# RinceWND/extPOM

Hardware: AMD Instinct MI355X
Metric: 3D cell-updates/sec on internal mode (one internal step = the 3-D baroclinic step and its isplit 2-D external substeps; whole-step wall time) (higher is better)
Workload: dtype f64

## Files before the change

### extpom_amd/csrc/k_adv.hip

```cpp
#include "pomgpu_internal.hpp"

#define dt_(i, j) F2(dt, i, j)
#define dx_(i, j) F2(dx, i, j)
#define dy_(i, j) F2(dy, i, j)
#define h_(i, j) F2(h, i, j)
#define u_(i, j, k) F3(u, i, j, k)
#define v_(i, j, k) F3(v, i, j, k)
#define ub_(i, j, k) F3(ub, i, j, k)
#define vb_(i, j, k) F3(vb, i, j, k)
#define w_(i, j, k) F3(w, i, j, k)
#define aam_(i, j, k) F3(aam, i, j, k)

#define MARCH3(call)                                                                  \
  const int g_ = (int)(blockIdx.x * blockDim.x + threadIdx.x);    \
  const int L_ = g_ >> 6, xcd_ = L_ & 7, m_ = L_ >> 3;                                \
  const int bpl_ = P.g_bpl, nbx_ = P.g_nbx;                                           \
  const int p_ = m_ % bpl_, t_ = m_ / bpl_;                                           \
  const int k = t_ % P.kb + 1;                                                        \
  const int band_ = (t_ / P.kb) * 8 + xcd_;                                           \
  const int i = (p_ % nbx_) * 64 + (g_ & 63) + 1;                                     \
  const int j = band_ * P.g_rb + (p_ / nbx_) * 4 + (int)threadIdx.y + 1;              \
  if (i > P.iml || j > P.jml) return;                                                 \
  call;
__device__ __forceinline__ void c_advct_a(const KP &P, const int i, const int j, const int k);
// ... 322 lines not shown
  }
  if (k >= 2 && k <= P.kbm1 && i >= 2 && i <= P.imm1 && j >= 2 && j <= P.jmm1) {
    const double fu = G3(ff, i, j, k - 1);
    double r = 0.;
    if (!(fc < value_min || fu < value_min)) {
      const double m = G3(zw, i, j, k);
      const double wdz = fabs(m);
      const double w2dt = P.dti2 * m * m / (F1(dzz, k - 1) * dt_(i, j));
      const double mol = (fu - fc) / (fc + fu + epsilon);
      r = (wdz - w2dt) * mol * P.sw;
      if (fabs(wdz) < fabs(w2dt)) r = 0.;
    }
    G3(zw, i, j, k) = r;
  }
}
__device__ __forceinline__ void c_copy3(const KP &P, const int i, const int j, const int k, double *dst, const double *src);
__global__ void k_copy3(KP P, double *dst, const double *src) {
  MARCH3(c_copy3(P, i, j, k, dst, src))
}
__device__ __forceinline__ void c_copy3(const KP &P, const int i, const int j, const int k, double *dst, const double *src) {
  G3(dst, i, j, k) = G3(src, i, j, k);
}
__device__ __forceinline__ void c_aam_copy(const KP &P, const int i, const int j, const int k, double *dst, const double *src) {
  if (k <= P.kbm1) G3(dst, i, j, k) = G3(src, i, j, k);
}
__global__ void k_aam_copy(KP P, double *dst, const double *src) {
  MARCH3(c_aam_copy(P, i, j, k, dst, src))
}
__device__ __forceinline__ double advt2_xdiff(const KP &P, const double *fb, const double *fc, int i, int j, int k) {
  const double am = 0.5 * (aam_(i, j, k) + aam_(i - 1, j, k));
  return -am * (h_(i, j) + h_(i - 1, j)) * P.tprni *
         ((G3(fb, i, j, k) - G3(fc, i, j, k)) - (G3(fb, i - 1, j, k) - G3(fc, i - 1, j, k))) * F2(dum, i, j) *
         (dy_(i, j) + dy_(i - 1, j)) * 0.5 / (dx_(i, j) + dx_(i - 1, j));
}
__device__ __forceinline__ double advt2_ydiff(const KP &P, const double *fb, const double *fc, int i, int j, int k) {
  const double am = 0.5 * (aam_(i, j, k) + aam_(i, j - 1, k));
  return -am * (h_(i, j) + h_(i, j - 1)) * P.tprni *
         ((G3(fb, i, j, k) - G3(fc, i, j, k)) - (G3(fb, i, j - 1, k) - G3(fc, i, j - 1, k))) * F2(dvm, i, j) *
         (dx_(i, j) + dx_(i, j - 1)) * 0.5 / (dy_(i, j) + dy_(i, j - 1));
}
__device__ __forceinline__ void c_advt2_diff(const KP &P, const int i, const int j, const int k, const double *fb, const double *fc, double *ff);
__global__ void k_advt2_diff(KP P, const double *fb, const double *fc, double *ff) {
  MARCH3(c_advt2_diff(P, i, j, k, fb, fc, ff))
}
__device__ __forceinline__ void c_advt2_diff(const KP &P, const int i, const int j, const int k, const double *fb, const double *fc, double *ff) {
  if (k > P.kbm1 || i < 2 || i > P.imm1 || j < 2 || j > P.jmm1) return;
  G3(ff, i, j, k) = G3(ff, i, j, k) -
                    P.dti2 * (advt2_xdiff(P, fb, fc, i + 1, j, k) - advt2_xdiff(P, fb, fc, i, j, k) +
                              advt2_ydiff(P, fb, fc, i, j + 1, k) - advt2_ydiff(P, fb, fc, i, j, k)) /
                        ((h_(i, j) + F2(etf, i, j)) * F2(art, i, j));
}

__device__ __forceinline__ double dens_point(const KP &P, double si, double ti, int i, int j, int k);
template <int TAU> __device__ __forceinline__ void c_ts_update(const KP &P, const int i, const int j, const int k, double fold, double fnew, int rt, int store_rst, double tau_b, double tau_f, const unsigned long long *rtf);
template <int TAU> __global__ void k_ts_update(KP P, double fold, double fnew, int rt, int store_rst, double tau_b, double tau_f, const unsigned long long *rtf) {
  MARCH3(c_ts_update<TAU>(P, i, j, k, fold, fnew, rt, store_rst, tau_b, tau_f, rtf))
}
__global__ void k_ts_update_same(KP P, double fold, double fnew, int rt, int store_rst, const unsigned long long *rtf) {
  MARCH3(c_ts_update<2>(P, i, j, k, fold, fnew, rt, store_rst, 0., 0., rtf))
}
template <int TAU> __device__ __forceinline__ void c_ts_update(const KP &P, const int i, const int j, const int k, double fold, double fnew, int rt, int store_rst, double tau_b, double tau_f, const unsigned long long *rtf) {
  const bool act = (i <= P.im && j <= P.jm), lev = (k <= P.kbm1);
  const pomgpu_ct m = F2(fsm, i, j);
  pomgpu_ct uf = F3(uf, i, j, k), vf = F3(vf, i, j, k);
  if (lev && act) {
    uf = uf * m;
    vf = vf * m;
  }
  pomgpu_ct tb = F3(tb, i, j, k), sb = F3(sb, i, j, k);
  bool rtc = rt != 0;
  if (rtc && rtf && lev) rtc = ((rtf[RT_WORD(P, i, j, k)] >> RT_BIT(i)) & 1ull) != 0;
  if (rtc) {
    const pomgpu_ct tc = F3(tclim, i, j, k), sc = F3(sclim, i, j, k);
    tb = (tb - tc) + tc;
    sb = (sb - sc) + sc;
  }
  const pomgpu_ct t0 = F3(t, i, j, k), s0 = F3(s, i, j, k);
  pomgpu_ct tbn = t0 + CT(.5) * CT(P.smoth) * (uf + tb - CT(2.) * t0);
  pomgpu_ct sbn = s0 + CT(.5) * CT(P.smoth) * (vf + sb - CT(2.) * s0);
  pomgpu_ct tn = uf, sn = vf;
  if (lev) {
    if (act) {
      const pomgpu_ct tr = CT(fold) * CT(F3(trstrb, i, j, k)) + CT(fnew) * CT(F3(trstrf, i, j, k));
      const pomgpu_ct sr = CT(fold) * CT(F3(srstrb, i, j, k)) + CT(fnew) * CT(F3(srstrf, i, j, k));
      pomgpu_ct ta;
      if (TAU == 1) ta = CT(fold) * CT(tau_b) + CT(fnew) * CT(tau_f);
      else if (TAU == 2) { const pomgpu_ct x = CT(F3(taurstrf, i, j, k)); ta = CT(fold) * x + CT(fnew) * x; }
      else ta = CT(fold) * CT(F3(taurstrb, i, j, k)) + CT(fnew) * CT(F3(taurstrf, i, j, k));
      if (store_rst) {
        F3(trstr, i, j, k) = tr;
        F3(srstr, i, j, k) = sr;
        F3(taurstr, i, j, k) = ta;
      }
      const pomgpu_ct c = CT(2.) * CT(P.dti) / CT(86400.);
      tn = tn + c * ta * (tr - tn);
      tbn = tbn + c * ta * (tr - tbn);
      sn = sn + c * ta * (sr - sn);
      sbn = sbn + c * ta * (sr - sbn);
    }
    tn = tn * m; tbn = tbn * m; sn = sn * m; sbn = sbn * m;
  }
  F3(t, i, j, k) = tn;
  F3(tb, i, j, k) = tbn;
  F3(s, i, j, k) = sn;
  F3(sb, i, j, k) = sbn;
  if (lev && act) F3(rho, i, j, k) = dens_point(P, sn, tn, i, j, k);
}
template <int NF> struct TrUpds { TrUpd u[NF]; };
template <int NF> __device__ __forceinline__ void c_tr_update(const KP &P, const int i, const int j, const int k, const TrUpds<NF> &A, int rt) {
  const bool msk = (i <= P.im && j <= P.jm && k <= P.kbm1);
  const double m = F2(fsm, i, j);
#pragma unroll
  for (int f = 0; f < NF; f++) {
    const TrUpd &u = A.u[f];
    double ff = G3(u.ff, i, j, k);
    if (msk) ff = ff * m;
    double fb = G3(u.fb, i, j, k);
    if (rt) {
      const double fc = G3(u.fc, i, j, k);
      fb = (fb - fc) + fc;
    }
    const double f0 = G3(u.f, i, j, k);
    G3(u.fb, i, j, k) = f0 + .5 * P.smoth * (ff + fb - 2. * f0);
    G3(u.f, i, j, k) = ff;
  }
}
template <int NF> __global__ void k_tr_update(KP P, TrUpds<NF> A, int rt) {
  MARCH3(c_tr_update<NF>(P, i, j, k, A, rt))
}
__device__ __forceinline__ void c_tr_source(const KP &P, const int i, const int j, const int k, double *ff, const double *fb, const double *fc, const double *q, double lam) {
  if (k > P.kbm1 || i > P.im || j > P.jm) return;
  double x = G3(fb, i, j, k);
  if (fc) { const double y = G3(fc, i, j, k); x = (x - y) + y; }
  const double a = lam * x;
  const double b = (q ? (double)G3(q, i, j, k) : 0.) - a;
  const double d = P.dti2 * b;
  G3(ff, i, j, k) = (double)G3(ff, i, j, k) + d;
}
__global__ void k_tr_source(KP P, double *ff, const double *fb, const double *fc, const double *q, double lam) {
  MARCH3(c_tr_source(P, i, j, k, ff, fb, fc, q, lam))
}
__device__ __forceinline__ void c_mask_ts(const KP &P, const int i, const int j, const int k);
__global__ void k_mask_ts(KP P) {
  MARCH3(c_mask_ts(P, i, j, k))
}
__device__ __forceinline__ void c_mask_ts(const KP &P, const int i, const int j, const int k) {
  if (k > P.kbm1 || i > P.im || j > P.jm) return;
  const double m = F2(fsm, i, j);
  F3(uf, i, j, k) = F3(uf, i, j, k) * m;
  F3(vf, i, j, k) = F3(vf, i, j, k) * m;
}
__device__ __forceinline__ void c_mask_uv(const KP &P, const int i, const int j, const int k);
__global__ void k_mask_uv(KP P) {
  MARCH3(c_mask_uv(P, i, j, k))
}
__device__ __forceinline__ void c_mask_uv(const KP &P, const int i, const int j, const int k) {
  if (k > P.kbm1 || i > P.im || j > P.jm) return;
  F3(uf, i, j, k) = F3(uf, i, j, k) * F2(dum, i, j);
  F3(vf, i, j, k) = F3(vf, i, j, k) * F2(dvm, i, j);
// ... 325 lines not shown
}
#undef LD2
#undef A3


void launch_advct_a(pomgpu_ctx *c) { LAUNCH(c, k_advct_a, gridm(c->P), blk2(), c->P); }
void launch_advct_b(pomgpu_ctx *c) { LAUNCH(c, k_advct_b, gridm(c->P), blk2(), c->P); }
void launch_advct_c(pomgpu_ctx *c) { LAUNCH(c, k_advct_c, gridm(c->P), blk2(), c->P); }
void launch_aam(pomgpu_ctx *c) {
  const KP &P = c->P;
#ifdef POMGPU_STORE_F32
  const bool pair_ok = false;
#else
  const bool pair_ok = true;
#endif
  if (pair_ok && P.iml % 2 == 0 && !SW(c, NO_PAIR)) {
    const long nbands = (P.jml + P.g_rb - 1) / P.g_rb, rounds = (nbands + 7) / 8;
    const long bpl = (long)((P.iml / 2 + 61) / 62) * (P.g_rb / 4);
    const long nch = (P.kbm1 + AAM_KCH - 1) / AAM_KCH;
    LAUNCHN(c, "k_aam_pair", k_aam_pair, dim3((unsigned)(8 * rounds * nch * bpl), 1, 1), blk2(), c->P);
  } else {
    LAUNCH(c, k_aam, gridm(c->P), blk2(), c->P);
  }
}
void launch_roundtrip(pomgpu_ctx *c, double *a, const double *b, int fix_kb) { LAUNCH(c, k_roundtrip, gridm(c->P), blk2(), c->P, a, b, fix_kb); }
void launch_roundtrip_level(pomgpu_ctx *c, double *a, const double *b, int k) { LAUNCH(c, k_roundtrip_level, grid2(c->P), blk2(), c->P, a, b, k); }
void launch_advq_flux(pomgpu_ctx *c, const double *q, const double *qb, double *xf, double *yf) {
  LAUNCH(c, k_advq_flux, gridm(c->P), blk2(), c->P, q, qb, xf, yf);
}
void launch_advq_step(pomgpu_ctx *c, const double *q, const double *qb, double *qf, const double *xf, const double *yf, int zero_else) {
  LAUNCH(c, k_advq_step, gridm(c->P), blk2(), c->P, q, qb, qf, xf, yf, zero_else);
}
void launch_q_filter(pomgpu_ctx *c, int mask) { LAUNCH(c, k_q_filter, gridm(c->P), blk2(), c->P, mask); }
void launch_q_filter_rim(pomgpu_ctx *c) {
  const KP &P = c->P;
  const int len = P.im > P.jm ? P.im : P.jm;
  LAUNCH(c, k_q_filter_rim, dim3((len + 63) / 64, 8, P.kb), dim3(64, 1, 1), c->P);
}
void launch_mask_q(pomgpu_ctx *c) { LAUNCH(c, k_mask_q, gridm(c->P), blk2(), c->P); }
void launch_advt1(pomgpu_ctx *c, double *fb, double *f, const double *fclim, double *ff) {
  LAUNCH(c, k_advt1, gridm(c->P), blk2(), c->P, (const double *)fb, (const double *)f, fclim, ff);
  LAUNCH(c, k_copy_kb, grid2(c->P), blk2(), c->P, f, (double *)NULL);
}
void launch_copy_kb(pomgpu_ctx *c, double *f, double *g) { LAUNCH(c, k_copy_kb, grid2(c->P), blk2(), c->P, f, g); }
void launch_advt2_mass(pomgpu_ctx *c) { LAUNCH(c, k_advt2_mass, gridm(c->P), blk2(), c->P); }
void launch_advt2_step(pomgpu_ctx *c, const double *fbmem, const double *f, const double *eta, double *ff, int itera) {
  LAUNCH(c, k_advt2_step, gridm(c->P), blk2(), c->P, fbmem, f, eta, ff, itera);
}
void launch_mask3(pomgpu_ctx *c, double *a, const double *m2) { LAUNCH(c, k_mask3, gridm(c->P), blk2(), c->P, a, m2); }
void launch_smol(pomgpu_ctx *c, const double *ff) { LAUNCH(c, k_smol, gridm(c->P), blk2(), c->P, ff); }
void launch_copy3(pomgpu_ctx *c, double *dst, const double *src) { LAUNCH(c, k_copy3, gridm(c->P), blk2(), c->P, dst, src); }
void launch_aam_copy(pomgpu_ctx *c, double *dst, const double *src) { LAUNCH(c, k_aam_copy, gridm(c->P), blk2(), c->P, dst, src); }
void launch_advt2_diff(pomgpu_ctx *c, const double *fb, const double *fc, double *ff) { LAUNCH(c, k_advt2_diff, gridm(c->P), blk2(), c->P, fb, fc, ff); }
void launch_ts_update(pomgpu_ctx *c, double fold, double fnew, int rt, int store_rst, int rt_flags) {
  const unsigned long long *rtf = (rt && rt_flags) ? c->rt_words : NULL;
  if (rtf && c->prof_on) {
    const int s = pomgpu_prof_slot(c, "ts_rt_flags");
    if (s >= 0) (c->parent ? c->parent : c)->prof[s].launches++;
  }
  if (c->tau_known[0] && c->tau_known[1] && !c->tau_handed && !SW(c, TAU_ARRAYS))
    LAUNCHN(c, "k_ts_update", (k_ts_update<1>), gridm(c->P), blk2(), c->P, fold, fnew, rt, store_rst, c->tau_val[0], c->tau_val[1], rtf);
  else if (c->tau_same && !c->tau_handed && !SW(c, TAU_ARRAYS))
    LAUNCH(c, k_ts_update_same, gridm(c->P), blk2(), c->P, fold, fnew, rt, store_rst, rtf);
  else
    LAUNCHN(c, "k_ts_update", (k_ts_update<0>), gridm(c->P), blk2(), c->P, fold, fnew, rt, store_rst, 0., 0., rtf);
}
void launch_restore_fields(pomgpu_ctx *c, double fold, double fnew) { LAUNCH(c, k_restore_fields, gridm(c->P), blk2(), c->P, fold, fnew); }
void launch_mask_ts(pomgpu_ctx *c) { LAUNCH(c, k_mask_ts, gridm(c->P), blk2(), c->P); }
void launch_tr_update(pomgpu_ctx *c, const TrUpd *u, int nf, int rt) {
  if (nf == 2) {
    TrUpds<2> A; A.u[0] = u[0]; A.u[1] = u[1];
    LAUNCHN(c, "k_tr_update2", (k_tr_update<2>), gridm(c->P), blk2(), c->P, A, rt);
  } else {
    TrUpds<1> A; A.u[0] = u[0];
    LAUNCHN(c, "k_tr_update", (k_tr_update<1>), gridm(c->P), blk2(), c->P, A, rt);
  }
}
void launch_tr_source(pomgpu_ctx *c, double *ff, const double *fb, const double *fc, const double *q, double lam) {
  LAUNCH(c, k_tr_source, gridm(c->P), blk2(), c->P, ff, fb, fc, q, lam);
}
void launch_mask_uv(pomgpu_ctx *c) { LAUNCH(c, k_mask_uv, gridm(c->P), blk2(), c->P); }
void launch_mask_w(pomgpu_ctx *c) { LAUNCH(c, k_mask_w, gridm(c->P), blk2(), c->P); }
void launch_restore(pomgpu_ctx *c, double fold, double fnew) { LAUNCH(c, k_restore, gridm(c->P), blk2(), c->P, fold, fnew); }
void launch_restore_shift(pomgpu_ctx *c) { LAUNCH(c, k_restore_shift, gridm(c->P), blk2(), c->P); }
void launch_restore_load(pomgpu_ctx *c, const double *tr, const double *sr, double tau, const double *taur, int fill_tau) { LAUNCH(c, k_restore_load, gridm(c->P), blk2(), c->P, tr, sr, tau, taur, fill_tau); }
void launch_probe_gpow15(pomgpu_ctx *c, long n, const double *x, double *out) { LAUNCH(c, k_probe_gpow15, dim3((unsigned)((n + 255) / 256), 1, 1), dim3(256, 1, 1), n, x, out); }
void launch_dens(pomgpu_ctx *c, const double *si, const double *ti, double *rhoo) { LAUNCH(c, k_dens, gridm(c->P), blk2(), c->P, si, ti, rhoo); }
void launch_realvertvl(pomgpu_ctx *c, int etf_is_et) {
  if (SW(c, REALVERTVL_CELLS)) LAUNCH(c, k_realvertvl, gridm(c->P), blk2(), c->P, etf_is_et);
  else LAUNCHN(c, "k_realvertvl_col", k_realvertvl_col, grid2(c->P), blk2(), c->P, etf_is_et);
}
```

### extpom_amd/csrc/k_tile.hip

```cpp
#include "pomgpu_internal.hpp"


__global__ void k_coef_static(KP P) {
  const int i = TID_I, j = TID_J;
  if (i > P.iml || j > P.jml) return;
  const int iw = i > 1 ? i - 1 : 1, js = j > 1 ? j - 1 : 1;
  P.m8[IX2(i, j)] = (unsigned char)((F2(fsm, i, j) != 0. ? 1 : 0) | (F2(dum, i, j) != 0. ? 2 : 0) | (F2(dvm, i, j) != 0. ? 4 : 0));
  K2(HSX, i, j) = F2(h, i, j) + F2(h, iw, j);
  K2(HSY, i, j) = F2(h, i, j) + F2(h, i, js);
  K2(DYSX, i, j) = F2(dy, i, j) + F2(dy, iw, j);
  K2(DXSX, i, j) = F2(dx, i, j) + F2(dx, iw, j);
  K2(DXSY, i, j) = F2(dx, i, j) + F2(dx, i, js);
  K2(DYSY, i, j) = F2(dy, i, j) + F2(dy, i, js);
  K2(DX4, i, j) = F2(dx, i, j) + F2(dx, iw, j) + F2(dx, i, js) + F2(dx, iw, js);
  K2(DY4, i, j) = F2(dy, i, j) + F2(dy, iw, j) + F2(dy, i, js) + F2(dy, iw, js);
  const int ie = i < P.iml ? i + 1 : P.iml, jn = j < P.jml ? j + 1 : P.jml;
  K2(CVA, i, j) = F2(dy, ie, j) - F2(dy, iw, j);
  K2(CVB, i, j) = F2(dx, i, jn) - F2(dx, i, js);
  K2(R2DXSX, i, j) = 2.0 / (F2(dx, i, j) + F2(dx, iw, j));
  K2(R2DYSY, i, j) = 2.0 / (F2(dy, i, j) + F2(dy, i, js));
  K2(RDX, i, j) = 1.0 / F2(dx, i, j);
  K2(RDY, i, j) = 1.0 / F2(dy, i, j);
  if (j == 1)
    for (int n = i - 1; n < POM_NBLK1D * P.kb; n += P.iml) P.r1[n] = 1.0 / P.b1[n];
}
__global__ void k_coef_dt(KP P) {
  const int i = TID_I, j = TID_J;
  if (i > P.iml || j > P.jml) return;
  const int iw = i > 1 ? i - 1 : 1, js = j > 1 ? j - 1 : 1;
  K2(CMX, i, j) = 0.25 * (F2(dy, iw, j) + F2(dy, i, j)) * (F2(dt, iw, j) + F2(dt, i, j));
  K2(CMY, i, j) = 0.25 * (F2(dx, i, js) + F2(dx, i, j)) * (F2(dt, i, js) + F2(dt, i, j));
  K2(DTSX, i, j) = F2(dt, i, j) + F2(dt, iw, j);
  K2(DTSY, i, j) = F2(dt, i, j) + F2(dt, i, js);
  K2(DT4, i, j) = F2(dt, i, j) + F2(dt, iw, j) + F2(dt, i, js) + F2(dt, iw, js);
}
__global__ void k_coef_eta(KP P, int uvm) {
  const int i = TID_I, j = TID_J;
  if (i > P.iml || j > P.jml) return;
  K2(HEA, i, j) = (F2(h, i, j) + F2(etb, i, j)) * F2(art, i, j);
  K2(HFA, i, j) = (F2(h, i, j) + F2(etf, i, j)) * F2(art, i, j);
  if (uvm) {
    const unsigned long long mb = UVM_MARK;
    double mark;
    __builtin_memcpy(&mark, &mb, sizeof mark);
    const int iw = i > 1 ? i - 1 : 1, js = j > 1 ? j - 1 : 1;
    const double cu = (F2(utb, i, j) + F2(utf, i, j)) / (F2(dt, i, j) + F2(dt, iw, j));
    const double cv = (F2(vtb, i, j) + F2(vtf, i, j)) / (F2(dt, i, j) + F2(dt, i, js));
    K2(UCOR, i, j) = (i >= 2 && i <= P.im && j <= P.jm) ? cu : mark;
    K2(VCOR, i, j) = (j >= 2 && j <= P.jm && i <= P.im) ? cv : mark;
  }
}

__device__ __forceinline__ pomgpu_ct upw_(pomgpu_ct m, pomgpu_ct lo, pomgpu_ct hi) {
  return CT(0.5) * ((m + fabs(m)) * lo + (m - fabs(m)) * hi);
}
struct FaceT { pomgpu_ct adv, dif; };
struct TFields { const double *fb[2], *f[2], *fcl[2]; double *ff[2]; unsigned long long *rtf; };
template <int NF> struct LevT { pomgpu_ct c[2 * NF + 2], o[2], h[ROWSHARE_SLOTS(2 * NF + 2)]; };
template <int NS> struct NbrT { pomgpu_ct s[NS], n[NS]; };
struct CoefT { pomgpu_ct cm, hs, msk, ds_num; InvDc den; };
__device__ __forceinline__ CoefT coef_x(const KP &P, int i, int j) {
  CoefT c; c.cm = K2(CMX, i, j); c.hs = K2(HSX, i, j); c.msk = F2(dum, i, j); c.ds_num = K2(DYSX, i, j); c.den = inv_of(CT(K2(DXSX, i, j))); return c;
}
__device__ __forceinline__ CoefT coef_y(const KP &P, int i, int j) {
  CoefT c; c.cm = K2(CMY, i, j); c.hs = K2(HSY, i, j); c.msk = F2(dvm, i, j); c.ds_num = K2(DXSY, i, j); c.den = inv_of(CT(K2(DYSY, i, j))); return c;
}
__device__ __forceinline__ FaceT advt2_face(const pomgpu_ct tprni, const CoefT &c, pomgpu_ct vel, pomgpu_ct fb_hi, pomgpu_ct fb_lo, pomgpu_ct fc_hi,
                                            pomgpu_ct fc_lo, pomgpu_ct am_hi, pomgpu_ct am_lo) {
  FaceT f;
  f.adv = upw_(c.cm * vel, fb_lo, fb_hi);
  const pomgpu_ct am = CT(0.5) * (am_hi + am_lo);
  f.dif = divi(-am * c.hs * tprni * ((fb_hi - fc_hi) - (fb_lo - fc_lo)) * c.msk * c.ds_num * CT(0.5), c.den);
  return f;
}
#if COL_WX != 1
#error "the row-sharing column kernels keep one wavefront per workgroup row (COL_WX == 1)"
#endif
// ... 104 lines not shown
        auto east = [&] {
          return advt2_face(tprni, coef_x(P, ie, jc), uvm_ld<0>(P, ie, jc, L), G3(A.fb[f], ie, jc, L), fb_c, G3(A.fcl[f], ie, jc, L), fc_c,
                            G3(P.aamc, ie, jc, L), am_c);
        };
        FaceT xe;
        xe.adv = halo_e(xw.adv, [&] { return east().adv; });
        xe.dif = halo_e(xw.dif, [&] { return east().dif; });
        const FaceT ys = advt2_face(tprni, cs, v_c, fb_c, nb.s[f], fc_c, nb.s[NF + f], am_c, nb.s[AM]);
        const FaceT yn = advt2_face(tprni, cn, nb.n[VV], nb.n[f], fb_c, nb.n[NF + f], fc_c, nb.n[AM], am_c);
        s_adv = xe.adv - xw.adv + yn.adv - ys.adv;
        s_dif = xe.dif - xw.dif + yn.dif - ys.dif;
        zu = (L == 1) ? w_c * f1[f] * art : upw_(w_c, fb_c, p_fb[f]) * art;
      }
      {
        pomgpu_ct rr = p_adv[f] + divi(p_zu[f] - zu, dzk);
        rr = divi(p_fb[f] * hea - dti2 * rr, hfa);
        rr = rr * fsm;
        rr = rr - divi(dti2 * p_dif[f], hfa);
        bstc(bff[f], (L >= 2 && L <= kbm1 + 1) ? ost : BOFF_NONE, (unsigned)(L >= 2 ? L - 2 : 0) * lvb, rr);
      }
      p_adv[f] = s_adv; p_dif[f] = s_dif; p_fb[f] = fb_c; p_zu[f] = zu;
    }
  };
  LevT<NF> ra, rb;
  load(ra, 0u);
  rb = ra;
  for (int L = 1; L <= kbm1 + 1; L += 2) {
    step(L, 1, ra, rb);
    step(L + 1, 0, rb, ra);
  }
  if (icol) {
    for (int k = in ? P.kb : 1; k <= P.kb; k++) {
#pragma unroll
      for (int f = 0; f < NF; f++) G3(A.ff[f], i, jc, k) = CT(G3(A.ff[f], i, jc, k)) * fsm;
    }
  }
}

struct QFields { const double *q[2], *qb[2]; double *qf[2]; };
template <int NF, int NO = 2> struct LevQa { pomgpu_ct c[2 * NF + 2], o[NO], h[ROWSHARE_SLOTS(2 * NF + 2)]; };
struct CoefQ { pomgpu_ct dts, hs, msk, ds_num; InvDc den; };
__device__ __forceinline__ CoefQ coefq_x(const KP &P, int i, int j) {
  CoefQ c; c.dts = K2(DTSX, i, j); c.hs = K2(HSX, i, j); c.msk = F2(dum, i, j); c.den = inv_of(CT(K2(DXSX, i, j))); c.ds_num = K2(DYSX, i, j); return c;
}
__device__ __forceinline__ CoefQ coefq_y(const KP &P, int i, int j) {
  CoefQ c; c.dts = K2(DTSY, i, j); c.hs = K2(HSY, i, j); c.msk = F2(dvm, i, j); c.den = inv_of(CT(K2(DYSY, i, j))); c.ds_num = K2(DXSY, i, j); return c;
}
__device__ __forceinline__ pomgpu_ct advq_face(const CoefQ &c, pomgpu_ct q_hi, pomgpu_ct q_lo, pomgpu_ct vel_k, pomgpu_ct vel_km1, pomgpu_ct am_hi_k,
                                               pomgpu_ct am_lo_k, pomgpu_ct am_hi_m, pomgpu_ct am_lo_m, pomgpu_ct qb_hi, pomgpu_ct qb_lo) {
  pomgpu_ct x = CT(.125) * (q_hi + q_lo) * c.dts * (vel_k + vel_km1);
  x = x - divi(CT(.25) * (am_hi_k + am_lo_k + am_hi_m + am_lo_m) * c.hs * (qb_hi - qb_lo) * c.msk, c.den);
  return CT(.5) * c.ds_num * x;
}
template <int NF, bool WF = false, bool UM = false>
__global__ void __launch_bounds__(64 * LDS_ROWS) k_advq_col(KP P, QFields A, int zero_else) {
  constexpr int NS = 2 * NF + 2, NH = ROWSHARE_SLOTS(NS), AM = 2 * NF, VV = 2 * NF + 1;
  typedef LevQa<NF, WF ? 1 : 2> Lev;
  HALO_XCD_DECODE_R(LDS_ROWS)
  const int r = WAVE_UNIFORM((int)threadIdx.y), j0w = j - r;
  const bool jrow = j <= P.jml;
  const int jc = jrow ? j : P.jml;
  const bool icol = jrow && (lane >= 1 && lane <= 62 && i0 <= P.iml);
#ifdef POMGPU_EMU
  if (!icol) return;
#endif
  const int i = i0 < 1 ? 1 : (i0 > P.iml ? P.iml : i0);
  const int iw = i > 1 ? i - 1 : 1, ie = i < P.iml ? i + 1 : P.iml;
  const int js = jc > 1 ? jc - 1 : 1, jn = jc < P.jml ? jc + 1 : P.jml;
  const bool in = icol && (i >= 2 && i <= P.imm1 && jc >= 2 && jc <= P.jmm1);
  const CoefQ cw = coefq_x(P, i, jc), cs = coefq_y(P, i, jc), cn = coefq_y(P, i, jn);
  const pomgpu_ct art = F2(art, i, jc), hea = K2(HEA, i, jc);
  const InvDc hfa = inv_of(CT(K2(HFA, i, jc)));
  const int kb = P.kb, kbm1 = P.kbm1;
  BufA bs[NS], bo[2], bqf[NF], bh[NH];
  const double *ps[NS];
#pragma unroll
  for (int f = 0; f < NF; f++) { ps[f] = A.q[f]; ps[NF + f] = A.qb[f]; bqf[f] = BUF3(A.qf[f]); }
  ps[AM] = P.aamc; ps[VV] = A3(v); bo[0] = BUF3(A3(u)); bo[1] = BUF3(A3(w));
#pragma unroll
  for (int x = 0; x < NS; x++) bs[x] = BUF3(ps[x]);
  const RowShare<NS> S = rowshare_setup<NS>(P, r, j, j0w, i);
#pragma unroll
  for (int q = 0; q < NH; q++) bh[q] = BUF3(rowshare_pick<NS>(ps, S.hop[q]));
  const UvmC mu = UM ? uvm_of<0>(P, i, jc) : uvm_none(), mv = UM ? uvm_of<1>(P, i, jc) : uvm_none();
  UvmC mh[NH];
#pragma unroll
  for (int q = 0; q < NH; q++) mh[q] = UM ? rowshare_uvm<1, NS, LDS_ROWS>(P, S, q, VV, j0w, i) : uvm_none();
  const unsigned oc = BOFF2(i, jc), lvb = LVB;
  const unsigned ost = in ? oc : ((zero_else && icol) ? oc : BOFF_NONE);
  const unsigned ostw = in ? oc : BOFF_NONE;
#ifndef POMGPU_EMU
  __shared__ pomgpu_ct slab[2][NS][ROWSHARE_ROWS][64];
#else
  const unsigned os = BOFF2(i, js), on = BOFF2(i, jn);
#endif
  double vv_cw = 0., vv_ce = 0., vv_cs = 0., vv_cn = 0., vv_det = 0., vv_m = 0., wk = 0.;
  InvD vv_area; vv_area.b = vv_area.y = 0.;
  if constexpr (WF) {
    vv_m = F2(fsm, i, jc);
    const double dyc = F2(dy, i, jc), dtc = F2(dt, i, jc), dxc = F2(dx, i, jc);
    const double dyw = halo_w(dyc, [&] { return F2(dy, iw, jc); }), dtw = halo_w(dtc, [&] { return F2(dt, iw, jc); });
    const double dye = halo_e(dyc, [&] { return F2(dy, ie, jc); }), dte = halo_e(dtc, [&] { return F2(dt, ie, jc); });
    vv_cw = .25 * (dyc + dyw) * (dtc + dtw);
    vv_ce = .25 * (dye + dyc) * (dte + dtc);
    vv_cs = .25 * (dxc + F2(dx, i, js)) * (dtc + F2(dt, i, js));
    vv_cn = .25 * (F2(dx, i, jn) + dxc) * (F2(dt, i, jn) + dtc);
    vv_area = inv_of(dxc * dyc);
    vv_det = (F2(etf, i, jc) - F2(etb, i, jc)) / P.dti2;
    wk = 0.5 * (F2(vfluxb, i, jc) + F2(vfluxf, i, jc));
  }
  auto load = [&](Lev &L, int k) {
    const unsigned lv = (unsigned)WAVE_UNIFORM(k - 1) * lvb;
#pragma unroll
    for (int x = 0; x < NS; x++) L.c[x] = bldc(bs[x], oc, lv);
    L.o[0] = bldc(bo[0], oc, lv);
    if constexpr (!WF) L.o[1] = bldc(bo[1], oc, lv);
#pragma unroll
    for (int q = 0; q < NH; q++) L.h[q] = bldc(bh[q], S.hoff[q], lv);
  };
  pomgpu_ct u_m = 0., v_m = 0., vn_m = 0., am_m = 0., ams_m = 0., amn_m = 0.;
  pomgpu_ct am_w_prv = 0.;
  pomgpu_ct ue_m = 0.;
  pomgpu_ct wq_pp[NF], wq_p[NF];
  pomgpu_ct xe_p[NF], xw_p[NF], yn_p[NF], ys_p[NF], qb_p[NF];
#pragma unroll
  for (int f = 0; f < NF; f++) wq_pp[f] = wq_p[f] = xe_p[f] = xw_p[f] = yn_p[f] = ys_p[f] = qb_p[f] = 0.;
  auto step = [&](const int L, const int par, const Lev &cur, Lev &nxt) {
    load(nxt, L + 1 <= kb ? L + 1 : kb);
    NbrT<NS> nb;
    const bool lcor = L <= kbm1;
    const pomgpu_ct v_c = uvm_fix(cur.c[VV], mv, lcor), u_c = uvm_fix(cur.o[0], mu, lcor);
#ifndef POMGPU_EMU
#pragma unroll
    for (int x = 0; x < NS; x++) slab[par][x][r + 1][lane] = x == VV ? v_c : cur.c[x];
#pragma unroll
    for (int q = 0; q < NH; q++) slab[par][S.hop[q]][S.hrow[q]][lane] = uvm_fix(cur.h[q], mh[q], lcor);
    __syncthreads();
#pragma unroll
    for (int x = 0; x < NS; x++) { nb.s[x] = slab[par][x][S.ss][lane]; nb.n[x] = slab[par][x][S.sn][lane]; }
#else
    const unsigned lvc = (unsigned)((L <= kb ? L : kb) - 1) * lvb;
#pragma unroll
    for (int x = 0; x < NS; x++) { nb.s[x] = bldc(bs[x], os, lvc); nb.n[x] = bldc(bs[x], on, lvc); }
    nb.s[VV] = uvm_fix(nb.s[VV], uvm_of<1>(P, i, js), lcor); nb.n[VV] = uvm_fix(nb.n[VV], uvm_of<1>(P, i, jn), lcor);
#endif
    const pomgpu_ct am_c = cur.c[AM];
    const pomgpu_ct am_s = nb.s[AM], am_n = nb.n[AM], v_n = nb.n[VV];
    const pomgpu_ct am_w = halo_w(am_c, [&] { return G3(P.aamc, iw, jc, L); });
    pomgpu_ct w_c, ue_c = 0.;
    if constexpr (WF) {
      ue_c = halo_e(u_c, [&] { return uvm_ld<0>(P, ie, jc, L); });
      const double wn = wk + F1(dz, L >= 2 ? L - 1 : 1) *
                             (divi(vv_ce * (double)ue_m - vv_cw * (double)u_m + vv_cn * (double)vn_m - vv_cs * (double)v_m, vv_area) + vv_det);
      wk = L >= 2 ? wn : wk;
      const double wst = L <= kbm1 ? wk * vv_m : wk;
      bst(bo[1], ostw, (unsigned)WAVE_UNIFORM(L - 1) * lvb, wst);
      w_c = CT((pomgpu_st)wst);
    } else {
      w_c = cur.o[1];
    }
    const int k = L - 1;
    InvDc dz2; dz2.b = dz2.y = 0.;
    if (k >= 2 && k <= kbm1) { dz2.b = CT(F1(dz, k)) + CT(F1(dz, k - 1)); dz2.y = CT(1.0) / dz2.b; }
#pragma unroll
    for (int f = 0; f < NF; f++) {
      const pomgpu_ct q_c = cur.c[f], qb_c = cur.c[NF + f];
      pomgpu_ct xe_c = 0., xw_c = 0., yn_c = 0., ys_c = 0.;
      if (L >= 2 && L <= kbm1) {
        const pomgpu_ct q_w = halo_w(q_c, [&] { return G3(A.q[f], iw, jc, L); });
        const pomgpu_ct qb_w = halo_w(qb_c, [&] { return G3(A.qb[f], iw, jc, L); });
        const pomgpu_ct xw = advq_face(cw, q_c, q_w, u_c, u_m, am_c, am_w, am_m, am_w_prv, qb_c, qb_w);
        xw_c = xw;
        xe_c = halo_e(xw, [&] {
          return advq_face(coefq_x(P, ie, jc), G3(A.q[f], ie, jc, L), q_c, uvm_ld<0>(P, ie, jc, L), uvm_ld<0>(P, ie, jc, L - 1), G3(P.aamc, ie, jc, L), am_c,
                           G3(P.aamc, ie, jc, L - 1), am_m, G3(A.qb[f], ie, jc, L), qb_c);
        });
        ys_c = advq_face(cs, q_c, nb.s[f], v_c, v_m, am_c, am_s, am_m, ams_m, qb_c, nb.s[NF + f]);
        yn_c = advq_face(cn, nb.n[f], q_c, v_n, vn_m, am_n, am_c, amn_m, am_m, nb.n[NF + f], qb_c);
      }
      const pomgpu_ct wq_c = w_c * q_c;
      {
        pomgpu_ct rr = 0.;
        if (in && k >= 2 && k <= kbm1) {
          rr = divi((wq_pp[f] - wq_c) * art, dz2) + xe_p[f] - xw_p[f] + yn_p[f] - ys_p[f];
          rr = divi(hea * qb_p[f] - CT(P.dti2) * rr, hfa);
        }
        const bool lev_in = (k >= 2 && k <= kbm1);
        const unsigned o = (k >= 1) ? (lev_in ? ost : ((zero_else && icol) ? oc : BOFF_NONE)) : BOFF_NONE;
        bstc(bqf[f], o, (unsigned)WAVE_UNIFORM(k >= 1 ? k - 1 : 0) * lvb, rr);
      }
      wq_pp[f] = wq_p[f]; wq_p[f] = wq_c; qb_p[f] = qb_c;
      xe_p[f] = xe_c; xw_p[f] = xw_c; yn_p[f] = yn_c; ys_p[f] = ys_c;
    }
    am_w_prv = am_w;
    if constexpr (WF) ue_m = ue_c;
    u_m = u_c; v_m = v_c; vn_m = v_n; am_m = am_c; ams_m = am_s; amn_m = am_n;
  };
  Lev ra, rb;
  load(ra, 1);
  rb = ra;
  for (int L = 1; L <= kb; L += 2) {
    step(L, 1, ra, rb);
    if (L + 1 <= kb) step(L + 1, 0, rb, ra);
  }
  if (icol && zero_else) {
#pragma unroll
    for (int f = 0; f < NF; f++) G3(A.qf[f], i, jc, kb) = 0.;
  }
  if constexpr (WF) {
    if (icol && !in && i0 <= P.im && jc <= P.jm)
      for (int k = 1; k <= kbm1; k++) F3(w, i, jc, k) = F3(w, i, jc, k) * vv_m;
  }
// ... 370 lines not shown
                    v_n = uvm_fix(bldc(bs[V], on, (unsigned)(k - 1) * lvb), uvm_of<1>(P, i, jn));
#endif
    const pomgpu_ct w_c = c.c[W];
    const pomgpu_ct w_w = halo_w(w_c, [&] { return F3(w, iw, jc, k + 1); });
    const pomgpu_ct tc = cd_c * (v_n + v_k);
    const pomgpu_ct tw = halo_w(tc, [&] { return F2(cor, iw, jc) * F2(dt, iw, jc) * (uvm_ld<1>(P, iw, jn, k) + uvm_ld<1>(P, iw, jc, k)); });
    const pomgpu_ct u_e = halo_e(u_k, [&] { return uvm_ld<0>(P, ie, jc, k); });
    const pomgpu_ct u_se = halo_e(u_s, [&] { return uvm_ld<0>(P, ie, js, k); });
    pomgpu_ct fu_n = 0., fv_n = 0.;
    if (k + 1 <= kbm1) {
      if (i >= 2) fu_n = CT(.25) * (w_c + w_w) * (u_c + u_k);
      if (jc >= 2) fv_n = CT(.25) * (w_c + w_s) * (v_c + v_k);
    }
    pomgpu_ct ru = fu_k, rv = fv_k;
    if (in) {
      InvDc dzk; dzk.b = F1(dz, k); dzk.y = R1(dz, k);
      ru = divi(sau * c.ub - CT(2.) * dti2 * (c.advx + divi((fu_k - fu_n) * aru, dzk) - aru * CT(.25) * (tc + tw) + hcu + c.drhox), sdu);
      rv = divi(sav * c.vb -
                    CT(2.) * dti2 * (c.advy + divi((fv_k - fv_n) * arv, dzk) + arv * CT(.25) * (cd_c * (u_e + u_k) + cd_s * (u_se + u_s)) + hcv + c.drhoy),
                sdv);
    }
    const unsigned lv = (unsigned)WAVE_UNIFORM(k - 1) * lvb;
    bstc(buf, ost, lv, ru);
    bstc(bvf, ost, lv, rv);
    fu_k = fu_n; fv_k = fv_n;
    u_k = u_c; v_k = v_c;
  };
  LevUV ra, rb;
  load(ra, 1);
  rb = ra;
  for (int k = 1; k <= kbm1; k += 6) {
    step(k, 1, ra, rb);
    if (k + 1 <= kbm1) step(k + 1, 2, rb, ra);
    if (k + 2 <= kbm1) step(k + 2, 0, ra, rb);
    if (k + 3 <= kbm1) step(k + 3, 1, rb, ra);
    if (k + 4 <= kbm1) step(k + 4, 2, ra, rb);
    if (k + 5 <= kbm1) step(k + 5, 0, rb, ra);
  }
  if (out) { F3(uf, i, jc, kb) = 0.; F3(vf, i, jc, kb) = 0.; }
}

void launch_coef_static(pomgpu_ctx *c) { LAUNCH(c, k_coef_static, grid2(c->P), blk2(), c->P); }
void launch_coef_dt(pomgpu_ctx *c) { LAUNCH(c, k_coef_dt, grid2(c->P), blk2(), c->P); }
void launch_coef_eta(pomgpu_ctx *c, int uvm) { LAUNCH(c, k_coef_eta, grid2(c->P), blk2(), c->P, uvm); }
void launch_advq_col(pomgpu_ctx *c, const double *q, const double *qb, double *qf, int zero_else) {
  QFields A; A.q[0] = A.q[1] = q; A.qb[0] = A.qb[1] = qb; A.qf[0] = A.qf[1] = qf;
  LAUNCHN(c, "k_advq_col", (k_advq_col<1>), grid1_halo_r(c->P, LDS_ROWS), blk_col_r(LDS_ROWS), c->P, A, zero_else);
}
void launch_advq2_col(pomgpu_ctx *c, const double *q, const double *qb, double *qf, const double *ql, const double *qlb, double *qlf, int zero_else) {
  QFields A; A.q[0] = q; A.qb[0] = qb; A.qf[0] = qf; A.q[1] = ql; A.qb[1] = qlb; A.qf[1] = qlf;
  LAUNCHN(c, "k_advq2_col", (k_advq_col<2>), grid1_halo_r(c->P, LDS_ROWS), blk_col_r(LDS_ROWS), c->P, A, zero_else);
}
#if POMGPU_W_FUSE
void launch_advq2w_col(pomgpu_ctx *c, const double *q, const double *qb, double *qf, const double *ql, const double *qlb, double *qlf, int zero_else) {
  QFields A; A.q[0] = q; A.qb[0] = qb; A.qf[0] = qf; A.q[1] = ql; A.qb[1] = qlb; A.qf[1] = qlf;
#if POMGPU_UVM_ONLOAD
  if (c->P.uvm) { LAUNCHN(c, "k_advq2_col", (k_advq_col<2, true, true>), grid1_halo_r(c->P, LDS_ROWS), blk_col_r(LDS_ROWS), c->P, A, zero_else); return; }
#endif
  LAUNCHN(c, "k_advq2_col", (k_advq_col<2, true>), grid1_halo_r(c->P, LDS_ROWS), blk_col_r(LDS_ROWS), c->P, A, zero_else);
}
#endif
void launch_advct_col(pomgpu_ctx *c, int sum2d, double *aam_w) {
  const bool rows4 = SW(c, ADVCT_ROWS4) || (!SW(c, ADVCT_ROWS8) && c->P.jml <= 400 && c->exch);
  sum2d = (sum2d ? 1 : 0) | (POMGPU_UVM_ONLOAD && !c->exch && !c->tp.on && !c->wide.on && !(c->flags & POMGPU_CTX_2D) ? 2 : 0);
#if POMGPU_AAM_FUSE
  if (aam_w) {
    if (c->prof_on) {
      const int s = pomgpu_prof_slot(c, "advct_aam_fused");
      if (s >= 0) (c->parent ? c->parent : c)->prof[s].launches++;
    }
    LAUNCHN(c, "k_advct_col", (k_advct_col<LDS_ROWS, true>), grid1_halo_r(c->P, LDS_ROWS), blk_col_r(LDS_ROWS), c->P, sum2d, aam_w);
    return;
  }
#endif
  if (rows4) LAUNCHN(c, "k_advct_col", (k_advct_col<4>), grid1_halo_r(c->P, 4), blk_col_r(4), c->P, sum2d, (double *)NULL);
  else LAUNCHN(c, "k_advct_col", (k_advct_col<LDS_ROWS>), grid1_halo_r(c->P, LDS_ROWS), blk_col_r(LDS_ROWS), c->P, sum2d, (double *)NULL);
}
__global__ void k_advct_fix2d(KP P, int west, int south) {
  const int t = TID_I;
  if (west && t >= 2 && t <= P.jmm1) {
    double a = 0.;
#pragma unroll 8
    for (int k = 1; k <= P.kbm1; k++) a = a + F3(advx, 2, t, k) * F1(dz, k);
    F2(adx2d, 2, t) = a;
  }
  if (south && t >= 2 && t <= P.imm1) {
    double a = 0.;
#pragma unroll 8
    for (int k = 1; k <= P.kbm1; k++) a = a + F3(advy, t, 2, k) * F1(dz, k);
    F2(ady2d, t, 2) = a;
  }
}
void launch_advct_fix2d(pomgpu_ctx *c, int west, int south) {
  const KP &P = c->P;
  const int len = P.im > P.jm ? P.im : P.jm;
  LAUNCH(c, k_advct_fix2d, dim3((len + 63) / 64, 1, 1), dim3(64, 1, 1), c->P, west, south);
}
void launch_advct_edge(pomgpu_ctx *c, double *to_e, double *to_n) {
  const KP &P = c->P;
  const int len = P.im > P.jm ? P.im : P.jm;
  LAUNCH(c, k_advct_edge, dim3((len + 63) / 64, P.kbm1, 1), dim3(64, 1, 1), c->P, to_e, to_n);
}
void launch_advct_fix(pomgpu_ctx *c, const double *from_w, const double *from_s) {
  const KP &P = c->P;
  const int len = P.im > P.jm ? P.im : P.jm;
  LAUNCH(c, k_advct_fix, dim3((len + 63) / 64, P.kbm1, 1), dim3(64, 1, 1), c->P, from_w, from_s);
}
void launch_advuv_col(pomgpu_ctx *c) {
#if POMGPU_UVM_ONLOAD
// ... 29 lines not shown
```

### extpom_amd/csrc/k_vert.hip

```cpp
#include <type_traits>
#include "pomgpu_internal.hpp"
#include "dd_exp.h"

#define dt_(i, j) F2(dt, i, j)
#define dx_(i, j) F2(dx, i, j)
#define dy_(i, j) F2(dy, i, j)
#define h_(i, j) F2(h, i, j)
#define u_(i, j, k) F3(u, i, j, k)
#define v_(i, j, k) F3(v, i, j, k)
#define w_(i, j, k) F3(w, i, j, k)

#define ROWS_PROFUV 1
#define ROWS_PROFT 1
#ifndef ROWS_UVF
#define ROWS_UVF 8
#endif
#ifndef ROWS_UVM
#define ROWS_UVM 4
#endif
#define COL2                               \
  const int i = TID_I, j = TID_J;          \
  if (i > P.iml || j > P.jml) return;

__global__ void k_baropg(KP P, int sum2d) {
// ... 310 lines not shown
    const unsigned lv = (unsigned)WAVE_UNIFORM(k - 1) * lvb;
    L.u = bld(bu, oc, lv); L.v = bld(bv, oc, lv); L.vh = bld(bv, onh, lv);
  };
  double wk = 0.5 * (F2(vfluxb, i, jc) + F2(vfluxf, i, jc));
  bst(bw, ost, 0u, mask ? wk * m : wk);
  auto step = [&](const int k, const Lev &cur, Lev &nxt) {
    const int par = k & 1;
    load(nxt, k + 2 <= kbm1 ? k + 2 : kbm1);
#ifndef POMGPU_EMU
    slab[par][r][lane] = cur.v;
    if (r == VVL_ROWS - 1) slab[par][VVL_ROWS][lane] = cur.vh;
    __syncthreads();
    const double v_n = slab[par][r + 1][lane];
#else
    (void)par;
    const double v_n = F3(v, i, jn, k);
#endif
    const double u_e = halo_e(cur.u, [&] { return F3(u, ie, jc, k); });
    wk = wk + F1(dz, k) * (divi(ce * u_e - cw * cur.u + cn * v_n - cs * cur.v, area) + det);
    bst(bw, ost, (unsigned)WAVE_UNIFORM(k) * lvb, (mask && k + 1 <= kbm1) ? wk * m : wk);
  };
  Lev ra, rb, rc;
  load(ra, 1);
  load(rb, 2 <= kbm1 ? 2 : kbm1);
  rc = ra;
  for (int k = 1; k <= kbm1; k += 3) {
    step(k, ra, rc);
    if (k + 1 <= kbm1) step(k + 1, rb, ra);
    if (k + 2 <= kbm1) step(k + 2, rc, rb);
  }
  if (own && !in && mask)
    for (int k = 1; k <= kbm1; k++) F3(w, i, jc, k) = w_(i, jc, k) * m;
}

__global__ void k_profq_bc(KP P) {
  COL2
  if (i > P.im || j > P.jm) return;
  double ut = 0.;
  if (i <= P.imm1 && j <= P.jmm1) {
    ut = sqrt(sq(.5 * (F2(wusurf, i, j) + F2(wusurf, i + 1, j))) + sq(.5 * (F2(wvsurf, i, j) + F2(wvsurf, i, j + 1))));
    F3(uf, i, j, P.kb) =
        sqrt(sq(.5 * (F2(wubot, i, j) + F2(wubot, i + 1, j))) + sq(.5 * (F2(wvbot, i, j) + F2(wvbot, i, j + 1)))) * P.const1_profq;
  }
  G2(P.s2[4], i, j) = ut;
}
__device__ __forceinline__ double profq_cc(const KP &P, int i, int j, int k) {
  const double tp = F3(t, i, j, k) + P.tbias;
  const double sp = F3(s, i, j, k) + P.sbias;
  const double p = P.grav * P.rhoref * (-F1(zz, k) * h_(i, j)) * 1.e-4;
  double cc = 1449.1 + .00821 * p + 4.55 * tp - .045 * sq(tp) + 1.34 * (sp - 35.0);
  cc = cc / sqrt((1. - .01642 * p / cc) * (1. - 0.40 * p / sq(cc)));
  return cc;
}
__device__ __forceinline__ double profq_cc_v(const KP &P, double t, double s_, double hij, int k) {
  const double tp = t + P.tbias;
  const double sp = s_ + P.sbias;
  const double p = P.grav * P.rhoref * (-F1(zz, k) * hij) * 1.e-4;
  double cc = 1449.1 + .00821 * p + 4.55 * tp - .045 * sq(tp) + 1.34 * (sp - 35.0);
  cc = cc / sqrt((1. - .01642 * p / cc) * (1. - 0.40 * p / sq(cc)));
  return cc;
}
__device__ __forceinline__ double profq_rho(const KP &P, int i, int j, int k, int rho_rt) {
  const double r = F3(rho, i, j, k);
  if (!rho_rt) return r;
  const double m = F3(rmean, i, j, k);
  return (r - m) + m;
}
__device__ __forceinline__ double profq_boygr(const KP &P, int i, int j, int k, double ccm, double cck, int rho_rt = 0) {
  return P.grav * (profq_rho(P, i, j, k - 1, rho_rt) - profq_rho(P, i, j, k, rho_rt)) / (F1(dzz, k - 1) * h_(i, j)) +
         sq(P.grav) * 2. / (sq(ccm) + sq(cck));
}
__global__ void k_profq_prod(KP P, int rho_rt) {
  COL2
  if (i > P.im || j > P.jm) return;
  double *prod = P.s3[0];
  G3(prod, i, j, 1) = 0.;
  G3(prod, i, j, P.kb) = 0.;
  const bool in = (i >= 2 && i <= P.imm1 && j >= 2 && j <= P.jmm1);
  if (!in) {
    for (int k = 2; k <= P.kbm1; k++) G3(prod, i, j, k) = 0.;
    return;
  }
  const double dh = h_(i, j) + F2(etf, i, j);
  const double sef = 1., shiw = 0.;
  double ccm = profq_cc(P, i, j, 1);
  for (int k = 2; k <= P.kbm1; k++) {
    const double cck = profq_cc(P, i, j, k);
    const double bg = profq_boygr(P, i, j, k, ccm, cck, rho_rt);
    const double km = F3(km, i, j, k);
    double p = km * .25 * sef *
                   (sq(u_(i, j, k) - u_(i, j, k - 1) + u_(i + 1, j, k) - u_(i + 1, j, k - 1)) +
                    sq(v_(i, j, k) - v_(i, j, k - 1) + v_(i, j + 1, k) - v_(i, j + 1, k - 1))) /
                   sq(F1(dzz, k - 1) * dh) -
               shiw * km * bg;
    p = p + F3(kh, i, j, k) * bg;
    G3(prod, i, j, k) = p;
    ccm = cck;
  }
}
__global__ void k_profq_prod_lines(KP P, int rho_rt) {
  const int t = TID_I, line = (int)blockIdx.y, k = (int)blockIdx.z + 1;
  int i, j;
  if (line < 4) { if (t > P.jm) return; j = t; i = line == 0 ? 1 : (line == 1 ? 2 : (line == 2 ? P.imm1 : P.im)); }
  else { if (t > P.im) return; i = t; j = line == 4 ? 1 : (line == 5 ? 2 : (line == 6 ? P.jmm1 : P.jm)); }
  double *prod = P.s3[0];
  double p = 0.;
  const bool wanted = line == 1 ? !P.W : (line == 2 ? !P.E : (line == 5 ? !P.S : (line == 6 ? !P.N : true)));
  if (!wanted) return;
  if (k >= 2 && k <= P.kbm1 && i >= 2 && i <= P.imm1 && j >= 2 && j <= P.jmm1) {
    const double dh = h_(i, j) + F2(etf, i, j);
    const double sef = 1., shiw = 0.;
    const double ccm = profq_cc(P, i, j, k - 1), cck = profq_cc(P, i, j, k);
    const double bg = profq_boygr(P, i, j, k, ccm, cck, rho_rt);
    const double km = F3(km, i, j, k);
    p = km * .25 * sef *
            (sq(u_(i, j, k) - u_(i, j, k - 1) + u_(i + 1, j, k) - u_(i + 1, j, k - 1)) +
             sq(v_(i, j, k) - v_(i, j, k - 1) + v_(i, j + 1, k) - v_(i, j + 1, k - 1))) /
            sq(F1(dzz, k - 1) * dh) -
        shiw * km * bg;
    p = p + F3(kh, i, j, k) * bg;
  }
  G3(prod, i, j, k) = p;
}
struct LevQ { double t, s, rho, rm, q2b, q2lb, q2, km, kh, uf, vf, uc, ue, vc, vn, kq1, prod; };
struct LevB { double e1, g1, e2, g2, qb, qlb, q, ql; };
#ifndef PROFQ_KL
#define PROFQ_KL 19
#endif
#ifndef PROFQ_BIG
#define PROFQ_BIG 8
#endif
template <int FP, int FF, int ROWS, int LD = 1>
__global__ void __launch_bounds__(64 * ROWS) k_profq(KP P, int rho_rt_pace, int jfirst, int jlast, const unsigned *rtcol) {
#ifndef POMGPU_EMU
  constexpr int KL = ROWS >= 8 ? PROFQ_KL : (PROFQ_KL < 9 ? PROFQ_KL : 9);
  __shared__ double evec[2 * KL][ROWS][64];
#endif
  const int i = TID_I, j = TID_J + jfirst - 1;
  if (i > P.iml || j > P.jml || j > jlast) return;
  const int rho_rt = rho_rt_pace & 1, pace = rho_rt_pace & 2;
  const int ty = (int)threadIdx.y, tx = (int)threadIdx.x;
  if (i > P.im || j > P.jm) return;
  const double a1 = 0.92, b1 = 16.6, a2 = 0.74, b2 = 10.1, c1 = 0.08, e1 = 1.8, e2 = 1.33, surfl = 2.e5;
  const int kb = P.kb, kbm1 = P.kbm1;
  const double dh = h_(i, j) + F2(etf, i, j);
  const double utau2 = G2(P.s2[4], i, j);
  const double l0 = surfl * utau2 / P.grav;
  const double umol2 = 2. * P.umol;
  const double z1 = F1(z, 1), zkb = F1(z, kb);
  const double coef4 = 18. * a1 * a1 + 9. * a1 * a2, coef5 = 9. * a1 * a2;
  const double coef1 = a2 * (1. - 6. * a1 / b1 * 1.), coef2 = 3. * a2 * b2 / 1. + 18. * a1 * a2,
               coef3 = a1 * (1. - 3. * c1 - 6. * a1 / b1 * 1.);
  const bool repl = (P.W && i == 1) || (P.E && i == P.im) || (P.S && j == 1) || (P.N && j == P.jm);
  const int ti = (P.W && i == 2) ? 1 : ((P.E && i == P.imm1) ? P.im : 0);
  const int tj = (P.S && j == 2) ? 1 : ((P.N && j == P.jmm1) ? P.jm : 0);
  const double fsm_c = F2(fsm, i, j);
  const double m_ti = F2(fsm, ti ? ti : i, j), m_tj = F2(fsm, i, tj ? tj : j), m_tij = F2(fsm, ti ? ti : i, tj ? tj : j);
  const bool pin = FP && (i >= 2 && i <= P.imm1 && j >= 2 && j <= P.jmm1);
  const bool ffil = FF && (i >= 3 && i <= P.imm1 - 1 && j >= 3 && j <= P.jmm1 - 1);
  const int ie = i < P.iml ? i + 1 : i, jn = j < P.jml ? j + 1 : j;
  const double hij = h_(i, j);
  const InvD dhk = inv_of(dh * P.kappa);
  UvmC m_uc = uvm_none(), m_ue = uvm_none(), m_vc = uvm_none(), m_vn = uvm_none();
#if POMGPU_UVM_ONLOAD
  if (FP == 1 && P.uvm) {
    m_uc.s = K2(USUM, i, j); m_uc.c = K2(UCOR, i, j); m_ue.s = K2(USUM, ie, j); m_ue.c = K2(UCOR, ie, j);
    m_vc.s = K2(VSUM, i, j); m_vc.c = K2(VCOR, i, j); m_vn.s = K2(VSUM, i, jn); m_vn.c = K2(VCOR, i, jn);
    m_uc.on = m_ue.on = m_vc.on = m_vn.on = true;
  }
#endif
#define bt BUF3(A3(t))
#define bs_ BUF3(A3(s))
#define brho BUF3(A3(rho))
#define bq2b BUF3(A3(q2b))
#define bq2lb BUF3(A3(q2lb))
#define bq2 BUF3(A3(q2))
#define bq2l BUF3(A3(q2l))
#define bkm BUF3(A3(km))
#define bkh BUF3(A3(kh))
#define bkq BUF3(A3(kq))
#define buf BUF3(A3(uf))
#define bvf BUF3(A3(vf))
#define bu BUF3(A3(u))
#define bv BUF3(A3(v))
#define bl BUF3(A3(l))
#define bdt BUF3(A3(dtef))
#define bpr BUF3(P.s3[0])
#define be1 BUF3(P.s3[4])
#define be2 BUF3(P.s3[5])
  const unsigned oc = BOFF2(i, j), oe = BOFF2(ie, j), on = BOFF2(i, jn), lvb = LVB;
  const unsigned o_k = repl ? BOFF_NONE : oc;
  const unsigned o_abs = ffil ? BOFF_NONE : oc;
  const unsigned o_fil = ffil ? oc : BOFF_NONE, o_uv = ffil ? BOFF_NONE : oc;
  const unsigned o_pr = (FP == 0 || (FP == 2 && !pin)) ? oc : BOFF_NONE;
  unsigned o_rm = rho_rt ? oc : BOFF_NONE;
  if (rho_rt_pace & 4) o_rm = (rho_rt && rtcol[(size_t)(j - 1) * P.iml + (i - 1)]) ? oc : BOFF_NONE;
#ifdef PROFQ_OLDWALK
  const double vbot = P.kappa * (1 + F1(z, kbm1)) * dh * F3(q2, i, j, kbm1);
  const double ufbot = F3(uf, i, j, kb);
#else
  double ufbot;
#endif
  double e1p = 0., g1p = P.cb_profq * utau2;
  double e2p = 0., g2p = 0.;
  double ccm = 0., rhom = 0.;
  double kqm = 0., kqc = F3(kq, i, j, 1);
  double ucm = 0., uem = 0., vcm = 0., vnm = 0.;
#ifdef PROFQ_OLDWALK
  auto lev = [&](LevQ &L, int k) {
    const unsigned lv = (unsigned)WAVE_UNIFORM(k - 1) * lvb;
    L.t = bld(bt, oc, lv); L.s = bld(bs_, oc, lv); L.rho = bld(brho, oc, lv); L.rm = bld(BUF3(A3(rmean)), o_rm, lv);
    L.q2b = bld(bq2b, oc, lv); L.q2lb = bld(bq2lb, oc, lv); L.q2 = bld(bq2, oc, lv);
    L.km = bld(bkm, oc, lv); L.kh = bld(bkh, oc, lv);
    L.uf = bld(buf, oc, lv); L.vf = bld(bvf, oc, lv);
    if (FP) { L.uc = bld(bu, oc, lv); L.ue = bld(bu, oe, lv); L.vc = bld(bv, oc, lv); L.vn = bld(bv, on, lv); }
    else L.uc = L.ue = L.vc = L.vn = 0.;
    L.kq1 = bld(bkq, oc, (unsigned)WAVE_UNIFORM(k < kb ? k : kb - 1) * lvb);
    L.prod = (FP != 1) ? bld(bpr, o_pr, lv) : 0.;
  };
  auto step = [&](const int k, const LevQ &cur, LevQ &nxt) {
    lev(nxt, k + 1 <= kb ? k + 1 : kb);
    const bool mid = (k >= 2 && k <= kbm1);
    const unsigned lv = (unsigned)WAVE_UNIFORM(k - 1) * lvb;
    const double kqp = cur.kq1;
    double cck = 0., rhok = 0.;
    if (k <= kbm1) { cck = profq_cc_v(P, cur.t, cur.s, hij, k); rhok = (o_rm != BOFF_NONE) ? (cur.rho - cur.rm) + cur.rm : cur.rho; }
    double q2b = cur.q2b;
    double l, gh = 0.;
    double uck = 0., uek = 0., vck = 0., vnk = 0., bg = 0.;
    if (pin && k <= kbm1) { uck = uvm_fix(cur.uc, m_uc); uek = uvm_fix(cur.ue, m_ue); vck = uvm_fix(cur.vc, m_vc); vnk = uvm_fix(cur.vn, m_vn); }
    double q2lb = 0.;
    if (mid) {
      q2b = fabs(q2b);
      q2lb = fabs(cur.q2lb);
      bg = P.grav * (rhom - rhok) / (F1(dzz, k - 1) * hij) + sq(P.grav) * 2. / (sq(ccm) + sq(cck));
      l = fabs(q2lb / q2b);
      if (F1(z, k) > -0.5) l = fmax(l, P.kappa * l0);
      gh = fmin(sq(l) * bg / q2b, .028);
    } else {
      l = (k == 1) ? P.kappa * l0 : 0.;
    }
    bst(bq2b, mid ? o_abs : BOFF_NONE, lv, q2b);
    bst(bq2lb, mid ? o_abs : BOFF_NONE, lv, q2lb);
    if (LD) bst(bl, oc, lv, l);
    const double dtef1 = sqrt(fabs(q2b)) * 1. / (b1 * l + P.small_);
    double dtef2 = dtef1;
    if (mid) dtef2 = dtef1 * (1. + e2 * sq(divi((1. / fabs(F1(z, k) - z1) + 1. / fabs(F1(z, k) - zkb)) * l, dhk)));
    if (LD) bst(bdt, oc, lv, dtef2);
    if (mid) {
      const double a = -P.dti2 * (kqp + kqc + umol2) * .5 / (F1(dzz, k - 1) * F1(dz, k) * dh * dh);
      const double c = -P.dti2 * (kqm + kqc + umol2) * .5 / (F1(dzz, k - 1) * F1(dz, k - 1) * dh * dh);
      double pr;
      if (FP == 0 || (FP == 2 && !pin)) {
        pr = cur.prod;
      } else if (pin) {
        const double sef = 1., shiw = 0.;
        const double km = cur.km;
        pr = km * .25 * sef * (sq(uck - ucm + uek - uem) + sq(vck - vcm + vnk - vnm)) / sq(F1(dzz, k - 1) * dh) - shiw * km * bg;
        pr = pr + cur.kh * bg;
      } else {
        pr = 0.;
      }
      const double g = 1. / (a + c * (1. - e1p) - (2. * P.dti2 * dtef1 + 1.));
      e1p = a * g;
      g1p = (-2. * P.dti2 * pr + c * g1p - cur.uf) * g;
      if (k == 2) {
        e2p = 0.;
        g2p = -P.kappa * F1(z, 2) * dh * cur.q2;
      } else {
        const double rhs = (k == kbm1) ? vbot : cur.vf;
        const double g2 = 1. / (a + c * (1. - e2p) - (P.dti2 * dtef2 + 1.));
        e2p = a * g2;
        g2p = (P.dti2 * (-pr * l * e1) + c * g2p - rhs) * g2;
      }
    }
    {
      const unsigned ov = (k <= kbm1) ? oc : BOFF_NONE;
#ifndef POMGPU_EMU
      const bool inl = k <= KL;
      if (inl) { evec[k - 1][ty][tx] = e1p; evec[KL + k - 1][ty][tx] = e2p; }
      const unsigned oe_ = inl ? BOFF_NONE : ov;
#else
      const unsigned oe_ = ov;
#endif
      bst(be1, oe_, lv, e1p); bst(buf, ov, lv, g1p); bst(be2, oe_, lv, e2p); bst(bvf, ov, lv, g2p);
    }
    double kq_n = 0., km_n = 0., kh_n = 0.;
    {
      const double sh = coef1 / (1. - coef2 * gh);
      double sm = coef3 + sh * coef4 * gh;
      sm = sm / (1. - coef5 * gh);
      const double pl = l * sqrt(fabs(cur.q2));
      kq_n = (pl * .41 * sh + kqc) * .5;
      km_n = (pl * sm + cur.km) * .5;
      kh_n = (pl * sh + cur.kh) * .5;
      bst(bkq, o_k, lv, kq_n * fsm_c);
      bst(bkm, o_k, lv, km_n * fsm_c);
      bst(bkh, o_k, lv, kh_n * fsm_c);
    }
    if ((ti | tj) && !repl) {
#define PUT(ii, jj, m)                               \
  {                                                  \
    G3(P.s3[1], ii, jj, k) = km_n * m;               \
    G3(P.s3[2], ii, jj, k) = kh_n * m;               \
    G3(P.s3[3], ii, jj, k) = kq_n * m;               \
  }
      if (ti) PUT(ti, j, m_ti)
      if (tj) PUT(i, tj, m_tj)
      if (ti && tj) PUT(ti, tj, m_tij)
#undef PUT
    }
    ccm = cck; rhom = rhok;
    ucm = uck; uem = uek; vcm = vck; vnm = vnk;
    kqm = kqc; kqc = kqp;
  };
  {
    LevQ ra, rb;
    lev(ra, 1);
    rb = ra;
    for (int k = 1; k <= kb; k += 2) {
      if (pace) PACE_BARRIER();
      step(k, ra, rb);
      if (k + 1 <= kb) step(k + 1, rb, ra);
    }
  }
#else
  enum { PH_1, PH_2, PH_LDS, PH_MEM, PH_KBM1, PH_KB };
  auto lev = [&](LevQ &L, int k) {
    const unsigned lv = (unsigned)WAVE_UNIFORM(k - 1) * lvb;
    L.t = bld(bt, oc, lv); L.s = bld(bs_, oc, lv); L.rho = bld(brho, oc, lv); L.rm = bld(BUF3(A3(rmean)), o_rm, lv);
    L.q2b = bld(bq2b, oc, lv); L.q2lb = bld(bq2lb, oc, lv); L.q2 = bld(bq2, oc, lv);
    L.km = bld(bkm, oc, lv); L.kh = bld(bkh, oc, lv);
    L.uf = bld(buf, oc, lv); L.vf = bld(bvf, oc, lv);
    if (FP) { L.uc = bld(bu, oc, lv); L.ue = bld(bu, oe, lv); L.vc = bld(bv, oc, lv); L.vn = bld(bv, on, lv); }
    else L.uc = L.ue = L.vc = L.vn = 0.;
    L.kq1 = bld(bkq, oc, (unsigned)WAVE_UNIFORM(k < kb ? k : kb - 1) * lvb);
    L.prod = (FP != 1) ? bld(bpr, o_pr, lv) : 0.;
  };
  auto step = [&](auto ph, const int k, const LevQ &cur, LevQ &nxt) {
    constexpr int PH = decltype(ph)::value;
    constexpr bool mid = (PH != PH_1 && PH != PH_KB);
    if (PH != PH_KB) lev(nxt, k + 1);
    const unsigned lv = (unsigned)WAVE_UNIFORM(k - 1) * lvb;
    const double kqp = cur.kq1;
    double cck = 0., rhok = 0.;
    if (PH != PH_KB) { cck = profq_cc_v(P, cur.t, cur.s, hij, k); rhok = (o_rm != BOFF_NONE) ? (cur.rho - cur.rm) + cur.rm : cur.rho; }
    double q2b = cur.q2b;
    double l, gh = 0.;
    double uck = 0., uek = 0., vck = 0., vnk = 0., bg = 0.;
    if (PH != PH_KB) {
      uck = pin ? uvm_fix(cur.uc, m_uc) : 0.; uek = pin ? uvm_fix(cur.ue, m_ue) : 0.;
      vck = pin ? uvm_fix(cur.vc, m_vc) : 0.; vnk = pin ? uvm_fix(cur.vn, m_vn) : 0.;
    }
    double q2lb = 0.;
    if (mid) {
      q2b = fabs(q2b);
      q2lb = fabs(cur.q2lb);
      bg = P.grav * (rhom - rhok) / (F1(dzz, k - 1) * hij) + sq(P.grav) * 2. / (sq(ccm) + sq(cck));
      l = fabs(q2lb / q2b);
      const double lmx = fmax(l, P.kappa * l0);
      l = (F1(z, k) > -0.5) ? lmx : l;
      gh = fmin(sq(l) * bg / q2b, .028);
      bst(bq2b, o_abs, lv, q2b);
      bst(bq2lb, o_abs, lv, q2lb);
    } else {
      l = (PH == PH_1) ? P.kappa * l0 : 0.;
    }
    if (LD) bst(bl, oc, lv, l);
    const double dtef1 = sqrt(fabs(q2b)) * 1. / (b1 * l + P.small_);
    double dtef2 = dtef1;
    if (mid) dtef2 = dtef1 * (1. + e2 * sq(divi((1. / fabs(F1(z, k) - z1) + 1. / fabs(F1(z, k) - zkb)) * l, dhk)));
    if (LD) bst(bdt, oc, lv, dtef2);
    if (mid) {
      const double a = -P.dti2 * (kqp + kqc + umol2) * .5 / (F1(dzz, k - 1) * F1(dz, k) * dh * dh);
      const double c = -P.dti2 * (kqm + kqc + umol2) * .5 / (F1(dzz, k - 1) * F1(dz, k - 1) * dh * dh);
      double pr;
      if (FP == 0) {
        pr = cur.prod;
      } else {
        const double sef = 1., shiw = 0.;
        const double km = cur.km;
        pr = km * .25 * sef * (sq(uck - ucm + uek - uem) + sq(vck - vcm + vnk - vnm)) / sq(F1(dzz, k - 1) * dh) - shiw * km * bg;
        pr = pr + cur.kh * bg;
        pr = pin ? pr : (FP == 2 ? cur.prod : 0.);
      }
      const double g = 1. / (a + c * (1. - e1p) - (2. * P.dti2 * dtef1 + 1.));
      e1p = a * g;
      g1p = (-2. * P.dti2 * pr + c * g1p - cur.uf) * g;
      if (PH == PH_2) {
        e2p = 0.;
        g2p = -P.kappa * F1(z, 2) * dh * cur.q2;
      } else {
        const double rhs = (PH == PH_KBM1) ? P.kappa * (1 + F1(z, kbm1)) * dh * cur.q2 : cur.vf;
        const double g2 = 1. / (a + c * (1. - e2p) - (P.dti2 * dtef2 + 1.));
        e2p = a * g2;
        g2p = (P.dti2 * (-pr * l * e1) + c * g2p - rhs) * g2;
      }
    }
    if (PH != PH_KB) {
#ifndef POMGPU_EMU
      if (PH == PH_1 || PH == PH_2 || PH == PH_LDS) {
        evec[k - 1][ty][tx] = e1p; evec[KL + k - 1][ty][tx] = e2p;
      } else if (PH == PH_MEM) {
        bst(be1, oc, lv, e1p); bst(be2, oc, lv, e2p);
      } else {
        const bool inl = k <= KL;
        if (inl) { evec[k - 1][ty][tx] = e1p; evec[KL + k - 1][ty][tx] = e2p; }
        const unsigned oe_ = inl ? BOFF_NONE : oc;
        bst(be1, oe_, lv, e1p); bst(be2, oe_, lv, e2p);
      }
#else
      bst(be1, oc, lv, e1p); bst(be2, oc, lv, e2p);
#endif
      bst(buf, oc, lv, g1p); bst(bvf, oc, lv, g2p);
    }
    double kq_n = 0., km_n = 0., kh_n = 0.;
    {
      const double sh = coef1 / (1. - coef2 * gh);
      double sm = coef3 + sh * coef4 * gh;
      sm = sm / (1. - coef5 * gh);
      const double pl = l * sqrt(fabs(cur.q2));
      kq_n = (pl * .41 * sh + kqc) * .5;
      km_n = (pl * sm + cur.km) * .5;
      kh_n = (pl * sh + cur.kh) * .5;
      bst(bkq, o_k, lv, kq_n * fsm_c);
      bst(bkm, o_k, lv, km_n * fsm_c);
      bst(bkh, o_k, lv, kh_n * fsm_c);
    }
    if ((ti | tj) && !repl) {
#define PUT(ii, jj, m)                               \
  {                                                  \
    G3(P.s3[1], ii, jj, k) = km_n * m;               \
    G3(P.s3[2], ii, jj, k) = kh_n * m;               \
    G3(P.s3[3], ii, jj, k) = kq_n * m;               \
  }
// ... 865 lines not shown
  G3(b, i, j, kb) = c_kb;
  G3(c, i, j, kb) = f_kb;
  if (V) F2(tps, i, j) = su;
#undef KC
}
__global__ void k_uv_filter_rim(KP P) {
  if (blockIdx.z == 0) d_uv_filter_rim<0>(P);
  else d_uv_filter_rim<1>(P);
}

static inline dim3 colblk() { return dim3(64, 2, 1); }
static inline dim3 rowblk(int rows) { return dim3(64, rows, 1); }
static inline dim3 rowgrid(const KP &P, int rows) { return dim3((P.iml + 63) / 64, (P.jml + rows - 1) / rows, 1); }
static inline dim3 colgrid(const KP &P) { return dim3((P.iml + 63) / 64, (P.jml + 1) / 2, 1); }
#define COLV_G(P) dim3(((P).iml + 63) / 64, ((P).jml + 3) / 4, 1)
#define COLV_B dim3(64, 4, 1)
int launch_baropg(pomgpu_ctx *c, int sum2d, unsigned *rtcol) {
  if (SW(c, BAROPG_CELLS)) { LAUNCH(c, k_baropg, COLV_G(c->P), COLV_B, c->P, sum2d); return 0; }
  LAUNCHN(c, "k_baropg", k_baropg_rs, grid1_halo_r(c->P, BPG_ROWS), blk_col_r(BPG_ROWS), c->P, sum2d, rtcol);
  return rtcol != NULL;
}
void launch_baropg_mcc(pomgpu_ctx *c, int sum2d) { LAUNCH(c, k_baropg_mcc, colgrid(c->P), colblk(), c->P, sum2d); }
void launch_order_pack(pomgpu_ctx *c, double *send_e, double *send_n) {
  const KP &P = c->P;
  const int len = P.iml > P.jml ? P.iml : P.jml;
  LAUNCH(c, k_order_pack, dim3((len + 63) / 64, P.kb + 1, 1), dim3(64, 1, 1), c->P, send_e, send_n);
}
static inline dim3 twin(dim3 g) { g.z = 2; return g; }
template <class F> static void with_kbt(int kb, F f) {
  if (kb <= 24) f(std::integral_constant<int, 24>{});
  else if (kb <= 32) f(std::integral_constant<int, 32>{});
  else if (kb <= 40) f(std::integral_constant<int, 40>{});
  else if (kb <= 44) f(std::integral_constant<int, 44>{});
  else if (kb <= 50) f(std::integral_constant<int, 50>{});
  else if (kb <= 56) f(std::integral_constant<int, 56>{});
  else f(std::integral_constant<int, 64>{});
}
#define KBT_OF(t) decltype(t)::value
void launch_int_uvmean(pomgpu_ctx *c) {
  if (!pomgpu_reg_kb(c)) { LAUNCH(c, k_int_uvmean, colgrid(c->P), colblk(), c->P); return; }
  with_kbt(c->P.kb, [&](auto t) { LAUNCHN(c, "k_int_uvmean_reg2", (k_int_uvmean_reg2<KBT_OF(t)>), twin(rowgrid(c->P, ROWS_UVM)), rowblk(ROWS_UVM), c->P); });
}
void launch_vertvl(pomgpu_ctx *c, int mask) {
  if (SW(c, VERTVL_CELLS)) { LAUNCH(c, k_vertvl, COLV_G(c->P), COLV_B, c->P, mask); return; }
  LAUNCHN(c, "k_vertvl", k_vertvl_rs, grid1_halo_r(c->P, VVL_ROWS), blk_col_r(VVL_ROWS), c->P, mask);
}
void launch_profq_bc(pomgpu_ctx *c) { LAUNCH(c, k_profq_bc, colgrid(c->P), colblk(), c->P); }
void launch_profq_prod(pomgpu_ctx *c, int lines_only, int rho_rt) {
  if (!lines_only) { LAUNCH(c, k_profq_prod, colgrid(c->P), colblk(), c->P, rho_rt); return; }
  const KP &P = c->P;
  const int len = P.im > P.jm ? P.im : P.jm;
  LAUNCH(c, k_profq_prod_lines, dim3((len + 63) / 64, 8, P.kb), dim3(64, 1, 1), c->P, rho_rt);
}
void launch_profq(pomgpu_ctx *c, int fuse_prod, int fuse_filter, int rho_rt, int jfirst, int jlast, int store_ld) {
  if (jlast < jfirst) { jfirst = 1; jlast = c->P.jml; }
  const int ld = store_ld || fuse_prod != 1 || !fuse_filter;
  if (ld && c->prof_on) {
    const int s = pomgpu_prof_slot(c, "profq_ld_store");
    if (s >= 0) (c->parent ? c->parent : c)->prof[s].launches++;
  }
  const int nrows = jlast - jfirst + 1;
  const int rows8 = !SW(c, PROFQ_ROWS2) && (SW(c, PROFQ_ROWS8) || (long)((c->P.iml + 63) / 64) * ((c->P.jml + 7) / 8) >= 3 * 256);
  const int cols = rho_rt && c->rho_rt_cols && !SW(c, RT_LOAD);
  if (cols && c->prof_on) {
    const int s = pomgpu_prof_slot(c, "profq_rm_flags");
    if (s >= 0) (c->parent ? c->parent : c)->prof[s].launches++;
  }
  rho_rt = (rho_rt ? 1 : 0) | (SW(c, PROFQ_NOPACE) ? 0 : 2) | (cols ? 4 : 0);
#define PQ(FP, FF, LD)                                                                                                                   \
  do {                                                                                                                                   \
    if (rows8) LAUNCHN(c, "k_profq", (k_profq<FP, FF, PROFQ_BIG, LD>), dim3((c->P.iml + 63) / 64, (nrows + PROFQ_BIG - 1) / PROFQ_BIG, 1), dim3(64, PROFQ_BIG, 1), c->P, rho_rt, jfirst, jlast, c->rt_cols); \
    else LAUNCHN(c, "k_profq", (k_profq<FP, FF, 2, LD>), dim3((c->P.iml + 63) / 64, (nrows + 1) / 2, 1), dim3(64, 2, 1), c->P, rho_rt, jfirst, jlast, c->rt_cols); \
  } while (0)
  if (fuse_filter) { if (fuse_prod == 0) PQ(0, 1, 1); else if (fuse_prod == 1) { if (ld) PQ(1, 1, 1); else PQ(1, 1, 0); } else PQ(2, 1, 1); }
  else { if (fuse_prod == 0) PQ(0, 0, 1); else if (fuse_prod == 1) PQ(1, 0, 1); else PQ(2, 0, 1); }
#undef PQ
  const KP &P = c->P;
  if (P.W || P.E || P.S || P.N) {
    const int len = P.im > P.jm ? P.im : P.jm;
    LAUNCH(c, k_profq_rim, dim3((len + 63) / 64, 4, P.kb), dim3(64, 1, 1), c->P);
  }
}
template <int KBT>
static void launch_proft_reg(pomgpu_ctx *c, double *f, const double *wfsurf, const double *fsurf, int nbc) {
  if (nbc == 2 || nbc == 4) LAUNCHN(c, "k_proft_reg", (k_proft_reg<KBT, 1>), rowgrid(c->P, ROWS_PROFT), rowblk(ROWS_PROFT), c->P, f, wfsurf, fsurf, nbc);
  else LAUNCHN(c, "k_proft_reg", (k_proft_reg<KBT, 0>), rowgrid(c->P, ROWS_PROFT), rowblk(ROWS_PROFT), c->P, f, wfsurf, fsurf, nbc);
}
void launch_proft(pomgpu_ctx *c, double *f, const double *wfsurf, const double *fsurf, int nbc) {
  if (!pomgpu_reg_kb(c)) { LAUNCH(c, k_proft, colgrid(c->P), colblk(), c->P, f, wfsurf, fsurf, nbc); return; }
  with_kbt(c->P.kb, [&](auto t) { launch_proft_reg<KBT_OF(t)>(c, f, wfsurf, fsurf, nbc); });
}
#define PROFT_TS_KBMAX 56
template <int KBT>
static void launch_proft2_reg(pomgpu_ctx *c, const ProftArgs &a0, const ProftArgs &a1, int sw, int lane) {
  if constexpr (KBT <= PROFT_TS_KBMAX) {
    if (lane) {
      if (c->prof_on) {
        const int s = pomgpu_prof_slot(c, "proft_ts_lane");
        if (s >= 0) (c->parent ? c->parent : c)->prof[s].launches++;
      }
      LAUNCHN(c, "k_proft_reg2", (k_proft_ts_reg<KBT>), rowgrid(c->P, ROWS_PROFT), rowblk(ROWS_PROFT), c->P, a0, a1);
      return;
    }
  }
  if (sw) LAUNCHN(c, "k_proft_reg2", (k_proft_reg2<KBT, 1>), twin(rowgrid(c->P, ROWS_PROFT)), rowblk(ROWS_PROFT), c->P, a0, a1);
  else LAUNCHN(c, "k_proft_reg2", (k_proft_reg2<KBT, 0>), twin(rowgrid(c->P, ROWS_PROFT)), rowblk(ROWS_PROFT), c->P, a0, a1);
}
int launch_proft2(pomgpu_ctx *c, double *f0, const double *wfsurf0, const double *fsurf0, int nbc0, double *f1, const double *wfsurf1, const double *fsurf1, int nbc1) {
  const int sw0 = (nbc0 == 2 || nbc0 == 4), sw1 = (nbc1 == 2 || nbc1 == 4);
  if (!pomgpu_reg_kb(c) || sw0 != sw1) return 0;
  const ProftArgs a0 = {f0, wfsurf0, fsurf0, nbc0}, a1 = {f1, wfsurf1, fsurf1, nbc1};
  const int lane = !SW(c, PROFT_TWIN) && !sw0 && (nbc0 <= 2) == (nbc1 <= 2);
  with_kbt(c->P.kb, [&](auto t) { launch_proft2_reg<KBT_OF(t)>(c, a0, a1, sw0, lane); });
  return 1;
}
void launch_advu_profu(pomgpu_ctx *c, int do_adv, int do_prof) { LAUNCH(c, k_advu_profu, colgrid(c->P), colblk(), c->P, do_adv, do_prof); }
void launch_advv_profv(pomgpu_ctx *c, int do_adv, int do_prof) { LAUNCH(c, k_advv_profv, colgrid(c->P), colblk(), c->P, do_adv, do_prof); }
int launch_profuv_reg(pomgpu_ctx *c) {
  const KP &P = c->P;
  if (!pomgpu_reg_kb(c)) return 0;
  with_kbt(P.kb, [&](auto t) {
    LAUNCHN(c, "k_profuv_reg2", (k_profuv_reg2<KBT_OF(t)>), dim3((P.iml + 61) / 62, (P.jml + ROWS_PROFUV - 1) / ROWS_PROFUV, 2), rowblk(ROWS_PROFUV), c->P);
  });
  return 1;
}
void launch_profuv_filter_reg(pomgpu_ctx *c, double *ubk, double *vbk) {
  const KP &P = c->P;
  LAUNCH(c, k_uvb_bottom, grid2(P), blk2(), c->P, ubk, vbk);
  with_kbt(P.kb, [&](auto t) {
// ... 38 lines not shown
```

### extpom_amd/csrc/pomgpu_api.hip

```cpp
#include <math.h>
#include <stdarg.h>
#include <stdio.h>
#include <stdlib.h>
#include <string.h>
#include <vector>
#include "pomgpu.h"
#include "pomgpu_internal.hpp"

struct ProfPair { int slot; hipEvent_t a, b; };
struct ProfState { std::vector<ProfPair> pending; std::vector<ProfPair> free_; char filter[64]; };
static ProfState *PS(pomgpu_ctx *c) { return (ProfState *)c->prof_state; }

#define SLOT2(c, n) ((c)->P.b2 + (size_t)(n) * (c)->P.n2)
#define SLOT3(c, n) ((c)->P.b3 + (size_t)(n) * (c)->P.a3)
#define D2(c, name) SLOT2(c, P2_##name)
#define D3(c, name) SLOT3(c, P3_##name)
#define LEV3(c, p, lev) ((double *)((pomgpu_st *)(p) + (size_t)(lev) * (c)->P.n2))

int pomgpu_fail(pomgpu_ctx *c, int code, const char *fmt, ...) {
  if (c && c->parent) c = c->parent;
  if (c) {
    va_list ap;
    va_start(ap, fmt);
    vsnprintf(c->err, sizeof c->err, fmt, ap);
// ... 175 lines not shown
}

static const int X2_SLOT[POMGPU_NGEN] = {P2_ua, P2_va, P2_d, P2_el, P2_elb, P2_uab, P2_vab};
static void ext_buffers(pomgpu_ctx *c) {
  KP &P = c->P;
  for (int n = 0; n < POMGPU_NGEN; n++) P.x2[n] = P.y2[n] = c->ext_parity ? c->alt2[n] : P.b2 + (size_t)X2_SLOT[n] * P.n2;
}
static void rho_materialize(pomgpu_ctx *c) {
  if (!c->rho_rt_pending || (c->flags & POMGPU_CTX_2D)) return;
  c->rho_rt_pending = c->rho_rt_cols = 0;
  launch_roundtrip(c, SLOT3(c, P3_rho), SLOT3(c, P3_rmean), 2);
}
static void side_join(pomgpu_ctx *c);
static void side_begin(pomgpu_ctx *c);
static void side_end(pomgpu_ctx *c, hipEvent_t ev);
static int rim_side(pomgpu_ctx *c);
static void early_invalidate(pomgpu_ctx *c);
void pomgpu_wr_materialize(pomgpu_ctx *c) {
  if (!c->wr_pending) return;
  c->wr_pending = 0;
  (void)hipSetDevice(c->device);
  if (!(c->flags & POMGPU_CTX_2D)) launch_realvertvl(c, 1);
}
static bool wr_on_demand(const pomgpu_ctx *c) {
  return !c->exch && !c->tp.on && !c->wide.on && !c->parent && !(c->flags & POMGPU_CTX_2D) && !c->wr_eager && !SW(c, WR_NODEFER);
}
static bool uv_fused(const pomgpu_ctx *c) {
  const KP &P = c->P;
  return !c->exch && !c->tp.on && !c->wide.on && !c->parent && !(c->flags & POMGPU_CTX_2D) && !c->wr_eager && pomgpu_reg_kb(c) &&
         P.im >= 8 && P.jm >= 8 && !SW(c, UV_NOFUSE);
}
static bool w_fused(const pomgpu_ctx *c) {
  return POMGPU_W_FUSE && !c->exch && !c->tp.on && !c->wide.on && !(c->flags & POMGPU_CTX_2D) && !SW(c, ADVQ_SINGLE) && !SW(c, ADVQ_EXCHANGE) &&
         !SW(c, VERTVL_CELLS) && !SW(c, W_NOFUSE);
}
static bool uvm_onload(const pomgpu_ctx *c) {
  const pom_blkcon &k = c->con;
  return POMGPU_UVM_ONLOAD && w_fused(c) && uv_fused(c) && c->uvm_valid && !SW(c, UVMEAN_PASS) &&
         (k.mode == 4 || (k.nadv == 2 && c->P.nitera == 1 && !SW(c, ADVT2_SINGLE))) &&
         (!c->ntr || (k.nadv == 2 && c->P.nitera == 1));
}
static bool rt_one_tile(const pomgpu_ctx *c) { return !c->exch && !c->tp.on && !c->wide.on && !c->parent && !(c->flags & POMGPU_CTX_2D) && !c->wr_eager; }
static bool ld_on_demand(const pomgpu_ctx *c) {
  return !c->exch && !c->tp.on && !c->wide.on && !c->parent && !(c->flags & POMGPU_CTX_2D) && !c->wr_eager && !SW(c, LD_EAGER);
}
static bool next_step_fetches_record(const pomgpu_ctx *c) {
  if (!c->frc_on && !c->lat_on && !c->wat_on) return false;
  const pom_blkcon &k = c->con;
  const int isrf = (int)(.125 * 86400. / k.dti), ibc = (int)((double)(1.f / 24.f) * 86400. / k.dti), iwater = (int)(86400. / k.dti);
  const int next = k.iint + 1 + k.cont_bry;
  return (c->frc_on && (isrf < 1 || next % isrf == 0)) || (c->lat_on && (ibc < 1 || next % ibc == 0)) ||
         (c->wat_on && (iwater < 1 || (k.iint + 1) % iwater == 0));
}
static void aam_buffers(pomgpu_ctx *c) {
  KP &P = c->P;
  P.aamc = (c->aam_parity && c->aam_spare) ? c->aam_spare : (P.b3 ? P.b3 + (size_t)P3_aam * P.a3 : NULL);
}
static void aam_canonical(pomgpu_ctx *c) {
  if (!c->aam_parity) return;
  (void)hipSetDevice(c->device);
  launch_aam_copy(c, SLOT3(c, P3_aam), c->aam_spare);
  c->aam_parity = 0;
  aam_buffers(c);
}
static bool aam_fused(pomgpu_ctx *c) {
  if (!POMGPU_AAM_FUSE || c->exch || c->tp.on || c->wide.on || c->parent || (c->flags & POMGPU_CTX_2D) || c->wr_eager || c->P.mode == 2 ||
      SW(c, AAM_NOFUSE) || c->aam_spare_failed)
    return false;
  if (!c->aam_spare) {
    const size_t bytes = c->P.n3 * sizeof(pomgpu_st);
    if (hipMalloc((void **)&c->aam_spare, bytes) != hipSuccess) { (void)hipGetLastError(); c->aam_spare = NULL; c->aam_spare_failed = 1; return false; }
    (void)hipMemsetAsync(c->aam_spare, 0, bytes, c->stream);
  }
  return true;
}
static void uvf_materialize(pomgpu_ctx *c) {
  if (!c->uvf_pending) return;
  c->uvf_pending = 0;
  launch_uvf_copy(c);
}
static void restore_materialize(pomgpu_ctx *c) {
  c->uvm_valid = 0;
  side_join(c);
  rho_materialize(c);
  pomgpu_wr_materialize(c);
  uvf_materialize(c);
  aam_canonical(c);
  if (!c->rst_pending) return;
  c->rst_pending = 0;
  launch_restore_fields(c, c->rst_fold, c->rst_fnew);
}
static void ext_flush_deferred(pomgpu_ctx *c);
static void ext_canonical(pomgpu_ctx *c) {
  ext_flush_deferred(c);
  if (!c->ext_parity) return;
  KP &P = c->P;
  for (int n = 0; n < POMGPU_NGEN; n++) launch_copy2(c, P.b2 + (size_t)X2_SLOT[n] * P.n2, c->alt2[n]);
  c->ext_parity = 0;
  ext_buffers(c);
}
static int ctx_create(pomgpu_ctx **out, const pomgpu_dims *d, int device, void *stream, int flags);
extern "C" int pomgpu_create(pomgpu_ctx **out, const pomgpu_dims *d, int device, void *stream) {
  return ctx_create(out, d, device, stream, 0);
}
static int ctx_create(pomgpu_ctx **out, const pomgpu_dims *d, int device, void *stream, int flags) {
  if (!out || !d) return POMGPU_EINVAL;
  *out = NULL;
  if (d->kb < 4 || d->kb > POMGPU_KBMAX || d->im < 5 || d->jm < 5 || d->im > d->im_local || d->jm > d->jm_local) {
    fprintf(stderr, "pomgpu_create: unsupported extents im=%d jm=%d kb=%d (need im,jm>=5, 4<=kb<=%d)\n", d->im, d->jm,
            d->kb, POMGPU_KBMAX);
    return POMGPU_EINVAL;
  }
  if ((size_t)d->im_local * d->jm_local * d->kb * sizeof(double) >= ((size_t)1 << 32)) {
    fprintf(stderr, "pomgpu_create: a 3-D array of this tile has %zu bytes; the column kernels address a level with 32-bit offsets "
                    "(< 4 GiB per array): split the domain into more tiles\n", (size_t)d->im_local * d->jm_local * d->kb * sizeof(double));
    return POMGPU_EINVAL;
  }
  int ndev = 0;
  if (hipGetDeviceCount(&ndev) != hipSuccess || ndev <= 0 || device < 0 || device >= ndev) {
    fprintf(stderr, "pomgpu_create: no usable HIP device (count=%d, asked %d); the hot path has no CPU fallback\n", ndev,
            device);
    return POMGPU_ENODEV;
  }
  pomgpu_ctx *c = (pomgpu_ctx *)calloc(1, sizeof(pomgpu_ctx));
  if (!c) return POMGPU_ENOMEM;
  c->device = device;
  c->flags = flags;
  c->lbry_sides = POMGPU_SIDE_EAST | POMGPU_SIDE_SOUTH;
  if (hipSetDevice(device) != hipSuccess) { free(c); return POMGPU_EHIP; }
  KP &P = c->P;
  P.im = d->im; P.jm = d->jm; P.kb = d->kb; P.imm1 = d->im - 1; P.jmm1 = d->jm - 1; P.kbm1 = d->kb - 1; P.kbm2 = d->kb - 2;
  P.iml = d->im_local; P.jml = d->jm_local;
  P.W = d->n_west == -1; P.E = d->n_east == -1; P.S = d->n_south == -1; P.N = d->n_north == -1;
  P.n2 = (size_t)P.iml * P.jml; P.n3 = P.n2 * P.kb;
  pomgpu_switches_read(c->sw);
  {
    const long pages = SW(c, PAD3) ? SWV(c, PAD3) : 0;
    P.a3 = P.n3 + (pages > 0 ? (size_t)pages * 512 : 0);
  }
  set_band_geometry(P, c->sw);
  size_t off = 0; int s = 0;
#define BD_(name, shape) P.bdoff[s++] = off; off += BDN_##shape;
#define BDN_J ((size_t)P.jml)
#define BDN_I ((size_t)P.iml)
#define BDN_JK ((size_t)P.jml * P.kb)
#define BDN_IK ((size_t)P.iml * P.kb)
  POM_BDRY(BD_)
#undef BD_
  const size_t nbd = off;
  c->con.error_status = 0;
  if (stream) { c->stream = (hipStream_t)stream; c->own_stream = false; }
  else {
    if (hipStreamCreateWithFlags(&c->stream, hipStreamNonBlocking) != hipSuccess) { free(c); return POMGPU_EHIP; }
    c->own_stream = true;
  }
  c->cur = c->stream;
  c->prof_state = new ProfState();
  PS(c)->filter[0] = 0;
  bool ok = true;
  auto alloc = [&](double **p, size_t n) {
    if (!ok) return;
    if (hipMalloc((void **)p, n * sizeof(double)) != hipSuccess) { ok = false; *p = NULL; return; }
    if (hipMemsetAsync(*p, 0, n * sizeof(double), c->stream) != hipSuccess) ok = false;
  };
  alloc(&P.b1, (size_t)POM_NBLK1D * P.kb);
  alloc(&P.r1, (size_t)POM_NBLK1D * P.kb);
  alloc(&P.b2, (size_t)POM_NBLK2D * P.n2);
  const bool only2d = (flags & POMGPU_CTX_2D) != 0;
  if (!only2d) alloc(&P.b3, (size_t)POM_NBLK3D * P.a3);
  alloc(&P.bd, nbd);
  for (int n = 0; n < POMGPU_NSCR3 && !only2d; n++) alloc(&P.s3[n], P.n3);
  for (int n = 0; n < POMGPU_NSCR2; n++) alloc(&P.s2[n], P.n2);
  for (int n = 0; n < 2 && !only2d; n++) alloc(&c->uvb_bot[n], P.n2);
  if (!only2d) {
    double *m = NULL; alloc(&m, (size_t)(P.kb > 1 ? P.kb - 1 : 1) * P.jml * RT_NBX(P)); c->rt_words = (unsigned long long *)m;
    m = NULL; alloc(&m, (P.n2 + 1) / 2); c->rt_cols = (unsigned *)m;
  }
  for (int n = 0; n < POMGPU_NCOEF2; n++) alloc(&P.c2[n], P.n2);
  alloc(&c->alt2[0], (size_t)POMGPU_NGEN * P.n2);
  for (int n = 1; n < POMGPU_NGEN && ok; n++) c->alt2[n] = c->alt2[0] + (size_t)n * P.n2;
  { double *m = NULL; alloc(&m, (P.n2 + 7) / 8 + 1); P.m8 = (unsigned char *)m; }
  for (int n = 0; n < 2; n++) {
    const size_t len = (size_t)(P.kb + 1) * (n == 0 ? P.jml : P.iml);
    alloc(&c->ord_send[n], len);
    alloc(&c->ord_recv[n], len);
  }
  if (ok) { P.g4[2] = c->ord_recv[0]; P.g4[0] = c->ord_recv[0] + P.jml; P.g4[3] = c->ord_recv[1]; P.g4[1] = c->ord_recv[1] + P.iml; }
  alloc(&c->d_vel, 4);
  alloc(&c->d_stats, 8);
  if (ok && hipMalloc((void **)&c->d_err, sizeof(int)) != hipSuccess) ok = false;
  if (ok && hipMalloc((void **)&c->d_areas, sizeof(int)) != hipSuccess) ok = false;
  if (ok && hipMemsetAsync(c->d_areas, 0, sizeof(int), c->stream) != hipSuccess) ok = false;
  if (ok && hipMemsetAsync(c->d_err, 0, sizeof(int), c->stream) != hipSuccess) ok = false;
  if (SW(c, DEBUG_ALLOC))
    fprintf(stderr, "pomgpu_create: b1 %p r1 %p b2 %p b3 %p bd %p s3[0] %p s3[4] %p s2[0] %p c2[0] %p\n", (void *)P.b1, (void *)P.r1, (void *)P.b2,
            (void *)P.b3, (void *)P.bd, (void *)P.s3[0], (void *)P.s3[4], (void *)P.s2[0], (void *)P.c2[0]);
  if (!ok) {
    fprintf(stderr, "pomgpu_create: device allocation failed (%zu MB per 3-D array)\n", P.n3 * 8 >> 20);
    pomgpu_destroy(c);
    return POMGPU_ENOMEM;
  }
  c->ext_parity = 0;
  c->rst_pending = 0;
  ext_buffers(c);
  aam_buffers(c);
  (void)hipStreamSynchronize(c->stream);
  *out = c;
  return POMGPU_OK;
}

static void wide_free(pomgpu_ctx *c);
extern "C" void pomgpu_destroy(pomgpu_ctx *c) {
  if (!c) return;
  (void)hipSetDevice(c->device);
  if (c->stream) (void)hipStreamSynchronize(c->stream);
  if (c->side) (void)hipStreamSynchronize(c->side);
  if (pomgpu_io_wait(c) != POMGPU_OK)
    fprintf(stderr, "pomgpu_destroy: the output / restart file still being written could not be completed -- call pomgpu_io_wait (or pomgpu_sync) "
                    "before pomgpu_destroy to get its status\n");
  wide_free(c);
  pomgpu_tp_free(c);
  pomgpu_ff_free(c);
  KP &P = c->P;
  (void)hipFree(P.r1);
  if (c->tune_block) {
    (void)hipFree(c->tune_block);
    c->tune_block = NULL; P.b3 = NULL;
    for (int n = 0; n < POMGPU_NSCR3; n++) P.s3[n] = NULL;
  }
  (void)hipFree(P.b1); (void)hipFree(P.b2); (void)hipFree(P.b3); (void)hipFree(P.bd);
  for (int n = 0; n < POMGPU_NSCR3; n++) (void)hipFree(P.s3[n]);
  for (int n = 0; n < POMGPU_NSCR2; n++) (void)hipFree(P.s2[n]);
  (void)hipFree(c->uvb_bot[0]); (void)hipFree(c->uvb_bot[1]);
  (void)hipFree(c->rt_words); (void)hipFree(c->rt_cols);
  (void)hipFree(c->aam_spare);
  for (int n = 0; n < POMGPU_NCOEF2; n++) (void)hipFree(P.c2[n]);
  (void)hipFree(c->alt2[0]); (void)hipFree(c->alt3[0]);
  (void)hipFree(P.m8);
  for (int n = 0; n < 2; n++) { (void)hipFree(c->ord_send[n]); (void)hipFree(c->ord_recv[n]); }
  for (int n = 0; n <= POMGPU_MAXREC; n++) { (void)hipFree(c->rec_t[n]); (void)hipFree(c->rec_s[n]); (void)hipFree(c->rec_tau[n]); }
  (void)hipFree(c->d_vel); (void)hipFree(c->d_err); (void)hipFree(c->d_areas); (void)hipFree(c->d_stats); (void)hipFree(c->ext_bar);
  for (int k = 0; k < 3; k++) for (int sl = 0; sl < 4; sl++) { (void)hipFree(c->frc_dev[k][sl][0]); (void)hipFree(c->frc_dev[k][sl][1]); }
  for (int sl = 0; sl < 4; sl++) { (void)hipFree(c->lat_dev[sl]); (void)hipFree(c->wat_dev[sl]); }
  (void)hipFree(c->mean_acc);
  tracers_free(c);
  ProfState *ps = PS(c);
  if (ps) {
    for (auto &p : ps->pending) { (void)hipEventDestroy(p.a); (void)hipEventDestroy(p.b); }
    for (auto &p : ps->free_) { (void)hipEventDestroy(p.a); (void)hipEventDestroy(p.b); }
    delete ps;
  }
  if (c->side) {
    (void)hipEventDestroy(c->ev_fork); (void)hipEventDestroy(c->ev_early);
    for (auto &e : c->side_ev) (void)hipEventDestroy(e.ev);
    (void)hipStreamDestroy(c->side);
  }
  if (c->own_stream && c->stream) (void)hipStreamDestroy(c->stream);
  free(c);
}

extern "C" int pomgpu_debug_switch(pomgpu_ctx *c, const char *name, const char *value) {
  if (!c || !name) return POMGPU_EINVAL;
  if (strncmp(name, "POMGPU_", 7) == 0) name += 7;
  for (int n = 0; n < SW__count; n++)
    if (strcmp(POMGPU_SW_NAMES[n], name) == 0) {
      pomgpu_ctx *two[2] = {c, c->wide.x};
      for (pomgpu_ctx *t : two)
        if (t) { t->sw.on[n] = value ? 1 : 0; t->sw.val[n] = value ? atol(value) : 0; }
      if (n == SW_AAM_NOFUSE) aam_canonical(c);
      return POMGPU_OK;
    }
  return fail(c, POMGPU_EINVAL, "debug_switch: no switch named %s", name);
}
extern "C" const char *pomgpu_last_error(const pomgpu_ctx *c) { return c ? c->err : "null context"; }
extern "C" void *pomgpu_stream(pomgpu_ctx *c) { return c ? (void *)c->stream : NULL; }
extern "C" void *pomgpu_current_stream(pomgpu_ctx *c) { return c ? (void *)c->cur : NULL; }

static int pull_err(pomgpu_ctx *c) {
  if (c->launch_err) return POMGPU_EHIP;
  int e = 0;
  HIPCHK(c, hipMemcpyAsync(&e, c->d_err, sizeof(int), hipMemcpyDeviceToHost, c->stream));
  HIPCHK(c, hipStreamSynchronize(c->stream));
  if (e) c->con.error_status = 1;
  if (e & POMGPU_DERR_BARRIER) {
    pomgpu_ctx *two[2] = {c, c->wide.x};
    for (pomgpu_ctx *t : two)
      if (t && t->ext_bar) {
        (void)hipMemsetAsync(t->ext_bar, 0, 2 * sizeof(unsigned), c->stream);
        t->ext_bar_base = 0;
        t->ext_loop_off = 1;
      }
  }
  return POMGPU_OK;
}
extern "C" int pomgpu_sync(pomgpu_ctx *c) {
  if (!c) return POMGPU_EINVAL;
  side_join(c);
  HIPCHK(c, hipStreamSynchronize(c->stream));
  { const int rio = pomgpu_io_wait(c); if (rio) return rio; }
  return c->launch_err ? POMGPU_EHIP : POMGPU_OK;
}

extern "C" int pomgpu_set_con(pomgpu_ctx *c, const pom_blkcon *con, int lramp) {
  if (!c || !con) return POMGPU_EINVAL;
  if (c->wr_pending && con->dti2 != c->P.dti2) pomgpu_wr_materialize(c);
  c->con = *con;
  c->lramp = lramp;
  sync_scalars(c);
  return POMGPU_OK;
}
extern "C" int pomgpu_get_con(pomgpu_ctx *c, pom_blkcon *con) {
  if (!c || !con) return POMGPU_EINVAL;
  int rc = pull_err(c);
  if (rc) return rc;
  *con = c->con;
  return POMGPU_OK;
}
static int check_masks(pomgpu_ctx *c, const double *blk2d) {
  const int slots[3] = {P2_fsm, P2_dum, P2_dvm};
  for (int s = 0; s < 3; s++) {
    const double *m = blk2d + (size_t)slots[s] * c->P.n2;
    for (size_t n = 0; n < c->P.n2; n++)
      if (m[n] != 0. && m[n] != 1.) return fail(c, POMGPU_EINVAL, "mask array (blk2d slot %d) holds a value other than 0/1", slots[s]);
  }
  return POMGPU_OK;
}
static void refresh_coefs(pomgpu_ctx *c);
extern "C" int pomgpu_upload(pomgpu_ctx *c, const double *b1, const double *b2, const double *b3, const double *bd,
                             const pom_blkcon *con, int lramp) {
  if (!c) return POMGPU_EINVAL;
  KP &P = c->P;
  HIPCHK(c, hipSetDevice(c->device));
  ext_canonical(c);
  restore_materialize(c);
  c->wide.static_done = 0;
  early_invalidate(c);
  if (b2) { int rc = check_masks(c, b2); if (rc) return rc; }
  if (b1) HIPCHK(c, hipMemcpyAsync(P.b1, b1, sizeof(double) * POM_NBLK1D * P.kb, hipMemcpyHostToDevice, c->stream));
  if (b2) HIPCHK(c, hipMemcpyAsync(P.b2, b2, sizeof(double) * POM_NBLK2D * P.n2, hipMemcpyHostToDevice, c->stream));
  if (b3) {
    pomgpu_tau_touched(c, 0); pomgpu_tau_touched(c, 1);
#ifndef POMGPU_STORE_F32
    if (P.a3 == P.n3) HIPCHK(c, hipMemcpyAsync(P.b3, b3, sizeof(double) * POM_NBLK3D * P.n3, hipMemcpyHostToDevice, c->stream));
    else
#endif
    for (int n = 0; n < POM_NBLK3D; n++) {
      const int rc3 = copy3_h2d(c, SLOT3(c, n), b3 + (size_t)n * P.n3);
      if (rc3) return rc3;
#ifdef POMGPU_STORE_F32
      HIPCHK(c, hipStreamSynchronize(c->stream));
#endif
    }
  }
  if (bd) {
    const size_t nbd = P.bdoff[PB__count - 1] + (size_t)P.iml * P.kb;
    HIPCHK(c, hipMemcpyAsync(P.bd, bd, sizeof(double) * nbd, hipMemcpyHostToDevice, c->stream));
  }
  HIPCHK(c, hipStreamSynchronize(c->stream));
// ... 205 lines not shown
    const size_t sc[8] = {0, T.nbr[1] >= 0 ? ne : 0, 0, T.nbr[3] >= 0 ? nn : 0, 0, 0, 0, 0};
    const size_t rc[8] = {T.nbr[0] >= 0 ? ne : 0, 0, T.nbr[2] >= 0 ? nn : 0, 0, 0, 0, 0, 0};
    const bool side = rim_side(c);
    double *const *snd = side ? T.send2 : T.send, *const *rcv = side ? T.recv2 : T.recv;
    if (side) side_begin(c);
    launch_advct_edge(c, T.nbr[1] >= 0 ? snd[1] : NULL, T.nbr[3] >= 0 ? snd[3] : NULL);
    const int rcm = side ? pomgpu_tp_move_side(c, sc, rc) : pomgpu_tp_move(c, sc, rc);
    if (side) side_end(c, c->side_ev[SIDE_R1].ev);
    if (rcm) return;
    launch_advct_col(c, sum2d);
    if (side) (void)hipStreamWaitEvent(c->stream, c->side_ev[SIDE_R1].ev, 0);
    launch_advct_fix(c, T.nbr[0] >= 0 ? rcv[0] : NULL, T.nbr[2] >= 0 ? rcv[2] : NULL);
    if (sum2d) launch_advct_fix2d(c, T.nbr[0] >= 0, T.nbr[2] >= 0);
    if (!defer_xch) xch(c, 2, D3(c, advx), P.kb, D3(c, advy), P.kb);
    return;
  }
  launch_advct_a(c);
  xch(c, 2, P.s3[0], P.kbm1, P.s3[1], P.kbm1);
  launch_advct_b(c);
  xch(c, 2, D3(c, advx), P.kb, P.s3[4], P.kbm1);
  launch_advct_c(c);
  xch(c, 1, D3(c, advy), P.kb);
}
static void seq_rho_roundtrip(pomgpu_ctx *c, int defer_rt, int cols = 0) {
  if (defer_rt) {
    launch_roundtrip_level(c, D3(c, rho), D3(c, rmean), c->P.kb);
    c->rho_rt_pending = 1;
    c->rho_rt_cols = cols;
  } else {
    launch_roundtrip(c, D3(c, rho), D3(c, rmean), 0);
  }
}
static void seq_baropg(pomgpu_ctx *c, int sum2d = 0, int defer_rt = 0) {
  const int cols = launch_baropg(c, sum2d, (defer_rt && rt_one_tile(c)) ? c->rt_cols : NULL);
  seq_rho_roundtrip(c, defer_rt, cols);
}
static void seq_baropg_mcc(pomgpu_ctx *c, int sum2d = 0, int defer_rt = 0) {
  KP &P = c->P;
  if (c->order) {
    launch_order_pack(c, c->ord_send[0], c->ord_send[1]);
    c->order(c->order_user, c->ord_send[0], (P.kb + 1) * P.jml, c->ord_send[1], (P.kb + 1) * P.iml, c->ord_recv[0], c->ord_recv[1]);
  }
  launch_baropg_mcc(c, sum2d);
  seq_rho_roundtrip(c, defer_rt);
}
static void seq_advq(pomgpu_ctx *c, double *qb, double *q, double *qf, int pair, int zero_else) {
  KP &P = c->P;
  if (!c->exch) { launch_coef_eta(c); launch_advq_col(c, q, qb, qf, zero_else); return; }
  double *xf = P.s3[pair ? 2 : 0], *yf = P.s3[pair ? 3 : 1];
  launch_advq_flux(c, q, qb, xf, yf);
  xch(c, 2, xf, P.kbm1, yf, P.kbm1);
  launch_advq_step(c, q, qb, qf, xf, yf, zero_else);
}
static void seq_profq(pomgpu_ctx *c, int fuse_filter = 0, int with_w = 0, int store_ld = 1) {
  KP &P = c->P;
  launch_profq_bc(c);
  double *ufkb = LEV3(c, D3(c, uf), P.kb - 1);
  const int lines = c->exch && c->tp.on && !SW(c, PROD_FULL);
  if (lines) {
    launch_profq_prod(c, 1, c->rho_rt_pending);
    if (with_w) xch(c, 4, P.s2[4], 1, ufkb, 1, LEV3(c, P.s3[0], 1), P.kbm2, D3(c, w), P.kb);
    else xch(c, 3, P.s2[4], 1, ufkb, 1, LEV3(c, P.s3[0], 1), P.kbm2);
    launch_profq(c, 2, fuse_filter, c->rho_rt_pending);
    return;
  }
  if (with_w) xch(c, 3, P.s2[4], 1, ufkb, 1, D3(c, w), P.kb);
  else xch(c, 2, P.s2[4], 1, ufkb, 1);
  if (!c->exch) { launch_profq(c, 1, fuse_filter, c->rho_rt_pending, 0, -1, store_ld); return; }
  launch_profq_prod(c, 0, c->rho_rt_pending);
  xch(c, 1, LEV3(c, P.s3[0], 1), P.kbm2);
  launch_profq(c, 0, fuse_filter, c->rho_rt_pending);
}
static void seq_fb_fix(pomgpu_ctx *c, double *fb, const double *fclim) {
  launch_copy_kb(c, fb);
  launch_roundtrip(c, fb, fclim, 0);
}
static void seq_advt1(pomgpu_ctx *c, double *fb, double *f, const double *fclim, double *ff) {
  launch_advt1(c, fb, f, fclim, ff);
  seq_fb_fix(c, fb, fclim);
}
static void seq_advt2(pomgpu_ctx *c, double *fb, double *f, const double *fclim, double *ff, bool defer_roundtrip = false) {
  KP &P = c->P;
  if (P.nitera == 1) {
    launch_coef_eta(c);
    launch_advt2_rows(c, fb, f, fclim, ff);
  } else {
    launch_advt2_mass(c);
    const double *fbmem = fb, *eta = D2(c, etb);
    for (int itera = 1; itera <= P.nitera; itera++) {
      launch_advt2_step(c, fbmem, f, eta, ff, itera);
      xch(c, 1, ff, P.kbm1);
      launch_mask3(c, ff, D2(c, fsm));
      launch_smol(c, ff);
      eta = D2(c, etf);
      launch_copy3(c, P.s3[3], ff);
      fbmem = P.s3[3];
    }
    launch_advt2_diff(c, fb, fclim, ff);
  }
  xch(c, 1, ff, P.kbm1);
  if (defer_roundtrip) launch_copy_kb(c, fb);
  else seq_fb_fix(c, fb, fclim);
}
static int restore_prepare(pomgpu_ctx *c, double *fold_out, double *fnew_out) {
  const pom_blkcon &k = c->con;
  const double trst = 30.;
  const int irst = (int)(trst * 86400. / k.dti);
  const int ntime = (int)(k.time / trst);
  auto load = [&](int n) -> int {
    const int rfile = pomgpu_ff_has(c, 3), steady = rfile && pomgpu_ff_rate_steady(c);
    if (rfile) { const int rc = pomgpu_ff_rate_have(c, n); if (rc) return rc; }
    const double *tr, *sr;
    if (pomgpu_ff_has(c, 2)) {
      const int rc = pomgpu_ff_fetch_restore(c, n);
      if (rc) return rc;
      tr = c->rec_t[0]; sr = c->rec_s[0];
    } else {
      if (n < 1 || n > POMGPU_MAXREC || !c->rec_t[n])
        return fail(c, POMGPU_EINVAL, "restore_interior: record %d was not supplied (pomgpu_set_restore_record)", n);
      tr = c->rec_t[n]; sr = c->rec_s[n];
    }
// ... 70 lines not shown
  const char *what = side ? "exchange (side stream)" : "exchange";
  double *const *snd = side ? T.send2 : T.send, *const *rcv = side ? T.recv2 : T.recv;
  const size_t *cap = side ? T.cap2 : T.cap;
  size_t total = 0;
  for (int a = 0; a < count; a++) total += (size_t)nz[a];
  const size_t len[8] = {(size_t)P.jm, (size_t)P.jm, (size_t)P.im, (size_t)P.im, 1, 1, 1, 1};
  size_t cnt[8];
  for (int d = 0; d < 8; d++) {
    cnt[d] = T.nbr[d] >= 0 ? total * len[d] : 0;
    if (cnt[d] > cap[d]) return fail(c, POMGPU_EINVAL, "%s: %zu doubles exceed the staging buffer", what, cnt[d]);
  }
  if (launch_halo_pack8(c, dev, nz, count, snd)) return fail(c, POMGPU_EINVAL, "%s: bad array list", what);
  const int rc = side ? pomgpu_tp_move_side(c, cnt, cnt) : pomgpu_tp_move(c, cnt, cnt);
  if (rc) return rc;
  (void)launch_halo_unpack8(c, dev, nz, count, rcv);
  if (dev2) (void)launch_halo_unpack8(c, dev2, nz, count, rcv);
  return POMGPU_OK;
}
static int rim_round(pomgpu_ctx *c, side_round r, double *const *dev, const int *nz, int count, double *const *dev2 = NULL) {
  side_begin(c);
  const int rc = round8(c, 1, dev, nz, count, dev2);
  side_post(c, r);
  return rc;
}
static void early_invalidate(pomgpu_ctx *c) {
  if (c->early_started) { (void)hipStreamWaitEvent(c->stream, c->ev_early, 0); c->early_started = 0; }
}
int pomgpu_side_stream(pomgpu_ctx *c) {
  if (c->side) return 1;
  if (hipStreamCreateWithFlags(&c->side, hipStreamNonBlocking) != hipSuccess) { c->side = NULL; return 0; }
  bool ok = hipEventCreateWithFlags(&c->ev_fork, hipEventDisableTiming) == hipSuccess && hipEventCreateWithFlags(&c->ev_early, hipEventDisableTiming) == hipSuccess;
  for (auto &e : c->side_ev) ok = ok && hipEventCreateWithFlags(&e.ev, hipEventDisableTiming) == hipSuccess;
  if (!ok) {
    (void)hipStreamDestroy(c->side);
    c->side = NULL;
    return 0;
  }
#ifdef POMGPU_EMU
  emu_stream_defer(c->side);
#endif
  return 1;
}
#define NEED_RAW(c) if (!(c)) return POMGPU_EINVAL; if ((c)->broken) return POMGPU_EHIP; (void)hipSetDevice((c)->device)
static void wide_flush(pomgpu_ctx *c);
#define NEED_HOT(c) NEED_RAW(c); ext_canonical(c); wide_flush(c)
#define NEED(c) NEED_HOT(c); side_join(c); restore_materialize(c)

int pomgpu_materialize(pomgpu_ctx *c) {
  NEED(c);
  return POMGPU_OK;
}
void pomgpu_mirrors_written(pomgpu_ctx *c) {
  c->uvm_valid = 0;
  c->rho_rt_cols = 0;
  c->wide.static_done = 0;
  early_invalidate(c);
  refresh_coefs(c);
}
void pomgpu_cold_tail(pomgpu_ctx *c, void (*update_initial)(pomgpu_ctx *), void (*sums)(pomgpu_ctx *)) {
  launch_dens(c, D3(c, sclim), D3(c, tclim), D3(c, rmean));
  launch_dens(c, D3(c, sb), D3(c, tb), D3(c, rho));
  update_initial(c);
  if (c->con.npg == 2) seq_baropg_mcc(c); else seq_baropg(c);
  sums(c);
  pomgpu_tau_touched(c, 0); pomgpu_tau_touched(c, 1);
  pomgpu_mirrors_written(c);
}
extern "C" int pomgpu_get_time(pomgpu_ctx *c) {
  NEED_HOT(c);
  pom_blkcon &k = c->con;
  k.time = k.dti * (double)(float)k.iint / 86400. + k.time0;
  if (k.iint >= k.iswtch) k.iprint = (int)lround(k.prtd2 * 24. * 3600. / k.dti);
  if (c->lramp) { k.ramp = k.time / k.period; if (k.ramp > 1.) k.ramp = 1.; }
  else k.ramp = 1.;
  sync_scalars(c);
  return POMGPU_OK;
}
static int lateral_viscosity(pomgpu_ctx *c, int sum2d, int defer_rt = 0) {
  NEED_HOT(c);
  side_wait(c, SIDE_RTS);
  rho_materialize(c);
  KP &P = c->P;
  c->aam2d_done = 0;
  if (P.mode != 2) {
    const bool lib_x = c->tp.on && c->exch && !SW(c, ADVCT_SPLIT);
    auto pressure_gradient = [&]() {
      if (P.npg == 1) seq_baropg(c, sum2d, defer_rt);
      else if (P.npg == 2) seq_baropg_mcc(c, sum2d, defer_rt);
      else {
        fprintf(stderr, "\nError: invalid value for npg\n");
        c->con.error_status = 1;
      }
    };
    const bool pg_first = c->side_ev[SIDE_R8].pending != 0;
    if (pg_first) pressure_gradient();
    side_wait(c, SIDE_R8);
    const bool fuse = sum2d && aam_fused(c);
    if (!fuse) aam_canonical(c);
    seq_advct(c, sum2d, lib_x, fuse ? (c->aam_parity ? SLOT3(c, P3_aam) : c->aam_spare) : NULL);
    if (!pg_first) pressure_gradient();
    if (fuse) { c->aam_parity ^= 1; aam_buffers(c); c->aam2d_done = 1; }
    else launch_aam(c);
    if (lib_x && sum2d && rim_side(c)) {
      double *arr[3] = {D3(c, advx), D3(c, advy), D3(c, aam)};
      const int nz[3] = {P.kb, P.kb, P.kbm1};
      side_begin(c);
// ... 504 lines not shown
    n += 1;
  }
  for (int n = 0; n < ntr; n++) {
    const pomgpu_ctx::pomgpu_tracer &a = c->trc[n];
    if (a.q || a.lam != 0.) launch_tr_source(c, a.trf, a.trb, rt ? a.clim : NULL, a.q, a.lam);
  }
  {
    double *ptr[POMGPU_TRMAX];
    int nz[POMGPU_TRMAX];
    for (int n = 0; n < ntr; n++) { ptr[n] = c->trc[n].trf; nz[n] = P.kbm1; }
    xchv(c, ptr, nz, ntr);
  }
  side_wait(c, SIDE_RQ);
  for (int n = 0; n < ntr;) {
    const pomgpu_ctx::pomgpu_tracer &a = c->trc[n];
    const int nf = (pairs && n + 1 < ntr) ? 2 : 1;
    const pomgpu_ctx::pomgpu_tracer &b = c->trc[n + nf - 1];
    if (nf == 1 || !launch_proft2(c, a.trf, a.wsurf, a.surf, a.nbc, b.trf, b.wsurf, b.surf, b.nbc)) {
      launch_proft(c, a.trf, a.wsurf, a.surf, a.nbc);
      if (nf == 2) launch_proft(c, b.trf, b.wsurf, b.surf, b.nbc);
    }
    const TrEdge e[2] = {{a.trf, a.tr, a.bd[0], a.bd[1], a.bd[2], a.bd[3]}, {b.trf, b.tr, b.bd[0], b.bd[1], b.bd[2], b.bd[3]}};
    launch_tr_edges(c, e, nf);
    const TrUpd u[2] = {{a.trf, a.clim, a.tr, a.trb}, {b.trf, b.clim, b.tr, b.trb}};
    launch_tr_update(c, u, nf, rt);
    n += nf;
  }
  return POMGPU_OK;
}
static int wr_on_side(pomgpu_ctx *c, int with_kernel) {
  const KP &P = c->P;
  side_wait(c, SIDE_WR);
  side_begin(c);
  if (with_kernel) launch_realvertvl(c);
  double *arr[1] = {D3(c, wr)};
  const int nz[1] = {P.kbm1};
  const int rcw = round8(c, 1, arr, nz, 1);
  side_post(c, SIDE_WR);
  return rcw;
}
static int mode_internal(pomgpu_ctx *c, int defer_wr) {
  NEED_HOT(c);
  KP &P = c->P;
  const pom_blkcon &k = c->con;
  side_wait(c, SIDE_R2);
  side_wait(c, SIDE_R8);
  if ((k.iint != 1 || k.time0 != 0.) && k.mode != 2) {
    c->uvf_pending = 0;
    if (!(k.nadv == 2 && P.nitera == 1) || (c->exch && SW(c, ADVQ_EXCHANGE))) aam_canonical(c);
    struct UvmScope { pomgpu_ctx *c; ~UvmScope() { c->P.uvm = 0; c->uvm_valid = 0; } } uvm_scope{c};
    P.uvm = uvm_onload(c) ? 1 : 0;
    if (!P.uvm) launch_int_uvmean(c);
    const bool wf = w_fused(c);
    if (!wf) launch_vertvl(c, 1);
    const bool lib_x = c->tp.on && c->exch;
    const bool rimr = lib_x && rim_side(c) && !SW(c, RIM_RESULTS_MAIN) && !SW(c, ADVQ_EXCHANGE) && !SW(c, PROD_FULL);
    if (rimr) {
      double *aw[1] = {D3(c, w)};
      const int nw[1] = {P.kb};
      const int rcw = rim_round(c, SIDE_RW, aw, nw, 1);
      if (rcw) return rcw;
    }
    else if (!lib_x) xch(c, 1, D3(c, w), P.kb);
    launch_coef_eta(c, P.uvm);
    if (!c->exch || !SW(c, ADVQ_EXCHANGE)) {
      if (SW(c, ADVQ_SINGLE)) {
        launch_advq_col(c, D3(c, q2), D3(c, q2b), D3(c, uf), 1);
        launch_advq_col(c, D3(c, q2l), D3(c, q2lb), D3(c, vf), 1);
#if POMGPU_W_FUSE
      } else if (wf) {
        launch_advq2w_col(c, D3(c, q2), D3(c, q2b), D3(c, uf), D3(c, q2l), D3(c, q2lb), D3(c, vf), 1);
#endif
      } else {
        launch_advq2_col(c, D3(c, q2), D3(c, q2b), D3(c, uf), D3(c, q2l), D3(c, q2lb), D3(c, vf), 1);
      }
    } else {
      double *x0 = P.s3[0], *y0 = P.s3[1], *x1 = P.s3[2], *y1 = P.s3[3];
      launch_advq_flux(c, D3(c, q2), D3(c, q2b), x0, y0);
      launch_advq_flux(c, D3(c, q2l), D3(c, q2lb), x1, y1);
      xch(c, 4, x0, P.kbm1, y0, P.kbm1, x1, P.kbm1, y1, P.kbm1);
      launch_advq_step(c, D3(c, q2), D3(c, q2b), D3(c, uf), x0, y0, 1);
      launch_advq_step(c, D3(c, q2l), D3(c, q2lb), D3(c, vf), x1, y1, 1);
    }
    const int qfuse = !SW(c, QFILTER_SPLIT);
    if (rimr) {
      launch_profq_bc(c);
      launch_profq(c, 1, qfuse, c->rho_rt_pending, P.S ? 1 : 2, P.N ? P.jm : P.jmm1);
    } else {
      seq_profq(c, qfuse, lib_x, !(defer_wr && ld_on_demand(c) && !next_step_fetches_record(c)));
      xch(c, 2, LEV3(c, D3(c, uf), 1), P.kbm2, LEV3(c, D3(c, vf), 1), P.kbm2);
    }
    launch_bcond6_edges(c);
    if (qfuse) launch_q_filter_rim(c);
    else launch_q_filter(c, 1);
    if (rimr) {
      double *aq[9] = {D3(c, q2), D3(c, q2b), D3(c, q2l), D3(c, q2lb), D3(c, km), D3(c, kh), D3(c, kq), D3(c, l), D3(c, dtef)};
      const int nq[9] = {P.kb, P.kb, P.kb, P.kb, P.kb, P.kb, P.kb, P.kb, P.kb};
      const int rcq = rim_round(c, SIDE_RQ, aq, nq, 9);
      if (rcq) return rcq;
    }
    side_wait(c, SIDE_RW);
    if (k.mode != 4) {
      bool ts_flags = false;
      if (k.nadv == 1) {
        seq_advt1(c, D3(c, tb), D3(c, t), D3(c, tclim), D3(c, uf));
        seq_advt1(c, D3(c, sb), D3(c, s), D3(c, sclim), D3(c, vf));
      } else if (k.nadv == 2) {
        if (P.nitera == 1 && !SW(c, ADVT2_SINGLE)) {
          ts_flags = rt_one_tile(c);
          launch_advt2x2_col(c, D3(c, tb), D3(c, t), D3(c, tclim), D3(c, uf), D3(c, sb), D3(c, s), D3(c, sclim), D3(c, vf), ts_flags ? c->rt_words : NULL);
          if (!lib_x) xch(c, 1, D3(c, uf), P.kbm1);
          if (!lib_x) xch(c, 1, D3(c, vf), P.kbm1);
          launch_copy_kb(c, D3(c, tb), D3(c, sb));
        } else {
          seq_advt2(c, D3(c, tb), D3(c, t), D3(c, tclim), D3(c, uf), true);
          seq_advt2(c, D3(c, sb), D3(c, s), D3(c, sclim), D3(c, vf), true);
        }
      } else {
        return fail(c, POMGPU_EINVAL, "Error: invalid value for nadv");
      }
      const bool rts = rimr && k.nadv == 2 && P.nitera == 1 && !SW(c, ADVT2_SINGLE);
      if (!rts) xch(c, 2, D3(c, uf), rimr ? P.kb : P.kbm1, D3(c, vf), P.kbm1);
      if (!rts) side_wait(c, SIDE_RQ);
      if (!launch_proft2(c, D3(c, uf), D2(c, wtsurf), D2(c, tsurf), k.nbct, D3(c, vf), D2(c, wssurf), D2(c, ssurf), k.nbcs)) {
        launch_proft(c, D3(c, uf), D2(c, wtsurf), D2(c, tsurf), k.nbct);
        launch_proft(c, D3(c, vf), D2(c, wssurf), D2(c, ssurf), k.nbcs);
      }
      launch_bcond4_edges(c);
      double fold, fnew;
      int rc = restore_prepare(c, &fold, &fnew);
      if (rc) return rc;
      launch_ts_update(c, fold, fnew, k.nadv == 2, 0, ts_flags && !SW(c, RT_LOAD));
      c->rho_rt_pending = c->rho_rt_cols = 0;
      c->rst_pending = 1; c->rst_fold = fold; c->rst_fnew = fnew;
      if (rts) {
        double *at[5] = {D3(c, t), D3(c, tb), D3(c, s), D3(c, sb), D3(c, rho)};
        const int nt[5] = {P.kb, P.kb, P.kb, P.kb, P.kb};
        const int rct = rim_round(c, SIDE_RTS, at, nt, 5);
        if (rct) return rct;
      }
    }
    if (c->ntr) {
      const int rct = tracer_stage(c, lib_x);
      if (rct) return rct;
    }
    side_wait(c, SIDE_RQ);
    const bool fuse = uv_fused(c);
    if (pomgpu_reg_kb(c)) {
      launch_advuv_col(c);
      if (fuse) launch_profuv_filter_reg(c, c->uvb_bot[0], c->uvb_bot[1]);
      else launch_profuv_reg(c);
    } else {
      launch_advu_profu(c, 1, 1);
      launch_advv_profv(c, 1, 1);
    }
    if (!lib_x) xch(c, 2, D2(c, wubot), 1, D2(c, wvbot), 1);
    launch_bcondorl3(c);
    const bool rim78 = lib_x && rim_side(c);
    if (rim78) {
      const int top = P.kb - 1;
      double *a7[4] = {D2(c, wubot), D2(c, wvbot), D3(c, uf), D3(c, vf)}, *b7[4] = {D2(c, wubot), D2(c, wvbot), D3(c, u), D3(c, v)};
      const int n7[4] = {1, 1, P.kbm1, P.kbm1};
      side_begin(c);
      const int rc7 = round8(c, 1, a7, n7, 4, b7);
      side_end(c, c->side_ev[SIDE_R8].ev);
      launch_uv_filter(c, 1);
      double *a8[6] = {D3(c, ub), D3(c, vb), LEV3(c, D3(c, u), top), LEV3(c, D3(c, uf), top), LEV3(c, D3(c, v), top), LEV3(c, D3(c, vf), top)};
      const int n8[6] = {P.kb, P.kb, 1, 1, 1, 1};
      if (rc7) { side_begin(c); side_post(c, SIDE_R8); return rc7; }
      const int rc8 = rim_round(c, SIDE_R8, a8, n8, 6);
      if (rc8) return rc8;
    } else {
      if (lib_x) xch(c, 4, D2(c, wubot), 1, D2(c, wvbot), 1, D3(c, uf), P.kbm1, D3(c, vf), P.kbm1);
      else xch(c, 2, D3(c, uf), P.kbm1, D3(c, vf), P.kbm1);
      if (fuse) { launch_uv_filter_rim(c); c->uvf_pending = 1; }
      else launch_uv_filter(c);
      if (lib_x) {
        const int top = P.kb - 1;
        xch(c, 6, D3(c, ub), P.kb, D3(c, vb), P.kb, LEV3(c, D3(c, u), top), 1, LEV3(c, D3(c, uf), top), 1, LEV3(c, D3(c, v), top), 1, LEV3(c, D3(c, vf), top), 1);
      } else {
        xch(c, 6, D3(c, ub), P.kb, D3(c, u), P.kb, D3(c, uf), P.kb, D3(c, vb), P.kb, D3(c, v), P.kb, D3(c, vf), P.kb);
      }
    }
  }
  launch_int_tail(c);
// ... 479 lines not shown
  const int ph_ext = prof_phase_open(c);
  if (!ext_loop_all(c))
  for (int iext = 1; iext <= c->con.isplit; iext++) {
    if (ext_pair(c, iext)) { iext++; continue; }
    c->con.iext = iext;
    if ((rc = mode_external(c, 0))) return rc;
  }
  prof_phase_close(c, ph_ext, "phase_external");
  c->con.iext = c->con.isplit + 1;
  if ((rc = mode_internal(c, more_steps_follow))) return rc;
  if (c->mean_acc && (rc = mean_accumulate(c))) return rc;
  launch_check_velocity(c);
  prof_phase_close(c, ph_step, "phase_step");
  return POMGPU_OK;
}
extern "C" int pomgpu_run(pomgpu_ctx *c, int nsteps) {
  NEED_HOT(c);
  c->wr_deferred = 0;
  for (int n = 0; n < nsteps; n++) {
    c->con.iint += 1;
    int rc = advance(c, n + 1 < nsteps);
    if (rc) return rc;
  }
  return POMGPU_OK;
}

static int piece_move(pomgpu_ctx *c, double *dst, const double *src, size_t n) {
  if (dst == src || !n) return POMGPU_OK;
  const size_t shift = dst > src ? (size_t)(dst - src) : (size_t)(src - dst), chunk = shift < n ? shift : n;
  const size_t nch = (n + chunk - 1) / chunk;
  for (size_t q = 0; q < nch; q++) {
    const size_t m = dst > src ? nch - 1 - q : q;
    const size_t o = m * chunk, len = (o + chunk <= n ? chunk : n - o);
    HIPCHK(c, hipMemcpyAsync(dst + o, src + o, len * sizeof(double), hipMemcpyDeviceToDevice, c->stream));
  }
  return POMGPU_OK;
}
struct TuneLay { size_t f, a; };
static double *tune_piece(const pomgpu_ctx *c, const TuneLay &L, int i) {
  return c->tune_block + L.f + (i < POM_NBLK3D ? (size_t)i * L.a : (size_t)POM_NBLK3D * L.a + (size_t)(i - POM_NBLK3D) * c->P.n3);
}
static int tune_relayout(pomgpu_ctx *c, TuneLay to) {
  const int np = POM_NBLK3D + POMGPU_NSCR3;
  auto one_way = [&](const TuneLay &from, const TuneLay &dst_) -> int {
    const bool up = dst_.f >= from.f && dst_.a >= from.a;
    for (int q = 0; q < np; q++) {
      const int i = up ? np - 1 - q : q;
      const int rc = piece_move(c, tune_piece(c, dst_, i), tune_piece(c, from, i), c->P.n3);
      if (rc) return rc;
    }
    return POMGPU_OK;
  };
  aam_canonical(c);
  const TuneLay cur = {c->tune_front, c->P.a3};
  int rc = POMGPU_OK;
  if ((to.f >= cur.f && to.a >= cur.a) || (to.f <= cur.f && to.a <= cur.a)) rc = one_way(cur, to);
  else {
    const TuneLay mid = {to.f > cur.f ? to.f : cur.f, to.a > cur.a ? to.a : cur.a};
    rc = one_way(cur, mid);
    if (!rc) rc = one_way(mid, to);
  }
  if (rc) return rc;
  KP &P = c->P;
  c->tune_front = to.f;
  P.a3 = to.a;
  P.b3 = c->tune_block + to.f;
  for (int n = 0; n < POMGPU_NSCR3; n++) P.s3[n] = P.b3 + (size_t)POM_NBLK3D * P.a3 + (size_t)n * P.n3;
  aam_buffers(c);
  return POMGPU_OK;
}
extern "C" int pomgpu_tune_placement(pomgpu_ctx *c, int steps, int max_try, double *ms_out, long *front_mib_out, long *pad_mib_out, int *ntried, int *kept) {
  NEED(c);
  if (ntried) *ntried = 0;
  if (kept) *kept = 0;
  if (c->mean_acc)
    return fail(c, POMGPU_EINVAL, "tune_placement: the time-mean output is on and the trial steps would count -- tune first, switch the mean on afterwards");
  if (c->ntr)
    return fail(c, POMGPU_EINVAL, "tune_placement: passive tracers are registered and the trial steps would move them -- tune first, register tracers afterwards");
#ifdef POMGPU_EMU
  (void)steps; (void)max_try; (void)ms_out; (void)front_mib_out; (void)pad_mib_out;
  return POMGPU_OK;
#else
  KP &P = c->P;
  if ((c->flags & POMGPU_CTX_2D) || !P.b3 || steps < 1 || max_try < 1) return fail(c, POMGPU_EINVAL, "tune_placement: a context with 3-D arrays, steps >= 1, max_try >= 1");
  if (c->dev3_handed)
    return fail(c, POMGPU_EINVAL, "tune_placement: pomgpu_device_3d has handed out addresses of the 3-D arrays, which this call would leave dangling -- tune first, take addresses afterwards");
  if (P.n3 * sizeof(double) < ((size_t)64 << 20) && !SW(c, TUNE_FORCE)) return POMGPU_OK;
  const size_t unit = 2 * P.n3;
  size_t pad1 = P.n3 * sizeof(double) >= ((size_t)512 << 20) ? ((size_t)256 << 20) / sizeof(double) : (P.n3 / 4 + 8191) / 8192 * 8192;
  HIPCHK(c, hipStreamSynchronize(c->stream));
  if (c->side) HIPCHK(c, hipStreamSynchronize(c->side));
  if (!c->tune_block) {
    size_t fre = 0, tot = 0;
    HIPCHK(c, hipMemGetInfo(&fre, &tot));
    const size_t a0 = P.a3;
    size_t amax = a0 + pad1;
    auto need = [&](int kmax, size_t am) { return ((size_t)kmax * unit + (size_t)POM_NBLK3D * am + (size_t)POMGPU_NSCR3 * P.n3) * sizeof(double) + ((size_t)2 << 30); };
    int kmax = max_try > 12 ? 30 : 10;
    while (kmax > 0 && need(kmax, amax) > fre) kmax--;
    if (kmax < 1) { amax = a0; kmax = 10; while (kmax > 0 && need(kmax, amax) > fre) kmax--; }
    if (kmax < 1) return POMGPU_OK;
    double *blk = NULL;
    if (hipMalloc((void **)&blk, need(kmax, amax) - ((size_t)2 << 30)) != hipSuccess) { (void)hipGetLastError(); return POMGPU_OK; }
    for (int n = 0; n < POM_NBLK3D; n++)
      HIPCHK(c, hipMemcpyAsync(blk + (size_t)n * a0, P.b3 + (size_t)n * a0, P.n3 * sizeof(double), hipMemcpyDeviceToDevice, c->stream));
    for (int n = 0; n < POMGPU_NSCR3; n++)
// ... 209 lines not shown
```

### extpom_amd/csrc/pomgpu_internal.hpp

```cpp
#pragma once
#include <hip/hip_runtime.h>
#include <stddef.h>
#include <stdlib.h>
#include "pom_layout.h"

#ifndef COL_ROWS
#define COL_ROWS 4
#endif
#ifndef COL_WX
#define COL_WX 1
#endif
#define POMGPU_NSCR3 8
#define POMGPU_NSCR2 8
#define POMGPU_NCOEF2 25
#define POMGPU_MAXREC 8
#define POMGPU_TRMAX 8
#define POMGPU_KBMAX 128
#define POMGPU_CTX_2D 1
#define POMGPU_DERR_VELOCITY 1
#define POMGPU_DERR_BARRIER 2
#define POMGPU_NGEN 7

struct KP {
  int im, jm, kb, imm1, jmm1, kbm1, kbm2, iml, jml;
// ... 19 lines not shown
  int uvm;
  const double *aamc;
};
enum pomgpu_x2 { X2_ua, X2_va, X2_d, X2_el, X2_elb, X2_uab, X2_vab };

#ifdef POMGPU_STORE_F32
typedef float pomgpu_st;
#else
typedef double pomgpu_st;
#endif
#define POMGPU_ST_BYTES ((unsigned)sizeof(pomgpu_st))
#if defined(POMGPU_COMPUTE_F32) && !defined(POMGPU_STORE_F32)
#error "POMGPU_COMPUTE_F32 is the fp32-arithmetic variant of the fp32-storage build: it needs POMGPU_STORE_F32"
#endif
#ifdef POMGPU_COMPUTE_F32
typedef float pomgpu_ct;
#else
typedef double pomgpu_ct;
#endif
#define CT(x) ((pomgpu_ct)(x))
#ifdef POMGPU_COMPUTE_F32
#define POMGPU_W_FUSE 0
#else
#define POMGPU_W_FUSE 1
#endif
#ifdef POMGPU_COMPUTE_F32
#define POMGPU_UVM_ONLOAD 0
#else
#define POMGPU_UVM_ONLOAD 1
#endif
#ifdef POMGPU_COMPUTE_F32
#define POMGPU_AAM_FUSE 0
#else
#define POMGPU_AAM_FUSE 1
#endif
#ifdef POMGPU_STORE_F32
struct Ref3 {
  pomgpu_st *p;
  __device__ __forceinline__ operator double() const { return (double)*p; }
  __device__ __forceinline__ const Ref3 &operator=(double v) const { *p = (pomgpu_st)v; return *this; }
  __device__ __forceinline__ const Ref3 &operator=(const Ref3 &o) const { *p = *o.p; return *this; }
};
#define REF3(ptr, idx) (Ref3{(pomgpu_st *)(ptr) + (idx)})
#else
#define REF3(ptr, idx) ((ptr)[(idx)])
#endif

#define IX2(i, j) ((size_t)((j)-1) * (size_t)P.iml + (size_t)((i)-1))
#define IX3(i, j, k) ((size_t)((k)-1) * P.n2 + IX2(i, j))
#if !defined(POMGPU_EMU) && !defined(POMGPU_F1_GLOBAL)
typedef const double __attribute__((address_space(4))) *pomgpu_cptr;
#define F1(name, k) ((pomgpu_cptr)(size_t)P.b1)[(size_t)P1_##name * P.kb + ((k)-1)]
#define R1(name, k) ((pomgpu_cptr)(size_t)P.r1)[(size_t)P1_##name * P.kb + ((k)-1)]
#else
#define F1(name, k) P.b1[(size_t)P1_##name * P.kb + ((k)-1)]
#define R1(name, k) P.r1[(size_t)P1_##name * P.kb + ((k)-1)]
#endif
#define F2(name, i, j) P.b2[(size_t)P2_##name * P.n2 + IX2(i, j)]
#define F3(name, i, j, k) REF3(P.b3 + (size_t)P3_##name * P.a3, IX3(i, j, k))
#define A2(name) (P.b2 + (size_t)P2_##name * P.n2)
#define A3(name) (P.b3 + (size_t)P3_##name * P.a3)
#define G3(p, i, j, k) REF3(p, IX3(i, j, k))
#define G2(p, i, j) (p)[IX2(i, j)]

enum pom_bdry_slot_dev {
#define POMGPU_BD_(name, shape) PB_##name,
  POM_BDRY(POMGPU_BD_)
#undef POMGPU_BD_
  PB__count
};
#define BD1(name, a) P.bd[P.bdoff[PB_##name] + (size_t)((a)-1)]
#define BDJ(name, a, k) P.bd[P.bdoff[PB_##name] + (size_t)((k)-1) * P.jml + (size_t)((a)-1)]
#define BDI(name, a, k) P.bd[P.bdoff[PB_##name] + (size_t)((k)-1) * P.iml + (size_t)((a)-1)]

__device__ __forceinline__ double sq(double x) { return x * x; }

enum pomgpu_coef2 {
  C2_HSX, C2_HSY,
  C2_DYSX, C2_DXSX,
  C2_DXSY, C2_DYSY,
  C2_CMX, C2_CMY,
  C2_HEA, C2_HFA,
  C2_DTSX, C2_DTSY,
  C2_DT4,
  C2_DX4, C2_DY4,
  C2_CVA, C2_CVB,
  C2_R2DXSX, C2_R2DYSY,
  C2_RDX, C2_RDY,
  C2_USUM, C2_VSUM,
  C2_UCOR, C2_VCOR,
  C2__count
};
static_assert(C2__count <= POMGPU_NCOEF2, "raise POMGPU_NCOEF2");
#define K2(name, i, j) P.c2[C2_##name][IX2(i, j)]

#define UVM_MARK 0x7ff8c0de5eed0001ULL
struct UvmC { double s, c; bool on; };
__device__ __forceinline__ UvmC uvm_none() { UvmC m; m.s = 0.; m.c = 0.; m.on = false; return m; }
template <int V> __device__ __forceinline__ UvmC uvm_of(const KP &P, int i, int j) {
  UvmC m = uvm_none();
#if POMGPU_UVM_ONLOAD
  if (P.uvm) {
    m.s = V ? K2(VSUM, i, j) : K2(USUM, i, j);
    m.c = V ? K2(VCOR, i, j) : K2(UCOR, i, j);
    unsigned long long b;
    __builtin_memcpy(&b, &m.c, sizeof b);
    m.on = b != UVM_MARK;
  }
#endif
  return m;
}
__device__ __forceinline__ double uvm_fix(double x, const UvmC &m, bool lev = true) {
#if POMGPU_UVM_ONLOAD
  const double y = (double)(pomgpu_st)((x - m.s) + m.c);
  return (m.on && lev) ? y : x;
#else
  return x;
#endif
}
__device__ __forceinline__ float uvm_fix(float x, const UvmC &, bool = true) { return x; }
template <int V> __device__ __forceinline__ double uvm_ld(const KP &P, int i, int j, int k) {
  const double x = V ? (double)F3(v, i, j, k) : (double)F3(u, i, j, k);
  return uvm_fix(x, uvm_of<V>(P, i, j), k <= P.kbm1);
}

#ifndef POMGPU_EMU
__device__ __forceinline__ double wave_up1(double x) {
  int lo = __double2loint(x), hi = __double2hiint(x);
// ... 247 lines not shown
    const int rem__ = m__ - s__ * rpx__ * st__, w__ = s__ < nfull__ ? st__ : (wlast__ > 0 ? wlast__ : 1); \
    byl__ = rem__ / w__; bxg__ = s__ * st__ + rem__ % w__;                                \
    if (bxg__ >= nbx__ || byl__ >= rpx__) return;                                         \
  } else {                                                                                \
    byl__ = m__ / nbx__; bxg__ = m__ % nbx__;                                             \
    if (byl__ >= rpx__) return;                                                           \
  }
#define HALO_XCD_DECODE HALO_XCD_DECODE_R(COL_ROWS)
#define HALO_XCD_DECODE_R(ROWS__)                                                         \
  const int g__ = (int)(blockIdx.x * blockDim.x + threadIdx.x);                           \
  const int L__ = g__ >> 6, nwx__ = (P.iml + 61) / 62, nbx__ = (nwx__ + COL_WX - 1) / COL_WX; \
  const int nby__ = (P.jml + ROWS__ - 1) / ROWS__;                                        \
  const int rpx__ = (nby__ + 7) / 8, m__ = L__ >> 3;                                      \
  int by__, bxg__;                                                                        \
  if (P.g_lin && 10 * nby__ < 72 * rpx__) {                                               \
    const int x__ = L__ & 7, T__ = nby__ * nbx__;                                         \
    const int c0__ = (int)(((long)x__ * T__) >> 3), c1__ = (int)(((long)(x__ + 1) * T__) >> 3); \
    const int t__ = c0__ + m__;                                                           \
    if (t__ >= c1__) return;                                                              \
    const int st__ = P.g_strip > 0 ? P.g_strip : nbx__, per__ = st__ * nby__, s__ = t__ / per__; \
    const int rem__ = t__ - s__ * per__, w__ = (s__ + 1) * st__ <= nbx__ ? st__ : nbx__ - s__ * st__; \
    by__ = rem__ / w__; bxg__ = s__ * st__ + rem__ % w__;                                 \
  } else {                                                                                \
    int byl__;                                                                            \
    HALO_XCD_ORDER                                                                        \
    by__ = (L__ & 7) * rpx__ + byl__;                                                     \
    if (by__ >= nby__) return;                                                            \
  }                                                                                       \
  const int lane = g__ & 63;                                                              \
  const int i0 = (bxg__ * COL_WX + (int)threadIdx.y % COL_WX) * 62 + lane;                \
  const int j = by__ * ROWS__ + (int)threadIdx.y / COL_WX + 1;
static inline dim3 grid1_halo_r(const KP &P, int rows) {
  const int nwx = (P.iml + 61) / 62, nbx = (nwx + COL_WX - 1) / COL_WX, nby = (P.jml + rows - 1) / rows, rpx = (nby + 7) / 8;
  if (P.g_lin && 10 * nby < 72 * rpx) return dim3((unsigned)(8 * ((nby * nbx + 7) / 8)), 1, 1);
  return dim3((unsigned)(8 * rpx * nbx), 1, 1);
}
static inline dim3 grid1_halo(const KP &P) { return grid1_halo_r(P, COL_ROWS); }
static inline dim3 blk_col_r(int rows) { return dim3(64, rows * COL_WX, 1); }
static inline dim3 blk_col() { return dim3(64, COL_ROWS * COL_WX, 1); }
#define HALO_COL (int)(((blockIdx.x * blockDim.x + threadIdx.x) >> 6) * 62 + ((blockIdx.x * blockDim.x + threadIdx.x) & 63))
static inline dim3 grid2_halo(const KP &P) { return dim3((P.iml + 61) / 62, (P.jml + 3) / 4, 1); }

#define TID_I (int)(blockIdx.x * blockDim.x + threadIdx.x + 1)
#define TID_J (int)(blockIdx.y * blockDim.y + threadIdx.y + 1)
#define TID_K (int)(blockIdx.z * blockDim.z + threadIdx.z + 1)

#define POMGPU_SWITCHES(X)                                                                                                    \
  X(THOMAS_SCRATCH) X(NO_PAIR) X(EXT_SPLIT) X(ADVAVE_SEPARATE) X(EXT_RIM_KERNEL) X(EXT_LOOP) X(EXT_NOMARCH) X(EXT_MARCH)      \
  X(EXT_ROWS) X(EXT_NOPAIR) X(EXT_PAIR) X(EXT_ROWS2) X(EXT_TWO_SETS) X(EXT_AREAS_LOAD) X(BAROPG_CELLS) X(VERTVL_CELLS)        \
  X(NO_LIN) X(ADVQ_SINGLE) X(ADVT2_SINGLE) X(REALVERTVL_CELLS) X(RHO_ROUNDTRIP) X(TAU_ARRAYS) X(PROFQ_ROWS8) X(PROFQ_ROWS2)    \
  X(PROFQ_NOPACE) X(COL_STRIP) X(BAND_BYTES) X(PAD3) X(IO_SYNC) X(ADVCT_SPLIT) X(ADVQ_EXCHANGE) X(PROD_FULL) X(QFILTER_SPLIT) \
  X(NO_OVERLAP) X(NO_SIDE_COMM) X(WR_MAIN) X(WIDE_W) X(WIDE_FULL) X(DEBUG_ALLOC) X(TEST_SPLIT_FAIL_RANK)  \
  X(WR_NODEFER) X(EXT_RING_FIRST) X(TUNE_FORCE) X(RIM_MAIN) X(RIM_RESULTS_MAIN) X(SUM2D_OFF) X(ADVCT_ROWS4) X(ADVCT_ROWS8) \
  X(IO_CHUNK_KB) X(UV_NOFUSE) X(W_NOFUSE) X(UVMEAN_PASS) X(PROFT_TWIN) X(LD_EAGER) X(TR_NOPAIR) X(RT_LOAD) X(AAM_NOFUSE)
enum pomgpu_sw {
#define POMGPU_SW_(name) SW_##name,
  POMGPU_SWITCHES(POMGPU_SW_)
#undef POMGPU_SW_
  SW__count
};
struct pomgpu_switches {
  unsigned char on[SW__count];
  long val[SW__count];
};
static const char *const POMGPU_SW_NAMES[SW__count] = {
#define POMGPU_SW_(name) #name,
  POMGPU_SWITCHES(POMGPU_SW_)
#undef POMGPU_SW_
};
static inline void pomgpu_switches_read(pomgpu_switches &s) {
  for (int n = 0; n < SW__count; n++) {
    char var[64] = "POMGPU_";
    size_t k = 7;
    for (const char *q = POMGPU_SW_NAMES[n]; *q && k + 1 < sizeof var; q++) var[k++] = *q;
    var[k] = 0;
    const char *e = getenv(var);
    s.on[n] = e ? 1 : 0;
    s.val[n] = e ? atol(e) : 0;
  }
}
static inline unsigned pomgpu_switches_collective_digest(const pomgpu_switches &s) {
  static const int coll[] = {SW_ADVCT_SPLIT, SW_ADVQ_EXCHANGE, SW_PROD_FULL, SW_QFILTER_SPLIT, SW_NO_OVERLAP,
                             SW_NO_SIDE_COMM, SW_WR_MAIN, SW_WIDE_W, SW_WIDE_FULL, SW_EXT_SPLIT, SW_ADVAVE_SEPARATE, SW_WR_NODEFER, SW_RIM_MAIN, SW_ADVT2_SINGLE, SW_RIM_RESULTS_MAIN, SW_SUM2D_OFF};
  unsigned h = 2166136261u;
  for (size_t n = 0; n < sizeof coll / sizeof coll[0]; n++) {
    h = (h ^ (unsigned)(s.on[coll[n]] ? 1 + coll[n] : 0)) * 16777619u;
    h = (h ^ (unsigned)s.val[coll[n]]) * 16777619u;
  }
  return h & 0x3fffffffu;
}
#define SW(c, NAME) ((c)->sw.on[SW_##NAME] != 0)
#define SWV(c, NAME) ((c)->sw.val[SW_##NAME])
struct ProfEntry { const char *name; long launches; double ms; };
struct pomgpu_ctx;

static const int POMGPU_OPP[8] = {1, 0, 3, 2, 7, 6, 5, 4};
struct pomgpu_transport {
  int on;
  int nbr[8];
  void (*fn)(void *, const double *const *, const size_t *, double *const *, const size_t *);
  void *user;
  void *rccl;
  double *send[8], *recv[8];
  size_t cap[8];
  double *send2[8], *recv2[8];
  size_t cap2[8];
  int fn_ordered;
// ... 14 lines not shown
  size_t e_scount[8], e_rcount[8], l_scount[8], l_rcount[8];
  int split;
  int pending;
  int static_done;
};
enum side_round { SIDE_WR, SIDE_R1, SIDE_R2, SIDE_R8, SIDE_RW, SIDE_RQ, SIDE_RTS, SIDE__count };

struct pomgpu_ctx {
  KP P;
  pomgpu_switches sw;
  int device;
  hipStream_t stream;
  bool own_stream;
  hipStream_t cur, side;
  hipEvent_t ev_fork, ev_early;
  struct { hipEvent_t ev; int pending; } side_ev[SIDE__count];
  int early_started;
  double *tune_block;
  size_t tune_front;
  int tune_kmax;
  size_t tune_a0, tune_amax;
  int dev3_handed;
  int broken;
  int wr_deferred;
  pom_blkcon con;
  int lramp;
  double *rec_t[POMGPU_MAXREC + 1], *rec_s[POMGPU_MAXREC + 1];
  const double *host2, *host3;
  void (*exch)(void *, double *const *, const int *, int);
  void *exch_user;
  void (*order)(void *, const double *, int, const double *, int, double *, double *);
  void *order_user;
  double *ord_send[2], *ord_recv[2];
  double *alt2[POMGPU_NGEN];
  double *alt3[POMGPU_NGEN];
  int ext_parity;
  int ext_deferred;
  int tau_known[2];
  double tau_val[2];
  double *rec_tau[POMGPU_MAXREC + 1];
  long tau_id[2], tau_gen;
  int tau_same, rate_in_f, tau_handed;
  int rho_rt_pending;
  unsigned long long *rt_words;
  unsigned *rt_cols;
  int rho_rt_cols;
  int rst_pending;
  double rst_fold, rst_fnew;
  int wr_pending;
  int uvf_pending;
  int uvm_valid;
  double *aam_spare;
  int aam_parity, aam_spare_failed, aam2d_done;
  double *uvb_bot[2];
  int wr_eager;
  double *d_vel;
  int *d_err;
  int *d_areas;
  int areas_checked;
  double *d_stats;
  double *frc_dev[3][4][2];
  int frc_n[3][4];
  double *lat_dev[4];
  int lat_n[4];
  int frc_on, lat_on;
  double *wat_dev[4];
  int wat_n[4];
  int wat_on;
  int sss_on;
  bool prof_on;
  ProfEntry prof[96];
  int nprof;
  void *prof_state;
  pomgpu_transport tp;
  pomgpu_wide wide;
  pomgpu_ctx *parent;
  int flags;
  unsigned *ext_bar;
  unsigned ext_bar_base;
  int ext_loop_off;
  void *io_job;
  int z_init, z_clim;
  int z_lbry;
  int lbry_sides;
  void *frc_files;
  int launch_err;
  double *mean_acc;
  size_t mean_off[9];
  int mean_count;
  int ntr;
  struct pomgpu_tracer { double *trb, *tr, *trf, *clim, *q, *wsurf, *surf, *bd[4]; int nbc; double lam; } trc[POMGPU_TRMAX];
  double *tr_zero3;
  double *trmean_acc;
  size_t trmean_stride;
  int trmean_count;
  double *d_trstats;
  char err[512];
};
static inline bool pomgpu_reg_kb(const pomgpu_ctx *c) { return c->P.kb >= 6 && c->P.kb <= 64 && !SW(c, THOMAS_SCRATCH); }

int pomgpu_prof_slot(pomgpu_ctx *c, const char *name);
void pomgpu_prof_pre(pomgpu_ctx *c);
void pomgpu_prof_post(pomgpu_ctx *c, int slot);
int pomgpu_fail(pomgpu_ctx *c, int code, const char *fmt, ...);
void pomgpu_launch_check(pomgpu_ctx *c, const char *name);

// ... 12 lines not shown
    if (_s >= 0) pomgpu_prof_pre(c);                                             \
    hipLaunchKernelGGL(kern, grid, block, 0, (c)->cur, __VA_ARGS__);             \
    pomgpu_launch_check((c), name);                                              \
    if (_s >= 0) pomgpu_prof_post((c), _s);                                      \
  } while (0)

static inline dim3 blk2() { return dim3(64, 4, 1); }
static inline dim3 grid2(const KP &P) { return dim3((P.iml + 63) / 64, (P.jml + 3) / 4, 1); }
static inline dim3 grid3(const KP &P, int nz) { return dim3((P.iml + 63) / 64, (P.jml + 3) / 4, nz); }
static inline dim3 gridm(const KP &P) {
  const long nbands = (P.jml + P.g_rb - 1) / P.g_rb;
  const long rounds = (nbands + 7) / 8;
  return dim3((unsigned)(8 * rounds * P.kb * P.g_bpl), 1, 1);
}
static inline void set_band_geometry(KP &P, const pomgpu_switches &sw) {
  long budget = 3L << 20;
  const bool e = sw.on[SW_BAND_BYTES] != 0;
  if (e && sw.val[SW_BAND_BYTES] >= 1024) budget = sw.val[SW_BAND_BYTES];
  long rows = budget / ((long)P.iml * 8 * 24);
  rows = (rows / 4) * 4;
  if (rows < 4) rows = 4;
  if (rows > ((P.jml + 3) / 4) * 4) rows = ((P.jml + 3) / 4) * 4;
  P.g_rb = (int)rows;
  P.g_nbx = (P.iml + 63) / 64;
  P.g_bpl = P.g_nbx * (int)(rows / 4);
  const int nbx = ((P.iml + 61) / 62 + COL_WX - 1) / COL_WX;
  const int nstr = (nbx + 11) / 12;
  P.g_strip = nbx >= 20 ? (nbx + nstr - 1) / nstr : 0;
  if (sw.on[SW_COL_STRIP]) P.g_strip = (int)sw.val[SW_COL_STRIP];
  P.g_lin = sw.on[SW_NO_LIN] ? 0 : 1;
  if (!e) {
    long best = -1, bslots = 0;
    for (long r = 4; r <= rows; r += 4) {
      const long nb = (P.jml + r - 1) / r, slots = (nb + 7) / 8 * 8 * r;
      if (best < 0 || slots < bslots || (slots == bslots && r > best)) { best = r; bslots = slots; }
    }
    P.g_rb = (int)best;
    P.g_bpl = P.g_nbx * (int)(best / 4);
  }
}

void launch_advave_a(pomgpu_ctx *c);
void launch_advave_b(pomgpu_ctx *c);
void launch_advave_c(pomgpu_ctx *c);
void launch_advave_fused(pomgpu_ctx *c);
void launch_advct_col(pomgpu_ctx *c, int sum2d, double *aam_w = NULL);
void launch_advct_edge(pomgpu_ctx *c, double *to_e, double *to_n);
void launch_advct_fix(pomgpu_ctx *c, const double *from_w, const double *from_s);
void launch_advct_fix2d(pomgpu_ctx *c, int west, int south);
void launch_advt2x2_col(pomgpu_ctx *c, const double *tb, const double *t, const double *tc, double *tf, const double *sb, const double *s_,
                        const double *sc, double *sf, unsigned long long *rtf = NULL);
void launch_advq2_col(pomgpu_ctx *c, const double *q, const double *qb, double *qf, const double *ql, const double *qlb, double *qlf, int zero_else);
#if POMGPU_W_FUSE
void launch_advq2w_col(pomgpu_ctx *c, const double *q, const double *qb, double *qf, const double *ql, const double *qlb, double *qlf, int zero_else);
#endif
void launch_advuv_col(pomgpu_ctx *c);
int launch_profuv_reg(pomgpu_ctx *c);
void launch_profuv_filter_reg(pomgpu_ctx *c, double *ubk, double *vbk);
void launch_uv_filter_rim(pomgpu_ctx *c);
void launch_uvf_copy(pomgpu_ctx *c);
void launch_advave_m2a(pomgpu_ctx *c);
void launch_advave_m2b(pomgpu_ctx *c);
void launch_vint(pomgpu_ctx *c, int only_aam, int ghost = 0);
void launch_modeint_tail(pomgpu_ctx *c);
void launch_ext_elf(pomgpu_ctx *c);
void launch_ext_uvaf(pomgpu_ctx *c, int interior);
void launch_ext_update(pomgpu_ctx *c);
void launch_ext_step(pomgpu_ctx *c, const KP &Q, int store_f, int fuse_adv);
void launch_check_areas(pomgpu_ctx *c);
int launch_ext_loop(pomgpu_ctx *c, const KP &Q, int first, int last);
int launch_ext_pair_ok(const pomgpu_switches &sw, const KP &Q);
int launch_ext_pair(pomgpu_ctx *c, const KP &Q, double *const *T, int store_f2);
void launch_copy2(pomgpu_ctx *c, double *dst, const double *src);
void launch_lat(pomgpu_ctx *c, int phase, const double *rec, double fold, double fnew);
void launch_frc_load(pomgpu_ctx *c, const double *ra, const double *rb, double *xf, double *yf);
void launch_frc_interp(pomgpu_ctx *c, double fold, double fnew, double *x, const double *xb, const double *xf, double *y, const double *yb,
                       const double *yf);
void launch_frc_load1(pomgpu_ctx *c, const double *ra, double *xf, double *xb);
void launch_frc_interp1(pomgpu_ctx *c, double fold, double fnew, double *x, const double *xb, const double *xf);
void launch_int_tail(pomgpu_ctx *c);
void launch_bcond1(pomgpu_ctx *c);
void launch_advct_a(pomgpu_ctx *c);
void launch_advct_b(pomgpu_ctx *c);
void launch_advct_c(pomgpu_ctx *c);
void launch_aam(pomgpu_ctx *c);
void launch_roundtrip(pomgpu_ctx *c, double *a, const double *b, int fix_kb);
void launch_roundtrip_level(pomgpu_ctx *c, double *a, const double *b, int k);
void launch_advq_flux(pomgpu_ctx *c, const double *q, const double *qb, double *xf, double *yf);
void launch_advq_step(pomgpu_ctx *c, const double *q, const double *qb, double *qf, const double *xf, const double *yf, int zero_else);
void launch_q_filter(pomgpu_ctx *c, int mask);
void launch_q_filter_rim(pomgpu_ctx *c);
void launch_mask_q(pomgpu_ctx *c);
void launch_advt1(pomgpu_ctx *c, double *fb, double *f, const double *fclim, double *ff);
void launch_copy_kb(pomgpu_ctx *c, double *f, double *g = NULL);
void launch_advt2_mass(pomgpu_ctx *c);
void launch_advt2_step(pomgpu_ctx *c, const double *fbmem, const double *f, const double *eta, double *ff, int itera);
void launch_mask3(pomgpu_ctx *c, double *a, const double *m2);
void launch_smol(pomgpu_ctx *c, const double *ff);
void launch_copy3(pomgpu_ctx *c, double *dst, const double *src);
void launch_aam_copy(pomgpu_ctx *c, double *dst, const double *src);
void launch_advt2_diff(pomgpu_ctx *c, const double *fb, const double *fc, double *ff);
void launch_ts_update(pomgpu_ctx *c, double fold, double fnew, int rt, int store_rst, int rt_flags = 0);
void launch_restore_fields(pomgpu_ctx *c, double fold, double fnew);
void launch_mask_ts(pomgpu_ctx *c);
struct TrUpd { const double *ff, *fc; double *f, *fb; };
void launch_tr_update(pomgpu_ctx *c, const TrUpd *u, int nf, int rt);
void launch_mask_uv(pomgpu_ctx *c);
void launch_mask_w(pomgpu_ctx *c);
void launch_restore(pomgpu_ctx *c, double fold, double fnew);
void launch_restore_shift(pomgpu_ctx *c);
void launch_restore_load(pomgpu_ctx *c, const double *tr, const double *sr, double tau, const double *taur = NULL, int fill_tau = 1);
void launch_dens(pomgpu_ctx *c, const double *si, const double *ti, double *rhoo);
void launch_realvertvl(pomgpu_ctx *c, int etf_is_et = 0);
int launch_baropg(pomgpu_ctx *c, int sum2d, unsigned *rtcol = NULL);
void launch_baropg_mcc(pomgpu_ctx *c, int sum2d);
void launch_order_pack(pomgpu_ctx *c, double *send_e, double *send_n);
void launch_int_uvmean(pomgpu_ctx *c);
void launch_vertvl(pomgpu_ctx *c, int mask);
void launch_profq_bc(pomgpu_ctx *c);
void launch_profq_prod(pomgpu_ctx *c, int lines_only, int rho_rt = 0);
void launch_profq(pomgpu_ctx *c, int fuse_prod, int fuse_filter, int rho_rt = 0, int jfirst = 0, int jlast = -1, int store_ld = 1);
void launch_proft(pomgpu_ctx *c, double *f, const double *wfsurf, const double *fsurf, int nbc);
int launch_proft2(pomgpu_ctx *c, double *f0, const double *wfsurf0, const double *fsurf0, int nbc0, double *f1, const double *wfsurf1, const double *fsurf1, int nbc1);
void launch_advu_profu(pomgpu_ctx *c, int do_adv, int do_prof);
void launch_advv_profv(pomgpu_ctx *c, int do_adv, int do_prof);
void launch_uv_filter(pomgpu_ctx *c, int own = 0);
void launch_coef_static(pomgpu_ctx *c);
void launch_coef_dt(pomgpu_ctx *c);
void launch_coef_eta(pomgpu_ctx *c, int uvm = 0);
void launch_advt2_rows(pomgpu_ctx *c, const double *fb, const double *f, const double *fc, double *ff);
void launch_advq_col(pomgpu_ctx *c, const double *q, const double *qb, double *qf, int zero_else);
void launch_bcond4_edges(pomgpu_ctx *c);
void launch_bcond6_edges(pomgpu_ctx *c);
void launch_bcondorl3(pomgpu_ctx *c);
struct TrEdge { double *ff; const double *f, *be, *bw, *bn, *bs; };
void launch_tr_edges(pomgpu_ctx *c, const TrEdge *e, int nf);
void launch_tr_source(pomgpu_ctx *c, double *ff, const double *fb, const double *fc, const double *q, double lam);
int launch_halo_pack(pomgpu_ctx *c, double *const *dev, const int *nz, int count, int dir, double *to_lo, double *to_hi);
int launch_halo_pack8(pomgpu_ctx *c, double *const *dev, const int *nz, int count, double *const *to);
int launch_halo_unpack8(pomgpu_ctx *c, double *const *dev, const int *nz, int count, const double *const *from);
int launch_halo_unpack(pomgpu_ctx *c, double *const *dev, const int *nz, int count, int dir, const double *from_lo, const double *from_hi);
void launch_rect_jobs(pomgpu_ctx *c, const RectJob *jobs_dev, int njobs, int max_ni, int max_nj);
int pomgpu_tp_move(pomgpu_ctx *c, const size_t *scount, const size_t *rcount);
int pomgpu_tp_move_ptr(pomgpu_ctx *c, const double *const *send, const size_t *scount, double *const *recv, const size_t *rcount);
int pomgpu_tp_setup(pomgpu_ctx *c, const int *nbr8);
int pomgpu_tp_rccl(pomgpu_ctx *c, const void *id128, int rank, int nranks, const char *librccl_path);
void pomgpu_tp_free(pomgpu_ctx *c);
int pomgpu_tp_reserve(pomgpu_ctx *c, const size_t *need);
int pomgpu_tp_reserve2(pomgpu_ctx *c, const size_t *need);
void pomgpu_wr_materialize(pomgpu_ctx *c);
int pomgpu_materialize(pomgpu_ctx *c);
void pomgpu_mirrors_written(pomgpu_ctx *c);
void pomgpu_cold_tail(pomgpu_ctx *c, void (*update_initial)(pomgpu_ctx *), void (*sums)(pomgpu_ctx *));
int pomgpu_side_stream(pomgpu_ctx *c);
int pomgpu_tp_side_ok(pomgpu_ctx *c);
int pomgpu_tp_move_side(pomgpu_ctx *c, const size_t *scount, const size_t *rcount);
int pomgpu_ff_has(pomgpu_ctx *c, int src);
int pomgpu_ff_fetch_surface(pomgpu_ctx *c, int kind, int n);
int pomgpu_ff_fetch_lateral(pomgpu_ctx *c, int n);
int pomgpu_ff_fetch_restore(pomgpu_ctx *c, int n);
int pomgpu_ff_has_water(pomgpu_ctx *c);
int pomgpu_ff_fetch_water(pomgpu_ctx *c, int n);
int pomgpu_ff_rate_steady(pomgpu_ctx *c);
int pomgpu_ff_rate_have(pomgpu_ctx *c, int n);
int pomgpu_ff_fetch_rate(pomgpu_ctx *c, int n);
static inline void pomgpu_tau_touched(pomgpu_ctx *c, int which) {
  c->tau_known[which] = 0; c->tau_id[which] = 0; c->tau_same = 0;
  if (which) c->rate_in_f = 0;
}
void pomgpu_ff_free(pomgpu_ctx *c);
int launch_ztosig(pomgpu_ctx *c, double *t, const double *zs, int ks, const double *src);
void launch_ztosig_edges(pomgpu_ctx *c, double *t);
int launch_ztosig_line(pomgpu_ctx *c, int edge, const double *zs, int ks, const double *src, double *out);
void launch_mean_accum(pomgpu_ctx *c, const double *const *x);
// ... 8 lines not shown
```

Baseline: 5.033 billion.

## Hand off sound speed and shear from upstream kernels into profq

The T/S update kernel now computes the sound-speed term per cell and stores it in a new buffer. profq then reads one value instead of loading t and s and recomputing the sqrt-heavy formula. The fused advq column kernel, which already holds the corrected velocities, writes the shear-squared term into scratch, so profq (new FP==3 mode) skips its four velocity loads. The per-level z reciprocal term is precomputed into r1 at setup. This trades an extra 3-D buffer and extra stores upstream, plus validity tracking that must be invalidated on constant or layout changes, for fewer loads and less arithmetic in profq.

```diff
diff --git a/extpom_amd/csrc/k_adv.hip b/extpom_amd/csrc/k_adv.hip
--- a/extpom_amd/csrc/k_adv.hip
+++ b/extpom_amd/csrc/k_adv.hip
@@ -398,14 +398,14 @@
 }
 
 __device__ __forceinline__ double dens_point(const KP &P, double si, double ti, int i, int j, int k);
-template <int TAU> __device__ __forceinline__ void c_ts_update(const KP &P, const int i, const int j, const int k, double fold, double fnew, int rt, int store_rst, double tau_b, double tau_f, const unsigned long long *rtf);
-template <int TAU> __global__ void k_ts_update(KP P, double fold, double fnew, int rt, int store_rst, double tau_b, double tau_f, const unsigned long long *rtf) {
-  MARCH3(c_ts_update<TAU>(P, i, j, k, fold, fnew, rt, store_rst, tau_b, tau_f, rtf))
-}
-__global__ void k_ts_update_same(KP P, double fold, double fnew, int rt, int store_rst, const unsigned long long *rtf) {
-  MARCH3(c_ts_update<2>(P, i, j, k, fold, fnew, rt, store_rst, 0., 0., rtf))
-}
-template <int TAU> __device__ __forceinline__ void c_ts_update(const KP &P, const int i, const int j, const int k, double fold, double fnew, int rt, int store_rst, double tau_b, double tau_f, const unsigned long long *rtf) {
+template <int TAU> __device__ __forceinline__ void c_ts_update(const KP &P, const int i, const int j, const int k, double fold, double fnew, int rt, int store_rst, double tau_b, double tau_f, const unsigned long long *rtf, double *cc);
+template <int TAU> __global__ void k_ts_update(KP P, double fold, double fnew, int rt, int store_rst, double tau_b, double tau_f, const unsigned long long *rtf, double *cc) {
+  MARCH3(c_ts_update<TAU>(P, i, j, k, fold, fnew, rt, store_rst, tau_b, tau_f, rtf, cc))
+}
+__global__ void k_ts_update_same(KP P, double fold, double fnew, int rt, int store_rst, const unsigned long long *rtf, double *cc) {
+  MARCH3(c_ts_update<2>(P, i, j, k, fold, fnew, rt, store_rst, 0., 0., rtf, cc))
+}
+template <int TAU> __device__ __forceinline__ void c_ts_update(const KP &P, const int i, const int j, const int k, double fold, double fnew, int rt, int store_rst, double tau_b, double tau_f, const unsigned long long *rtf, double *cc) {
   const bool act = (i <= P.im && j <= P.jm), lev = (k <= P.kbm1);
   const pomgpu_ct m = F2(fsm, i, j);
   pomgpu_ct uf = F3(uf, i, j, k), vf = F3(vf, i, j, k);
@@ -451,6 +451,11 @@
   F3(s, i, j, k) = sn;
   F3(sb, i, j, k) = sbn;
   if (lev && act) F3(rho, i, j, k) = dens_point(P, sn, tn, i, j, k);
+#ifndef POMGPU_COMPUTE_F32
+  if (cc && lev && act) cc[IX3(i, j, k)] = profq_cc_v(P, (double)(pomgpu_st)tn, (double)(pomgpu_st)sn, h_(i, j), k);
+#else
+  (void)cc;
+#endif
 }
 template <int NF> struct TrUpds { TrUpd u[NF]; };
 template <int NF> __device__ __forceinline__ void c_tr_update(const KP &P, const int i, const int j, const int k, const TrUpds<NF> &A, int rt) {
@@ -882,18 +887,18 @@
 void launch_copy3(pomgpu_ctx *c, double *dst, const double *src) { LAUNCH(c, k_copy3, gridm(c->P), blk2(), c->P, dst, src); }
 void launch_aam_copy(pomgpu_ctx *c, double *dst, const double *src) { LAUNCH(c, k_aam_copy, gridm(c->P), blk2(), c->P, dst, src); }
 void launch_advt2_diff(pomgpu_ctx *c, const double *fb, const double *fc, double *ff) { LAUNCH(c, k_advt2_diff, gridm(c->P), blk2(), c->P, fb, fc, ff); }
-void launch_ts_update(pomgpu_ctx *c, double fold, double fnew, int rt, int store_rst, int rt_flags) {
+void launch_ts_update(pomgpu_ctx *c, double fold, double fnew, int rt, int store_rst, int rt_flags, double *cc) {
   const unsigned long long *rtf = (rt && rt_flags) ? c->rt_words : NULL;
   if (rtf && c->prof_on) {
     const int s = pomgpu_prof_slot(c, "ts_rt_flags");
     if (s >= 0) (c->parent ? c->parent : c)->prof[s].launches++;
   }
   if (c->tau_known[0] && c->tau_known[1] && !c->tau_handed && !SW(c, TAU_ARRAYS))
-    LAUNCHN(c, "k_ts_update", (k_ts_update<1>), gridm(c->P), blk2(), c->P, fold, fnew, rt, store_rst, c->tau_val[0], c->tau_val[1], rtf);
+    LAUNCHN(c, "k_ts_update", (k_ts_update<1>), gridm(c->P), blk2(), c->P, fold, fnew, rt, store_rst, c->tau_val[0], c->tau_val[1], rtf, cc);
   else if (c->tau_same && !c->tau_handed && !SW(c, TAU_ARRAYS))
-    LAUNCH(c, k_ts_update_same, gridm(c->P), blk2(), c->P, fold, fnew, rt, store_rst, rtf);
+    LAUNCH(c, k_ts_update_same, gridm(c->P), blk2(), c->P, fold, fnew, rt, store_rst, rtf, cc);
   else
-    LAUNCHN(c, "k_ts_update", (k_ts_update<0>), gridm(c->P), blk2(), c->P, fold, fnew, rt, store_rst, 0., 0., rtf);
+    LAUNCHN(c, "k_ts_update", (k_ts_update<0>), gridm(c->P), blk2(), c->P, fold, fnew, rt, store_rst, 0., 0., rtf, cc);
 }
 void launch_restore_fields(pomgpu_ctx *c, double fold, double fnew) { LAUNCH(c, k_restore_fields, gridm(c->P), blk2(), c->P, fold, fnew); }
 void launch_mask_ts(pomgpu_ctx *c) { LAUNCH(c, k_mask_ts, gridm(c->P), blk2(), c->P); }
diff --git a/extpom_amd/csrc/k_tile.hip b/extpom_amd/csrc/k_tile.hip
--- a/extpom_amd/csrc/k_tile.hip
+++ b/extpom_amd/csrc/k_tile.hip
@@ -23,6 +23,10 @@
   K2(RDY, i, j) = 1.0 / F2(dy, i, j);
   if (j == 1)
     for (int n = i - 1; n < POM_NBLK1D * P.kb; n += P.iml) P.r1[n] = 1.0 / P.b1[n];
+  if (j == 1)
+    for (int k = i; k <= P.kb; k += P.iml)
+      P.r1[(size_t)POM_NBLK1D * P.kb + (k - 1)] = 1. / fabs(P.b1[(size_t)P1_z * P.kb + (k - 1)] - P.b1[(size_t)P1_z * P.kb]) +
+                                                  1. / fabs(P.b1[(size_t)P1_z * P.kb + (k - 1)] - P.b1[(size_t)P1_z * P.kb + (P.kb - 1)]);
 }
 __global__ void k_coef_dt(KP P) {
   const int i = TID_I, j = TID_J;
@@ -233,8 +237,9 @@
   x = x - divi(CT(.25) * (am_hi_k + am_lo_k + am_hi_m + am_lo_m) * c.hs * (qb_hi - qb_lo) * c.msk, c.den);
   return CT(.5) * c.ds_num * x;
 }
-template <int NF, bool WF = false, bool UM = false>
+template <int NF, bool WF = false, bool UM = false, bool SH = false>
 __global__ void __launch_bounds__(64 * LDS_ROWS) k_advq_col(KP P, QFields A, int zero_else) {
+  static_assert(!SH || (WF && UM), "the shear hand-off rides on the march that holds the corrected u_e");
   constexpr int NS = 2 * NF + 2, NH = ROWSHARE_SLOTS(NS), AM = 2 * NF, VV = 2 * NF + 1;
   typedef LevQa<NF, WF ? 1 : 2> Lev;
   HALO_XCD_DECODE_R(LDS_ROWS)
@@ -270,6 +275,9 @@
   const unsigned oc = BOFF2(i, jc), lvb = LVB;
   const unsigned ost = in ? oc : ((zero_else && icol) ? oc : BOFF_NONE);
   const unsigned ostw = in ? oc : BOFF_NONE;
+  constexpr unsigned SHS = 8 / POMGPU_ST_BYTES;
+  const unsigned osh = in ? oc * SHS : BOFF_NONE;
+  const BufA bsh = buf2_of(P.s3[0], P.n3);
 #ifndef POMGPU_EMU
   __shared__ pomgpu_ct slab[2][NS][ROWSHARE_ROWS][64];
 #else
@@ -339,6 +347,10 @@
       w_c = CT((pomgpu_st)wst);
     } else {
       w_c = cur.o[1];
+    }
+    if constexpr (SH) {
+      const double shr = sq((double)u_c - (double)u_m + (double)ue_c - (double)ue_m) + sq((double)v_c - (double)v_m + (double)v_n - (double)vn_m);
+      bst2(bsh, (L >= 2 && L <= kbm1) ? osh : BOFF_NONE, (unsigned)WAVE_UNIFORM(L - 1) * lvb * SHS, shr);
     }
     const int k = L - 1;
     InvDc dz2; dz2.b = dz2.y = 0.;
@@ -815,9 +827,10 @@
   LAUNCHN(c, "k_advq2_col", (k_advq_col<2>), grid1_halo_r(c->P, LDS_ROWS), blk_col_r(LDS_ROWS), c->P, A, zero_else);
 }
 #if POMGPU_W_FUSE
-void launch_advq2w_col(pomgpu_ctx *c, const double *q, const double *qb, double *qf, const double *ql, const double *qlb, double *qlf, int zero_else) {
+void launch_advq2w_col(pomgpu_ctx *c, const double *q, const double *qb, double *qf, const double *ql, const double *qlb, double *qlf, int zero_else, int shear) {
   QFields A; A.q[0] = q; A.qb[0] = qb; A.qf[0] = qf; A.q[1] = ql; A.qb[1] = qlb; A.qf[1] = qlf;
 #if POMGPU_UVM_ONLOAD
+  if (c->P.uvm && shear) { LAUNCHN(c, "k_advq2_col", (k_advq_col<2, true, true, true>), grid1_halo_r(c->P, LDS_ROWS), blk_col_r(LDS_ROWS), c->P, A, zero_else); return; }
   if (c->P.uvm) { LAUNCHN(c, "k_advq2_col", (k_advq_col<2, true, true>), grid1_halo_r(c->P, LDS_ROWS), blk_col_r(LDS_ROWS), c->P, A, zero_else); return; }
 #endif
   LAUNCHN(c, "k_advq2_col", (k_advq_col<2, true>), grid1_halo_r(c->P, LDS_ROWS), blk_col_r(LDS_ROWS), c->P, A, zero_else);
diff --git a/extpom_amd/csrc/k_vert.hip b/extpom_amd/csrc/k_vert.hip
--- a/extpom_amd/csrc/k_vert.hip
+++ b/extpom_amd/csrc/k_vert.hip
@@ -386,14 +386,6 @@
   cc = cc / sqrt((1. - .01642 * p / cc) * (1. - 0.40 * p / sq(cc)));
   return cc;
 }
-__device__ __forceinline__ double profq_cc_v(const KP &P, double t, double s_, double hij, int k) {
-  const double tp = t + P.tbias;
-  const double sp = s_ + P.sbias;
-  const double p = P.grav * P.rhoref * (-F1(zz, k) * hij) * 1.e-4;
-  double cc = 1449.1 + .00821 * p + 4.55 * tp - .045 * sq(tp) + 1.34 * (sp - 35.0);
-  cc = cc / sqrt((1. - .01642 * p / cc) * (1. - 0.40 * p / sq(cc)));
-  return cc;
-}
 __device__ __forceinline__ double profq_rho(const KP &P, int i, int j, int k, int rho_rt) {
   const double r = F3(rho, i, j, k);
   if (!rho_rt) return r;
@@ -464,8 +456,8 @@
 #ifndef PROFQ_BIG
 #define PROFQ_BIG 8
 #endif
-template <int FP, int FF, int ROWS, int LD = 1>
-__global__ void __launch_bounds__(64 * ROWS) k_profq(KP P, int rho_rt_pace, int jfirst, int jlast, const unsigned *rtcol) {
+template <int FP, int FF, int ROWS, int LD = 1, int CC = 0>
+__global__ void __launch_bounds__(64 * ROWS) k_profq(KP P, int rho_rt_pace, int jfirst, int jlast, const unsigned *rtcol, const double *cc) {
 #ifndef POMGPU_EMU
   constexpr int KL = ROWS >= 8 ? PROFQ_KL : (PROFQ_KL < 9 ? PROFQ_KL : 9);
   __shared__ double evec[2 * KL][ROWS][64];
@@ -481,7 +473,6 @@
   const double utau2 = G2(P.s2[4], i, j);
   const double l0 = surfl * utau2 / P.grav;
   const double umol2 = 2. * P.umol;
-  const double z1 = F1(z, 1), zkb = F1(z, kb);
   const double coef4 = 18. * a1 * a1 + 9. * a1 * a2, coef5 = 9. * a1 * a2;
   const double coef1 = a2 * (1. - 6. * a1 / b1 * 1.), coef2 = 3. * a2 * b2 / 1. + 18. * a1 * a2,
                coef3 = a1 * (1. - 3. * c1 - 6. * a1 / b1 * 1.);
@@ -520,13 +511,17 @@
 #define bl BUF3(A3(l))
 #define bdt BUF3(A3(dtef))
 #define bpr BUF3(P.s3[0])
+#define bsh buf2_of(P.s3[0], P.n3)
+#define bcc buf2_of(cc, P.n3)
 #define be1 BUF3(P.s3[4])
 #define be2 BUF3(P.s3[5])
   const unsigned oc = BOFF2(i, j), oe = BOFF2(ie, j), on = BOFF2(i, jn), lvb = LVB;
+  constexpr unsigned CCS = 8 / POMGPU_ST_BYTES;
+  const unsigned occ = oc * CCS;
+  const unsigned o_pr = (FP == 3) ? (pin ? occ : BOFF_NONE) : ((FP == 0 || (FP == 2 && !pin)) ? oc : BOFF_NONE);
   const unsigned o_k = repl ? BOFF_NONE : oc;
   const unsigned o_abs = ffil ? BOFF_NONE : oc;
   const unsigned o_fil = ffil ? oc : BOFF_NONE, o_uv = ffil ? BOFF_NONE : oc;
-  const unsigned o_pr = (FP == 0 || (FP == 2 && !pin)) ? oc : BOFF_NONE;
   unsigned o_rm = rho_rt ? oc : BOFF_NONE;
   if (rho_rt_pace & 4) o_rm = (rho_rt && rtcol[(size_t)(j - 1) * P.iml + (i - 1)]) ? oc : BOFF_NONE;
 #ifdef PROFQ_OLDWALK
@@ -543,14 +538,16 @@
 #ifdef PROFQ_OLDWALK
   auto lev = [&](LevQ &L, int k) {
     const unsigned lv = (unsigned)WAVE_UNIFORM(k - 1) * lvb;
-    L.t = bld(bt, oc, lv); L.s = bld(bs_, oc, lv); L.rho = bld(brho, oc, lv); L.rm = bld(BUF3(A3(rmean)), o_rm, lv);
+    if (CC) { L.t = bld2(bcc, occ, lv * CCS); L.s = 0.; }
+    else { L.t = bld(bt, oc, lv); L.s = bld(bs_, oc, lv); }
+    L.rho = bld(brho, oc, lv); L.rm = bld(BUF3(A3(rmean)), o_rm, lv);
     L.q2b = bld(bq2b, oc, lv); L.q2lb = bld(bq2lb, oc, lv); L.q2 = bld(bq2, oc, lv);
     L.km = bld(bkm, oc, lv); L.kh = bld(bkh, oc, lv);
     L.uf = bld(buf, oc, lv); L.vf = bld(bvf, oc, lv);
-    if (FP) { L.uc = bld(bu, oc, lv); L.ue = bld(bu, oe, lv); L.vc = bld(bv, oc, lv); L.vn = bld(bv, on, lv); }
+    if (FP == 1 || FP == 2) { L.uc = bld(bu, oc, lv); L.ue = bld(bu, oe, lv); L.vc = bld(bv, oc, lv); L.vn = bld(bv, on, lv); }
     else L.uc = L.ue = L.vc = L.vn = 0.;
     L.kq1 = bld(bkq, oc, (unsigned)WAVE_UNIFORM(k < kb ? k : kb - 1) * lvb);
-    L.prod = (FP != 1) ? bld(bpr, o_pr, lv) : 0.;
+    L.prod = (FP == 3) ? bld2(bsh, o_pr, lv * CCS) : ((FP != 1) ? bld(bpr, o_pr, lv) : 0.);
   };
   auto step = [&](const int k, const LevQ &cur, LevQ &nxt) {
     lev(nxt, k + 1 <= kb ? k + 1 : kb);
@@ -558,11 +555,11 @@
     const unsigned lv = (unsigned)WAVE_UNIFORM(k - 1) * lvb;
     const double kqp = cur.kq1;
     double cck = 0., rhok = 0.;
-    if (k <= kbm1) { cck = profq_cc_v(P, cur.t, cur.s, hij, k); rhok = (o_rm != BOFF_NONE) ? (cur.rho - cur.rm) + cur.rm : cur.rho; }
+    if (k <= kbm1) { cck = CC ? cur.t : profq_cc_v(P, cur.t, cur.s, hij, k); rhok = (o_rm != BOFF_NONE) ? (cur.rho - cur.rm) + cur.rm : cur.rho; }
     double q2b = cur.q2b;
     double l, gh = 0.;
     double uck = 0., uek = 0., vck = 0., vnk = 0., bg = 0.;
-    if (pin && k <= kbm1) { uck = uvm_fix(cur.uc, m_uc); uek = uvm_fix(cur.ue, m_ue); vck = uvm_fix(cur.vc, m_vc); vnk = uvm_fix(cur.vn, m_vn); }
+    if (FP != 3 && pin && k <= kbm1) { uck = uvm_fix(cur.uc, m_uc); uek = uvm_fix(cur.ue, m_ue); vck = uvm_fix(cur.vc, m_vc); vnk = uvm_fix(cur.vn, m_vn); }
     double q2lb = 0.;
     if (mid) {
       q2b = fabs(q2b);
@@ -579,7 +576,7 @@
     if (LD) bst(bl, oc, lv, l);
     const double dtef1 = sqrt(fabs(q2b)) * 1. / (b1 * l + P.small_);
     double dtef2 = dtef1;
-    if (mid) dtef2 = dtef1 * (1. + e2 * sq(divi((1. / fabs(F1(z, k) - z1) + 1. / fabs(F1(z, k) - zkb)) * l, dhk)));
+    if (mid) dtef2 = dtef1 * (1. + e2 * sq(divi(RQ1(k) * l, dhk)));
     if (LD) bst(bdt, oc, lv, dtef2);
     if (mid) {
       const double a = -P.dti2 * (kqp + kqc + umol2) * .5 / (F1(dzz, k - 1) * F1(dz, k) * dh * dh);
@@ -590,7 +587,8 @@
       } else if (pin) {
         const double sef = 1., shiw = 0.;
         const double km = cur.km;
-        pr = km * .25 * sef * (sq(uck - ucm + uek - uem) + sq(vck - vcm + vnk - vnm)) / sq(F1(dzz, k - 1) * dh) - shiw * km * bg;
+        const double shr = (FP == 3) ? cur.prod : sq(uck - ucm + uek - uem) + sq(vck - vcm + vnk - vnm);
+        pr = km * .25 * sef * shr / sq(F1(dzz, k - 1) * dh) - shiw * km * bg;
         pr = pr + cur.kh * bg;
       } else {
         pr = 0.;
@@ -662,14 +660,16 @@
   enum { PH_1, PH_2, PH_LDS, PH_MEM, PH_KBM1, PH_KB };
   auto lev = [&](LevQ &L, int k) {
     const unsigned lv = (unsigned)WAVE_UNIFORM(k - 1) * lvb;
-    L.t = bld(bt, oc, lv); L.s = bld(bs_, oc, lv); L.rho = bld(brho, oc, lv); L.rm = bld(BUF3(A3(rmean)), o_rm, lv);
+    if (CC) { L.t = bld2(bcc, occ, lv * CCS); L.s = 0.; }
+    else { L.t = bld(bt, oc, lv); L.s = bld(bs_, oc, lv); }
+    L.rho = bld(brho, oc, lv); L.rm = bld(BUF3(A3(rmean)), o_rm, lv);
     L.q2b = bld(bq2b, oc, lv); L.q2lb = bld(bq2lb, oc, lv); L.q2 = bld(bq2, oc, lv);
     L.km = bld(bkm, oc, lv); L.kh = bld(bkh, oc, lv);
     L.uf = bld(buf, oc, lv); L.vf = bld(bvf, oc, lv);
-    if (FP) { L.uc = bld(bu, oc, lv); L.ue = bld(bu, oe, lv); L.vc = bld(bv, oc, lv); L.vn = bld(bv, on, lv); }
+    if (FP == 1 || FP == 2) { L.uc = bld(bu, oc, lv); L.ue = bld(bu, oe, lv); L.vc = bld(bv, oc, lv); L.vn = bld(bv, on, lv); }
     else L.uc = L.ue = L.vc = L.vn = 0.;
     L.kq1 = bld(bkq, oc, (unsigned)WAVE_UNIFORM(k < kb ? k : kb - 1) * lvb);
-    L.prod = (FP != 1) ? bld(bpr, o_pr, lv) : 0.;
+    L.prod = (FP == 3) ? bld2(bsh, o_pr, lv * CCS) : ((FP != 1) ? bld(bpr, o_pr, lv) : 0.);
   };
   auto step = [&](auto ph, const int k, const LevQ &cur, LevQ &nxt) {
     constexpr int PH = decltype(ph)::value;
@@ -678,11 +678,11 @@
     const unsigned lv = (unsigned)WAVE_UNIFORM(k - 1) * lvb;
     const double kqp = cur.kq1;
     double cck = 0., rhok = 0.;
-    if (PH != PH_KB) { cck = profq_cc_v(P, cur.t, cur.s, hij, k); rhok = (o_rm != BOFF_NONE) ? (cur.rho - cur.rm) + cur.rm : cur.rho; }
+    if (PH != PH_KB) { cck = CC ? cur.t : profq_cc_v(P, cur.t, cur.s, hij, k); rhok = (o_rm != BOFF_NONE) ? (cur.rho - cur.rm) + cur.rm : cur.rho; }
     double q2b = cur.q2b;
     double l, gh = 0.;
     double uck = 0., uek = 0., vck = 0., vnk = 0., bg = 0.;
-    if (PH != PH_KB) {
+    if (PH != PH_KB && FP != 3) {
       uck = pin ? uvm_fix(cur.uc, m_uc) : 0.; uek = pin ? uvm_fix(cur.ue, m_ue) : 0.;
       vck = pin ? uvm_fix(cur.vc, m_vc) : 0.; vnk = pin ? uvm_fix(cur.vn, m_vn) : 0.;
     }
@@ -703,7 +703,7 @@
     if (LD) bst(bl, oc, lv, l);
     const double dtef1 = sqrt(fabs(q2b)) * 1. / (b1 * l + P.small_);
     double dtef2 = dtef1;
-    if (mid) dtef2 = dtef1 * (1. + e2 * sq(divi((1. / fabs(F1(z, k) - z1) + 1. / fabs(F1(z, k) - zkb)) * l, dhk)));
+    if (mid) dtef2 = dtef1 * (1. + e2 * sq(divi(RQ1(k) * l, dhk)));
     if (LD) bst(bdt, oc, lv, dtef2);
     if (mid) {
       const double a = -P.dti2 * (kqp + kqc + umol2) * .5 / (F1(dzz, k - 1) * F1(dz, k) * dh * dh);
@@ -714,7 +714,8 @@
       } else {
         const double sef = 1., shiw = 0.;
         const double km = cur.km;
-        pr = km * .25 * sef * (sq(uck - ucm + uek - uem) + sq(vck - vcm + vnk - vnm)) / sq(F1(dzz, k - 1) * dh) - shiw * km * bg;
+        const double shr = (FP == 3) ? cur.prod : sq(uck - ucm + uek - uem) + sq(vck - vcm + vnk - vnm);
+        pr = km * .25 * sef * shr / sq(F1(dzz, k - 1) * dh) - shiw * km * bg;
         pr = pr + cur.kh * bg;
         pr = pin ? pr : (FP == 2 ? cur.prod : 0.);
       }
@@ -1686,29 +1687,54 @@
   const int len = P.im > P.jm ? P.im : P.jm;
   LAUNCH(c, k_profq_prod_lines, dim3((len + 63) / 64, 8, P.kb), dim3(64, 1, 1), c->P, rho_rt);
 }
-void launch_profq(pomgpu_ctx *c, int fuse_prod, int fuse_filter, int rho_rt, int jfirst, int jlast, int store_ld) {
+void launch_profq(pomgpu_ctx *c, int fuse_prod, int fuse_filter, int rho_rt, int jfirst, int jlast, int store_ld, const double *cc) {
   if (jlast < jfirst) { jfirst = 1; jlast = c->P.jml; }
-  const int ld = store_ld || fuse_prod != 1 || !fuse_filter;
+  const int ld = store_ld || (fuse_prod != 1 && fuse_prod != 3) || !fuse_filter;
   if (ld && c->prof_on) {
     const int s = pomgpu_prof_slot(c, "profq_ld_store");
     if (s >= 0) (c->parent ? c->parent : c)->prof[s].launches++;
   }
   const int nrows = jlast - jfirst + 1;
   const int rows8 = !SW(c, PROFQ_ROWS2) && (SW(c, PROFQ_ROWS8) || (long)((c->P.iml + 63) / 64) * ((c->P.jml + 7) / 8) >= 3 * 256);
+  if ((fuse_prod != 1 && fuse_prod != 3) || !fuse_filter) cc = NULL;
+  if (fuse_prod == 1 && rows8) cc = NULL;
+  if (fuse_prod == 3 && c->prof_on) {
+    const int s = pomgpu_prof_slot(c, "profq_shear_in");
+    if (s >= 0) (c->parent ? c->parent : c)->prof[s].launches++;
+  }
+  if (cc && c->prof_on) {
+    const int s = pomgpu_prof_slot(c, "profq_cc_in");
+    if (s >= 0) (c->parent ? c->parent : c)->prof[s].launches++;
+  }
   const int cols = rho_rt && c->rho_rt_cols && !SW(c, RT_LOAD);
   if (cols && c->prof_on) {
     const int s = pomgpu_prof_slot(c, "profq_rm_flags");
     if (s >= 0) (c->parent ? c->parent : c)->prof[s].launches++;
   }
   rho_rt = (rho_rt ? 1 : 0) | (SW(c, PROFQ_NOPACE) ? 0 : 2) | (cols ? 4 : 0);
-#define PQ(FP, FF, LD)                                                                                                                   \
+#define PQ(FP, FF, LD, CC)                                                                                                                  \
   do {                                                                                                                                   \
-    if (rows8) LAUNCHN(c, "k_profq", (k_profq<FP, FF, PROFQ_BIG, LD>), dim3((c->P.iml + 63) / 64, (nrows + PROFQ_BIG - 1) / PROFQ_BIG, 1), dim3(64, PROFQ_BIG, 1), c->P, rho_rt, jfirst, jlast, c->rt_cols); \
-    else LAUNCHN(c, "k_profq", (k_profq<FP, FF, 2, LD>), dim3((c->P.iml + 63) / 64, (nrows + 1) / 2, 1), dim3(64, 2, 1), c->P, rho_rt, jfirst, jlast, c->rt_cols); \
+    if (rows8) LAUNCHN(c, "k_profq", (k_profq<FP, FF, PROFQ_BIG, LD, CC>), dim3((c->P.iml + 63) / 64, (nrows + PROFQ_BIG - 1) / PROFQ_BIG, 1), dim3(64, PROFQ_BIG, 1), c->P, rho_rt, jfirst, jlast, c->rt_cols, cc); \
+    else LAUNCHN(c, "k_profq", (k_profq<FP, FF, 2, LD, CC>), dim3((c->P.iml + 63) / 64, (nrows + 1) / 2, 1), dim3(64, 2, 1), c->P, rho_rt, jfirst, jlast, c->rt_cols, cc); \
   } while (0)
-  if (fuse_filter) { if (fuse_prod == 0) PQ(0, 1, 1); else if (fuse_prod == 1) { if (ld) PQ(1, 1, 1); else PQ(1, 1, 0); } else PQ(2, 1, 1); }
-  else { if (fuse_prod == 0) PQ(0, 0, 1); else if (fuse_prod == 1) PQ(1, 0, 1); else PQ(2, 0, 1); }
+#define PQ2(FP, FF, LD, CC) LAUNCHN(c, "k_profq", (k_profq<FP, FF, 2, LD, CC>), dim3((c->P.iml + 63) / 64, (nrows + 1) / 2, 1), dim3(64, 2, 1), c->P, rho_rt, jfirst, jlast, c->rt_cols, cc)
+  if (fuse_filter) {
+    if (fuse_prod == 0) PQ(0, 1, 1, 0);
+    else if (fuse_prod == 1) {
+      if (cc) { if (ld) PQ2(1, 1, 1, 1); else PQ2(1, 1, 0, 1); }
+      else { if (ld) PQ(1, 1, 1, 0); else PQ(1, 1, 0, 0); }
+    }
+#if POMGPU_UVM_ONLOAD
+    else if (fuse_prod == 3) {
+      if (cc) { if (ld) PQ(3, 1, 1, 1); else PQ(3, 1, 0, 1); }
+      else { if (ld) PQ(3, 1, 1, 0); else PQ(3, 1, 0, 0); }
+    }
+#endif
+    else PQ(2, 1, 1, 0);
+  }
+  else { if (fuse_prod == 0) PQ(0, 0, 1, 0); else if (fuse_prod == 1) PQ(1, 0, 1, 0); else PQ(2, 0, 1, 0); }
 #undef PQ
+#undef PQ2
   const KP &P = c->P;
   if (P.W || P.E || P.S || P.N) {
     const int len = P.im > P.jm ? P.im : P.jm;
diff --git a/extpom_amd/csrc/pomgpu_api.hip b/extpom_amd/csrc/pomgpu_api.hip
--- a/extpom_amd/csrc/pomgpu_api.hip
+++ b/extpom_amd/csrc/pomgpu_api.hip
@@ -251,6 +251,18 @@
   return (c->frc_on && (isrf < 1 || next % isrf == 0)) || (c->lat_on && (ibc < 1 || next % ibc == 0)) ||
          (c->wat_on && (iwater < 1 || (k.iint + 1) % iwater == 0));
 }
+static double *cc_handoff(pomgpu_ctx *c) {
+#ifdef POMGPU_COMPUTE_F32
+  return NULL;
+#endif
+  if (c->exch || c->tp.on || c->wide.on || c->parent || (c->flags & POMGPU_CTX_2D) || c->wr_eager || c->cc_failed) return NULL;
+  if (!c->cc) {
+    const size_t bytes = c->P.n3 * sizeof(double);
+    if (hipMalloc((void **)&c->cc, bytes) != hipSuccess) { (void)hipGetLastError(); c->cc = NULL; c->cc_failed = 1; return NULL; }
+    (void)hipMemsetAsync(c->cc, 0, bytes, c->stream);
+  }
+  return c->cc;
+}
 static void aam_buffers(pomgpu_ctx *c) {
   KP &P = c->P;
   P.aamc = (c->aam_parity && c->aam_spare) ? c->aam_spare : (P.b3 ? P.b3 + (size_t)P3_aam * P.a3 : NULL);
@@ -280,6 +292,7 @@
 }
 static void restore_materialize(pomgpu_ctx *c) {
   c->uvm_valid = 0;
+  c->cc_valid = 0;
   side_join(c);
   rho_materialize(c);
   pomgpu_wr_materialize(c);
@@ -363,7 +376,7 @@
     if (hipMemsetAsync(*p, 0, n * sizeof(double), c->stream) != hipSuccess) ok = false;
   };
   alloc(&P.b1, (size_t)POM_NBLK1D * P.kb);
-  alloc(&P.r1, (size_t)POM_NBLK1D * P.kb);
+  alloc(&P.r1, (size_t)(POM_NBLK1D + 1) * P.kb);
   alloc(&P.b2, (size_t)POM_NBLK2D * P.n2);
   const bool only2d = (flags & POMGPU_CTX_2D) != 0;
   if (!only2d) alloc(&P.b3, (size_t)POM_NBLK3D * P.a3);
@@ -433,6 +446,7 @@
   (void)hipFree(c->uvb_bot[0]); (void)hipFree(c->uvb_bot[1]);
   (void)hipFree(c->rt_words); (void)hipFree(c->rt_cols);
   (void)hipFree(c->aam_spare);
+  (void)hipFree(c->cc);
   for (int n = 0; n < POMGPU_NCOEF2; n++) (void)hipFree(P.c2[n]);
   (void)hipFree(c->alt2[0]); (void)hipFree(c->alt3[0]);
   (void)hipFree(P.m8);
@@ -503,6 +517,7 @@
 extern "C" int pomgpu_set_con(pomgpu_ctx *c, const pom_blkcon *con, int lramp) {
   if (!c || !con) return POMGPU_EINVAL;
   if (c->wr_pending && con->dti2 != c->P.dti2) pomgpu_wr_materialize(c);
+  if (con->tbias != c->con.tbias || con->sbias != c->con.sbias || con->grav != c->con.grav || con->rhoref != c->con.rhoref) c->cc_valid = 0;
   c->con = *con;
   c->lramp = lramp;
   sync_scalars(c);
@@ -814,7 +829,7 @@
   xch(c, 2, xf, P.kbm1, yf, P.kbm1);
   launch_advq_step(c, q, qb, qf, xf, yf, zero_else);
 }
-static void seq_profq(pomgpu_ctx *c, int fuse_filter = 0, int with_w = 0, int store_ld = 1) {
+static void seq_profq(pomgpu_ctx *c, int fuse_filter = 0, int with_w = 0, int store_ld = 1, const double *cc = NULL, int shear_in = 0) {
   KP &P = c->P;
   launch_profq_bc(c);
   double *ufkb = LEV3(c, D3(c, uf), P.kb - 1);
@@ -828,7 +843,7 @@
   }
   if (with_w) xch(c, 3, P.s2[4], 1, ufkb, 1, D3(c, w), P.kb);
   else xch(c, 2, P.s2[4], 1, ufkb, 1);
-  if (!c->exch) { launch_profq(c, 1, fuse_filter, c->rho_rt_pending, 0, -1, store_ld); return; }
+  if (!c->exch) { launch_profq(c, shear_in ? 3 : 1, fuse_filter, c->rho_rt_pending, 0, -1, store_ld, cc); return; }
   launch_profq_prod(c, 0, c->rho_rt_pending);
   xch(c, 1, LEV3(c, P.s3[0], 1), P.kbm2);
   launch_profq(c, 0, fuse_filter, c->rho_rt_pending);
@@ -1005,6 +1020,7 @@
 }
 void pomgpu_mirrors_written(pomgpu_ctx *c) {
   c->uvm_valid = 0;
+  c->cc_valid = 0;
   c->rho_rt_cols = 0;
   c->wide.static_done = 0;
   early_invalidate(c);
@@ -1615,6 +1631,7 @@
     P.uvm = uvm_onload(c) ? 1 : 0;
     if (!P.uvm) launch_int_uvmean(c);
     const bool wf = w_fused(c);
+    const bool shear = wf && P.uvm && !c->exch && !SW(c, QFILTER_SPLIT) && !SW(c, SHEAR_NOFUSE);
     if (!wf) launch_vertvl(c, 1);
     const bool lib_x = c->tp.on && c->exch;
     const bool rimr = lib_x && rim_side(c) && !SW(c, RIM_RESULTS_MAIN) && !SW(c, ADVQ_EXCHANGE) && !SW(c, PROD_FULL);
@@ -1632,7 +1649,7 @@
         launch_advq_col(c, D3(c, q2l), D3(c, q2lb), D3(c, vf), 1);
 #if POMGPU_W_FUSE
       } else if (wf) {
-        launch_advq2w_col(c, D3(c, q2), D3(c, q2b), D3(c, uf), D3(c, q2l), D3(c, q2lb), D3(c, vf), 1);
+        launch_advq2w_col(c, D3(c, q2), D3(c, q2b), D3(c, uf), D3(c, q2l), D3(c, q2lb), D3(c, vf), 1, shear);
 #endif
       } else {
         launch_advq2_col(c, D3(c, q2), D3(c, q2b), D3(c, uf), D3(c, q2l), D3(c, q2lb), D3(c, vf), 1);
@@ -1650,7 +1667,8 @@
       launch_profq_bc(c);
       launch_profq(c, 1, qfuse, c->rho_rt_pending, P.S ? 1 : 2, P.N ? P.jm : P.jmm1);
     } else {
-      seq_profq(c, qfuse, lib_x, !(defer_wr && ld_on_demand(c) && !next_step_fetches_record(c)));
+      const double *cc_in = (c->cc_valid && !SW(c, CC_LOAD_TS)) ? cc_handoff(c) : NULL;
+      seq_profq(c, qfuse, lib_x, !(defer_wr && ld_on_demand(c) && !next_step_fetches_record(c)), cc_in, shear);
       xch(c, 2, LEV3(c, D3(c, uf), 1), P.kbm2, LEV3(c, D3(c, vf), 1), P.kbm2);
     }
     launch_bcond6_edges(c);
@@ -1693,7 +1711,9 @@
       double fold, fnew;
       int rc = restore_prepare(c, &fold, &fnew);
       if (rc) return rc;
-      launch_ts_update(c, fold, fnew, k.nadv == 2, 0, ts_flags && !SW(c, RT_LOAD));
+      double *cc_out = cc_handoff(c);
+      launch_ts_update(c, fold, fnew, k.nadv == 2, 0, ts_flags && !SW(c, RT_LOAD), cc_out);
+      c->cc_valid = cc_out != NULL;
       c->rho_rt_pending = c->rho_rt_cols = 0;
       c->rst_pending = 1; c->rst_fold = fold; c->rst_fnew = fnew;
       if (rts) {
@@ -2279,6 +2299,7 @@
     return POMGPU_OK;
   };
   aam_canonical(c);
+  c->cc_valid = 0;
   const TuneLay cur = {c->tune_front, c->P.a3};
   int rc = POMGPU_OK;
   if ((to.f >= cur.f && to.a >= cur.a) || (to.f <= cur.f && to.a <= cur.a)) rc = one_way(cur, to);
diff --git a/extpom_amd/csrc/pomgpu_internal.hpp b/extpom_amd/csrc/pomgpu_internal.hpp
--- a/extpom_amd/csrc/pomgpu_internal.hpp
+++ b/extpom_amd/csrc/pomgpu_internal.hpp
@@ -95,9 +95,11 @@
 typedef const double __attribute__((address_space(4))) *pomgpu_cptr;
 #define F1(name, k) ((pomgpu_cptr)(size_t)P.b1)[(size_t)P1_##name * P.kb + ((k)-1)]
 #define R1(name, k) ((pomgpu_cptr)(size_t)P.r1)[(size_t)P1_##name * P.kb + ((k)-1)]
+#define RQ1(k) ((pomgpu_cptr)(size_t)P.r1)[(size_t)POM_NBLK1D * P.kb + ((k)-1)]
 #else
 #define F1(name, k) P.b1[(size_t)P1_##name * P.kb + ((k)-1)]
 #define R1(name, k) P.r1[(size_t)P1_##name * P.kb + ((k)-1)]
+#define RQ1(k) P.r1[(size_t)POM_NBLK1D * P.kb + ((k)-1)]
 #endif
 #define F2(name, i, j) P.b2[(size_t)P2_##name * P.n2 + IX2(i, j)]
 #define F3(name, i, j, k) REF3(P.b3 + (size_t)P3_##name * P.a3, IX3(i, j, k))
@@ -117,6 +119,14 @@
 #define BDI(name, a, k) P.bd[P.bdoff[PB_##name] + (size_t)((k)-1) * P.iml + (size_t)((a)-1)]
 
 __device__ __forceinline__ double sq(double x) { return x * x; }
+__device__ __forceinline__ double profq_cc_v(const KP &P, double t, double s_, double hij, int k) {
+  const double tp = t + P.tbias;
+  const double sp = s_ + P.sbias;
+  const double p = P.grav * P.rhoref * (-F1(zz, k) * hij) * 1.e-4;
+  double cc = 1449.1 + .00821 * p + 4.55 * tp - .045 * sq(tp) + 1.34 * (sp - 35.0);
+  cc = cc / sqrt((1. - .01642 * p / cc) * (1. - 0.40 * p / sq(cc)));
+  return cc;
+}
 
 enum pomgpu_coef2 {
   C2_HSX, C2_HSY,
@@ -470,7 +480,8 @@
   X(PROFQ_NOPACE) X(COL_STRIP) X(BAND_BYTES) X(PAD3) X(IO_SYNC) X(ADVCT_SPLIT) X(ADVQ_EXCHANGE) X(PROD_FULL) X(QFILTER_SPLIT) \
   X(NO_OVERLAP) X(NO_SIDE_COMM) X(WR_MAIN) X(WIDE_W) X(WIDE_FULL) X(DEBUG_ALLOC) X(TEST_SPLIT_FAIL_RANK)  \
   X(WR_NODEFER) X(EXT_RING_FIRST) X(TUNE_FORCE) X(RIM_MAIN) X(RIM_RESULTS_MAIN) X(SUM2D_OFF) X(ADVCT_ROWS4) X(ADVCT_ROWS8) \
-  X(IO_CHUNK_KB) X(UV_NOFUSE) X(W_NOFUSE) X(UVMEAN_PASS) X(PROFT_TWIN) X(LD_EAGER) X(TR_NOPAIR) X(RT_LOAD) X(AAM_NOFUSE)
+  X(IO_CHUNK_KB) X(UV_NOFUSE) X(W_NOFUSE) X(UVMEAN_PASS) X(PROFT_TWIN) X(LD_EAGER) X(TR_NOPAIR) X(RT_LOAD) X(AAM_NOFUSE) \
+  X(CC_LOAD_TS) X(SHEAR_NOFUSE)
 enum pomgpu_sw {
 #define POMGPU_SW_(name) SW_##name,
   POMGPU_SWITCHES(POMGPU_SW_)
@@ -591,6 +602,8 @@
   int uvm_valid;
   double *aam_spare;
   int aam_parity, aam_spare_failed, aam2d_done;
+  double *cc;
+  int cc_valid, cc_failed;
   double *uvb_bot[2];
   int wr_eager;
   double *d_vel;
@@ -709,7 +722,7 @@
                         const double *sc, double *sf, unsigned long long *rtf = NULL);
 void launch_advq2_col(pomgpu_ctx *c, const double *q, const double *qb, double *qf, const double *ql, const double *qlb, double *qlf, int zero_else);
 #if POMGPU_W_FUSE
-void launch_advq2w_col(pomgpu_ctx *c, const double *q, const double *qb, double *qf, const double *ql, const double *qlb, double *qlf, int zero_else);
+void launch_advq2w_col(pomgpu_ctx *c, const double *q, const double *qb, double *qf, const double *ql, const double *qlb, double *qlf, int zero_else, int shear = 0);
 #endif
 void launch_advuv_col(pomgpu_ctx *c);
 int launch_profuv_reg(pomgpu_ctx *c);
@@ -757,7 +770,7 @@
 void launch_copy3(pomgpu_ctx *c, double *dst, const double *src);
 void launch_aam_copy(pomgpu_ctx *c, double *dst, const double *src);
 void launch_advt2_diff(pomgpu_ctx *c, const double *fb, const double *fc, double *ff);
-void launch_ts_update(pomgpu_ctx *c, double fold, double fnew, int rt, int store_rst, int rt_flags = 0);
+void launch_ts_update(pomgpu_ctx *c, double fold, double fnew, int rt, int store_rst, int rt_flags = 0, double *cc = NULL);
 void launch_restore_fields(pomgpu_ctx *c, double fold, double fnew);
 void launch_mask_ts(pomgpu_ctx *c);
 struct TrUpd { const double *ff, *fc; double *f, *fb; };
@@ -776,7 +789,7 @@
 void launch_vertvl(pomgpu_ctx *c, int mask);
 void launch_profq_bc(pomgpu_ctx *c);
 void launch_profq_prod(pomgpu_ctx *c, int lines_only, int rho_rt = 0);
-void launch_profq(pomgpu_ctx *c, int fuse_prod, int fuse_filter, int rho_rt = 0, int jfirst = 0, int jlast = -1, int store_ld = 1);
+void launch_profq(pomgpu_ctx *c, int fuse_prod, int fuse_filter, int rho_rt = 0, int jfirst = 0, int jlast = -1, int store_ld = 1, const double *cc = NULL);
 void launch_proft(pomgpu_ctx *c, double *f, const double *wfsurf, const double *fsurf, int nbc);
 int launch_proft2(pomgpu_ctx *c, double *f0, const double *wfsurf0, const double *fsurf0, int nbc0, double *f1, const double *wfsurf1, const double *fsurf1, int nbc1);
 void launch_advu_profu(pomgpu_ctx *c, int do_adv, int do_prof);
```

After: 5.056 billion (median of 6 runs). No clear change (+0.5%).
